# jithendaraa/ODE-RL

Hardware: AMD Instinct MI355X
Metric: integrated latent frames/sec (ODEConvGRU, MovingMNIST) (higher is better)
Workload: dtype f32; 1 GPU; ODEConvGRU latents z0 (B=64,64,16,16) per GPU, T=10 output frames (9 intervals), fixed-step rk4 (3/8 rule), f = 5x conv3x3(64->64)+ReLU, forward only (BASELINE configs[1]); per_gpu_batch=64, frames=10, method=rk4, parallelism=batch-shard x1, nfe=36

## Files before the change

### include/odecgru_hip.h

```cpp
#ifndef ODECGRU_HIP_H
#define ODECGRU_HIP_H

#include <stddef.h>
#include <stdint.h>

#ifdef __cplusplus
extern "C" {
#endif

#define ODEHIP_ABI_VERSION 13
#define ODEHIP_MAX_LAYERS 8
#define ODEHIP_MAX_STAGES 7

enum {
  ODEHIP_OK = 0,
  ODEHIP_EINVAL = -1,
  ODEHIP_EHIP = -2,
  ODEHIP_ENOTCONV = -3,
  ODEHIP_ENAN = -4,
  ODEHIP_ETRUNC = -5
};

enum { ODEHIP_EULER = 0, ODEHIP_MIDPOINT = 1, ODEHIP_RK4 = 2, ODEHIP_DOPRI5 = 3 };

const char* odehip_last_error(void);
int odehip_version(void);
void odehip_set_debug_flags(int flags);
void odehip_set_debug_buffer(void* device_buffer);


size_t odehip_packed_weight_floats(int cout, int cin, int ks);

int odehip_pack_conv_weight(const float* w_oihw, float* w_packed, int cout, int cin, int ks,
                            int transpose_flip, void* stream);

size_t odehip_winograd_weight_floats(int cout, int cin);
int odehip_pack_conv_weight_winograd(const float* w_oihw, float* w_wino, int cout, int cin, int transpose_flip, void* stream);
#define ODEHIP_MAX_PACK_JOBS 32
typedef struct odehip_pack_job {
  const float* w;
  float* out;
  int cout, cin, ks, kind, transpose_flip;
} odehip_pack_job;
int odehip_pack_conv_weights(const odehip_pack_job* jobs, int n_jobs, void* stream);
size_t odehip_winograd5_weight_floats(int cout, int cin);
int odehip_pack_conv_weight_winograd5(const float* w_oihw, float* w_wino, int cout, int cin, int transpose_flip, void* stream);

size_t odehip_bf16_weight_bytes(int cout, int cin);
int odehip_pack_conv_weight_bf16(const float* w_oihw, void* w_bf16, int cout, int cin, int transpose_flip, void* stream);
size_t odehip_fused_bf16_weight_bytes(int n_layers);
int odehip_pack_convstack_fused_bf16(const float* w_oihw, void* w_fused, int exec_index, int transpose_flip, void* stream);
int odehip_pack_conv_weight_bf16_ks(const float* w_oihw, void* w_bf16, int cout, int cin, int ks, int transpose_flip, void* stream);

int odehip_nchw_to_q4(const float* src_nchw, float* dst_q4, int batch, int channels, void* stream);
int odehip_q4_to_nchw(const float* src_q4, float* dst_nchw, int batch, int channels, void* stream);


typedef struct odehip_conv_desc {
  const float* src1;
  const float* src2;
  int cin1, cin, cout, ks, batch;
  const float* w_packed;
  const float* w_wino;
  const void* w_bf16;
  const float* bias;
  float* dst;
  int relu;
} odehip_conv_desc;

int odehip_conv_q4(const odehip_conv_desc* d, void* stream);
struct odehip_convstack;
int odehip_debug_repeat_f(const struct odehip_convstack* f, const float* x_q4, float* out_q4, float* scratch, int batch, int n,
                          void* stream);
int odehip_debug_repeat_conv(const odehip_conv_desc* d, int n, void* stream);


typedef struct odehip_convstack {
  int n_convs;
  int ks;
  int channels[ODEHIP_MAX_LAYERS + 1];
  const float* w_packed[ODEHIP_MAX_LAYERS];
  const float* w_wino[ODEHIP_MAX_LAYERS];
  const void* w_bf16[ODEHIP_MAX_LAYERS];
  const void* w_fused;
  const float* bias[ODEHIP_MAX_LAYERS];
  int final_tanh;
  int act;
} odehip_convstack;

size_t odehip_convstack_workspace_bytes(const odehip_convstack* f, int batch);

int odehip_convstack_forward(const odehip_convstack* f, const float* y_nchw, float* out_nchw, int batch,
                             int negate, void* workspace, size_t workspace_bytes, void* stream);


size_t odehip_odeint_workspace_bytes(const odehip_convstack* f, int batch, int n_times, int method,
                                     int save_for_backward);

int odehip_odeint_fixed(const odehip_convstack* f, int method, const float* z0_nchw, const double* t_host,
                        int n_times, int batch, float* out_nchw, int save_for_backward, int negate, void* workspace,
                        size_t workspace_bytes, int* saved_format_out, void* stream);

int odehip_odeint_fixed_backward(const odehip_convstack* f, const odehip_convstack* f_dgrad, int method, const double* t_host,
                                 int n_times, int batch, const float* grad_out_nchw, float* grad_z0_nchw, float* const* grad_w,
                                 float* const* grad_b, int saved_format, void* workspace, size_t workspace_bytes, void* stream);

int odehip_odeint_adjoint_backward(const odehip_convstack* f, const odehip_convstack* f_dgrad, int method, const double* t_host,
                                   int n_times, int batch, const float* y_traj_nchw, const float* grad_out_nchw,
                                   float* grad_z0_nchw, float* const* grad_w, float* const* grad_b, void* workspace,
                                   size_t workspace_bytes, void* stream);

size_t odehip_adjoint_dopri5_workspace_bytes(const odehip_convstack* f, int batch, int n_times, int max_accept);
int odehip_odeint_adjoint_dopri5_backward(const odehip_convstack* f, const odehip_convstack* f_dgrad, const double* t_host,
                                          int n_times, int batch, float rtol, float atol, const float* y_traj_nchw,
                                          const float* grad_out_nchw, float* grad_z0_nchw, float* const* grad_w,
                                          float* const* grad_b, int max_accept, int mixed_norm, int* stats_host, void* workspace,
                                          size_t workspace_bytes, void* stream);


typedef struct odehip_convgru_cell {
  int input, hidden, ks;
  const float* w_gates;
  const float* b_gates;
  const float* gn_gates_w;
  const float* gn_gates_b;
  const float* w_can;
  const float* b_can;
  const float* gn_can_w;
  const float* gn_can_b;
  const void* w_gates_bf16;
  const void* w_can_bf16;
  const float* w_gates_wino;
  const float* w_can_wino;
} odehip_convgru_cell;

size_t odehip_convgru_cell_workspace_bytes(const odehip_convgru_cell* c, int batch);
int odehip_convgru_cell_forward(const odehip_convgru_cell* c, const float* x_nchw, const float* h_nchw, float* h_next_nchw,
                                int batch, void* workspace, size_t workspace_bytes, void* stream);

typedef struct odehip_encoder {
  odehip_convstack f_enc;
  odehip_convgru_cell cell;
  int head_hidden, out_ch;
  const float* w_head0;
  const float* b_head0;
  const float* w_head1;
  const float* b_head1;
} odehip_encoder;

size_t odehip_encoder_workspace_bytes(const odehip_encoder* e, int n_frames, int batch);
int odehip_odeconvgru_encode(const odehip_encoder* e, const float* inputs_nchw, const double* t_host, int n_frames, int batch,
                             int run_backwards, float* mean_nchw, float* std_nchw, float* latent_nchw, void* workspace,
                             size_t workspace_bytes, void* stream);
int odehip_odeconvgru_encode_masked(const odehip_encoder* e, const float* inputs_nchw, const double* t_host, int n_frames, int batch,
                                    int run_backwards, float* mean_nchw, float* std_nchw, float* latent_nchw, void* workspace,
                                    size_t workspace_bytes, void* stream, const float* mask_tb);
int odehip_odeconvgru_encode_steps(const odehip_encoder* e, const float* inputs_nchw, const double* t_host, int n_frames, int batch,
                                   int run_backwards, float* mean_nchw, float* std_nchw, float* latent_nchw, void* workspace,
                                   size_t workspace_bytes, void* stream, const float* mask_tb, const unsigned char* step_observed_host,
                                   int* cell_steps_run);

typedef struct odehip_convgru_cell_bwd {
  const float* w_gates_dx;
  const float* w_gates_dh;
  const float* w_can_dx;
  const float* w_can_dh;
  const void* bf16[4];
  const float* wino[4];
} odehip_convgru_cell_bwd;
typedef struct odehip_convgru_cell_grads {
  float *w_gates, *b_gates, *gn_gates_w, *gn_gates_b, *w_can, *b_can, *gn_can_w, *gn_can_b;
} odehip_convgru_cell_grads;
size_t odehip_convgru_cell_backward_workspace_bytes(const odehip_convgru_cell* c, int batch);
int odehip_convgru_cell_backward(const odehip_convgru_cell* c, const odehip_convgru_cell_bwd* cb, const float* x_nchw,
                                 const float* h_nchw, const float* grad_h_next_nchw, float* grad_x_nchw, float* grad_h_nchw,
                                 const odehip_convgru_cell_grads* grads, int batch, void* workspace, size_t workspace_bytes,
                                 void* stream);

typedef struct odehip_convgru_cell_halves {
  const float* wino[4];
  const void* bf16[4];
} odehip_convgru_cell_halves;
size_t odehip_convgru_sequence_workspace_bytes(const odehip_convgru_cell* c, int n_steps, int batch, int has_x, int train);
int odehip_convgru_sequence_forward(const odehip_convgru_cell* c, const odehip_convgru_cell_halves* hv, const float* x_seq_nchw, const float* h0_nchw, int n_steps,
                                    int batch, float* h_seq_nchw, void* workspace, size_t workspace_bytes, void* stream);
int odehip_convgru_sequence_train(const odehip_convgru_cell* c, const odehip_convgru_cell_halves* hv, const float* x_seq_nchw, const float* h0_nchw, int n_steps, int batch,
                                  float* h_seq_nchw, void* workspace, size_t workspace_bytes, void* stream);
int odehip_convgru_sequence_backward(const odehip_convgru_cell* c, const odehip_convgru_cell_halves* hv, const odehip_convgru_cell_bwd* cb, int has_x, int has_h0,
                                     int n_steps, int batch, const float* grad_h_seq_nchw, float* grad_x_seq_nchw,
                                     float* grad_h0_nchw, const odehip_convgru_cell_grads* grads, void* workspace,
                                     size_t workspace_bytes, void* stream);


typedef struct odehip_encoder_bwd {
  odehip_convstack f_dgrad;
  const float* w_gates_dx;
  const float* w_gates_dh;
  const float* w_can_dx;
  const float* w_can_dh;
  const float* w_head0_t;
  const float* w_head1_t;
  const void* bf16[4];
  const float* wino[4];
} odehip_encoder_bwd;

typedef struct odehip_encoder_grads {
  float* f_w[ODEHIP_MAX_LAYERS];
  float* f_b[ODEHIP_MAX_LAYERS];
  float *w_gates, *b_gates, *gn_gates_w, *gn_gates_b, *w_can, *b_can, *gn_can_w, *gn_can_b;
  float *w_head0, *b_head0, *w_head1, *b_head1;
} odehip_encoder_grads;

size_t odehip_encoder_train_workspace_bytes(const odehip_encoder* e, int n_frames, int batch);
int odehip_odeconvgru_encode_train(const odehip_encoder* e, const float* inputs_nchw, const double* t_host, int n_frames, int batch,
                                   int run_backwards, float* mean_nchw, float* std_nchw, float* latent_nchw, void* workspace,
                                   size_t workspace_bytes, void* stream);
int odehip_odeconvgru_encode_backward(const odehip_encoder* e, const odehip_encoder_bwd* eb, const double* t_host, int n_frames,
                                      int batch, int run_backwards, const float* grad_mean_nchw, const float* grad_std_nchw,
                                      const float* grad_latent_nchw, float* grad_inputs_nchw, const odehip_encoder_grads* grads,
                                      void* workspace, size_t workspace_bytes, void* stream);
int odehip_odeconvgru_encode_train_masked(const odehip_encoder* e, const float* inputs_nchw, const double* t_host, int n_frames,
                                          int batch, int run_backwards, float* mean_nchw, float* std_nchw, float* latent_nchw,
                                          void* workspace, size_t workspace_bytes, void* stream, const float* mask_tb);
int odehip_odeconvgru_encode_backward_masked(const odehip_encoder* e, const odehip_encoder_bwd* eb, const double* t_host, int n_frames,
                                             int batch, int run_backwards, const float* grad_mean_nchw, const float* grad_std_nchw,
                                             const float* grad_latent_nchw, float* grad_inputs_nchw, const odehip_encoder_grads* grads,
                                             void* workspace, size_t workspace_bytes, void* stream, const float* mask_tb);
int odehip_odeconvgru_encode_train_steps(const odehip_encoder* e, const float* inputs_nchw, const double* t_host, int n_frames,
                                         int batch, int run_backwards, float* mean_nchw, float* std_nchw, float* latent_nchw,
                                         void* workspace, size_t workspace_bytes, void* stream, const float* mask_tb,
                                         const unsigned char* step_observed_host, int* cell_steps_run);
int odehip_odeconvgru_encode_backward_steps(const odehip_encoder* e, const odehip_encoder_bwd* eb, const double* t_host, int n_frames,
                                            int batch, int run_backwards, const float* grad_mean_nchw, const float* grad_std_nchw,
                                            const float* grad_latent_nchw, float* grad_inputs_nchw, const odehip_encoder_grads* grads,
                                            void* workspace, size_t workspace_bytes, void* stream, const float* mask_tb,
                                            const unsigned char* step_observed_host, int* cell_steps_run);


typedef int (*odehip_allreduce_fn)(float* scratch_dev, int n, void* stream, void* user);
int odehip_set_norm_allreduce(odehip_allreduce_fn cb, void* user, int world_size, float* scratch_dev);

size_t odehip_dopri5_workspace_bytes(const odehip_convstack* f, int batch, int n_times);

int odehip_odeint_dopri5(const odehip_convstack* f, const float* z0_nchw, const double* t_host, int n_times, int batch,
                         float rtol, float atol, double first_step, int max_steps, int negate, float* out_nchw,
                         int* stats_host, double* accepted_host, int accepted_cap, void* workspace, size_t workspace_bytes,
                         void* stream);

size_t odehip_dopri5_backward_workspace_bytes(const odehip_convstack* f, int batch, int n_times, int n_steps);
int odehip_odeint_dopri5_backward(const odehip_convstack* f, const odehip_convstack* f_dgrad, const double* t_host, int n_times,
                                  int batch, const double* accepted_host, int n_steps, const float* z0_nchw,
                                  const float* grad_out_nchw, float* grad_z0_nchw, float* const* grad_w, float* const* grad_b,
                                  void* workspace, size_t workspace_bytes, void* stream);

size_t odehip_dopri5_saving_workspace_bytes(const odehip_convstack* f, int batch, int n_times, int max_accept);
int odehip_odeint_dopri5_saving(const odehip_convstack* f, const float* z0_nchw, const double* t_host, int n_times, int batch,
                                float rtol, float atol, double first_step, int max_steps, float* out_nchw, int* stats_host,
                                double* accepted_host, int accepted_cap, int max_accept, int* saved_out, void* workspace,
                                size_t workspace_bytes, void* stream);
int odehip_odeint_dopri5_backward_saved(const odehip_convstack* f, const odehip_convstack* f_dgrad, const double* t_host, int n_times,
                                        int batch, const double* accepted_host, int n_steps, const float* grad_out_nchw,
                                        float* grad_z0_nchw, float* const* grad_w, float* const* grad_b, int max_accept,
                                        void* saved_workspace, size_t saved_workspace_bytes, void* stream);

int odehip_odeint_dopri5_start(const odehip_convstack* f, const float* z0_nchw, const double* t_host, int n_times, int batch,
                               float rtol, float atol, double first_step, int max_steps, float* out_nchw, int max_accept,
                               int attempts, int* token_out, void* workspace, size_t workspace_bytes, void* stream);
int odehip_odeint_dopri5_collect(int token, int* stats_host, double* accepted_host, int accepted_cap, int* saved_out);


int odehip_adam_step(float* const* params, const float* const* grads, float* const* exp_avg, float* const* exp_avg_sq,
                     const long long* numel, int n_tensors, float lr, float beta1, float beta2, float eps, float weight_decay,
                     int step, void* stream);

size_t odehip_grad_norm_workspace_bytes(int n_tensors, const long long* numel);
int odehip_grad_norm(const float* const* grads, const long long* numel, int n_tensors, float max_norm, void* partials_ws, size_t ws_bytes,
                     float* out3, void* stream);
int odehip_grad_scale(float* const* grads, const long long* numel, int n_tensors, const float* coef_dev, void* stream);
int odehip_adam_step_clipped(float* const* params, float* const* grads, float* const* exp_avg, float* const* exp_avg_sq,
                             const long long* numel, int n_tensors, float lr, float beta1, float beta2, float eps, float weight_decay,
                             int step, const float* coef_dev, void* stream);

int odehip_adamax_step(float* const* params, const float* const* grads, float* const* exp_avg, float* const* exp_inf,
                       const long long* numel, int n_tensors, float lr, float beta1, float beta2, float eps, float weight_decay,
                       int step, void* stream);
int odehip_adamax_step_clipped(float* const* params, float* const* grads, float* const* exp_avg, float* const* exp_inf,
                               const long long* numel, int n_tensors, float lr, float beta1, float beta2, float eps, float weight_decay,
                               int step, const float* coef_dev, void* stream);


int odehip_warp_composite(const float* pred_outputs, const float* start_image, const float* grid_x, const float* grid_y, int batch,
                          int n_times, int channels, int height, int width, float* pred_x, float* warped, float* masks,
                          void* stream);
int odehip_warp_composite_backward(const float* pred_outputs, const float* start_image, const float* warped, const float* grid_x,
                                   const float* grid_y, const float* grad_pred_x, const float* grad_warped, const float* grad_masks,
                                   int batch, int n_times, int channels, int height, int width, float* grad_pred_outputs,
                                   float* grad_start_image, void* stream);

int odehip_upsample2x_bilinear(const float* in, float* out, long long planes, int height, int width, void* stream);
int odehip_upsample2x_bilinear_backward(const float* grad_out, float* grad_in, long long planes, int height, int width, void* stream);

size_t odehip_bn_workspace_bytes(int channels);
int odehip_bn_relu_up2x_forward(const float* x, int batch, int channels, int height, int width, const float* weight, const float* bias,
                                float* running_mean, float* running_var, int training, float momentum, float eps, int upsample, float* out,
                                float* mean_out, float* invstd_out, float* scale_out, float* shift_out, void* workspace,
                                size_t workspace_bytes, void* stream);
int odehip_bn_relu_up2x_backward(const float* grad_out, const float* x, int batch, int channels, int height, int width, const float* mean,
                                 const float* invstd, const float* scale, const float* shift, int training, int upsample, float* grad_x,
                                 float* grad_weight, float* grad_bias, float* g_pre, void* workspace, size_t workspace_bytes, void* stream);

int odehip_bn_sync_stats(const float* x, int batch, int channels, int height, int width, double* sums, void* workspace, size_t workspace_bytes,
                         void* stream);
int odehip_bn_sync_relu_up2x_forward(const float* x, int batch, int channels, int height, int width, const double* sums, const float* weight,
                                     const float* bias, float* running_mean, float* running_var, float momentum, float eps, int upsample,
                                     float* out, float* mean_out, float* invstd_out, float* scale_out, float* shift_out, void* stream);
int odehip_bn_sync_backward_sums(const float* grad_out, const float* x, int batch, int channels, int height, int width, const float* mean,
                                 const float* invstd, const float* scale, const float* shift, int upsample, float* g_pre, float* grad_weight,
                                 float* grad_bias, double* sums, void* workspace, size_t workspace_bytes, void* stream);
int odehip_bn_sync_backward_apply(const float* g_pre, const float* x, int batch, int channels, int height, int width, const float* mean,
                                  const float* invstd, const float* scale, const double* sums, const double* count, float* grad_x,
                                  void* workspace, size_t workspace_bytes, void* stream);

size_t odehip_frame_encoder_pack_floats(int in_ch, int out_ch);
int odehip_pack_frame_encoder(const float* w1, const float* b1, const float* w2, const float* b2, int in_ch, int out_ch, float* pack,
                              void* stream);
int odehip_frame_encode(const float* pack, const float* frames, int batch, int n_frames, int in_ch, int out_ch, float negative_slope,
                        float* out_time_first, void* stream);
size_t odehip_frame_decoder_pack_floats(int in_ch, int out_ch);
int odehip_pack_frame_decoder(const float* w1, const float* b1, const float* w2, const float* b2, int in_ch, int out_ch, float* pack,
                              void* stream);
int odehip_frame_decode(const float* pack, const float* latents, int n_images, int in_ch, int out_ch, float negative_slope,
                        int apply_sigmoid, float* out, void* stream);
int odehip_frame_decode_train(const float* pack, const float* latents, int n_images, int in_ch, int out_ch, float negative_slope,
                              int apply_sigmoid, float* out, float* mid_save, void* stream);
size_t odehip_frame_decode_backward_workspace_floats(int n_images, int in_ch, int out_ch);
int odehip_frame_decode_backward(const float* pack, const float* w1, const float* latents, const float* mid_saved, const float* pred,
                                 const float* g_out, int n_images, int in_ch, int out_ch, float negative_slope, int sigmoid_applied,
                                 float* g_latents, float* dw1, float* db1, float* dw2, float* db2, float* workspace,
                                 size_t workspace_floats, void* stream);
size_t odehip_frame_encode_backward_workspace_floats(int batch, int n_frames, int in_ch, int out_ch);
int odehip_frame_encode_backward(const float* pack, const float* w2, const float* frames, const float* out_time_first,
                                 const float* g_out_time_first, int batch, int n_frames, int in_ch, int out_ch, float negative_slope,
                                 float* dw1, float* db1, float* dw2, float* db2, float* workspace, size_t workspace_floats, void* stream);

int odehip_set_persistent_trajectory(int enable);
long long odehip_persistent_trajectory_launches(void);
int odehip_persistent_error(int clear);

int odehip_mmnist_render(const double* init, const int* digit_ids, const unsigned char* glyphs, int n_glyphs,
                         const float* lut256, int batch, int n_digits, int t_in, int t_out, float* out_in, float* out_pred,
                         void* stream);

int odehip_vidode_batch(const unsigned char* store, long long store_frames, int height, int width, int channels,
                        const float* lut256, const int* table, long long table_words, int batch, int n_outputs, float* const* outs,
                        const int* n_frames, void* stream);

int odehip_vidode_batch_rotated(const unsigned char* store, long long store_frames, int height, int width, int channels,
                                const unsigned char* frame_min, int input_norm, const int* table, long long table_words, int batch,
                                int n_outputs, float* const* outs, const int* n_frames, void* stream);

int odehip_frame_metrics(const float* pred, const float* truth, int batch, int n_frames, int channels, int height, int width,
                         float data_range, float* sse, float* ssim, float* mse, float* psnr, float* ssim_t, void* stream);

int odehip_png_metrics(const float* pred, const float* truth, int batch, int n_frames, int channels, int size, int denorm,
                       long long* sse, double* mse, double* ssim, unsigned char* pred_bytes, unsigned char* truth_bytes, void* accum,
                       void* stream);

int odehip_latent_sample(const float* mean, const float* std, int batch, int channels, int height, int width, int n_samples,
                         uint64_t seed, uint64_t offset, int batch_offset, int global_batch, const float* eps_in, float* z0, float* kl,
                         float* eps_out, void* stream);
int odehip_latent_sample_backward(const float* grad_z0, const float* grad_kl, const float* mean, const float* std, int batch,
                                  int channels, int height, int width, int n_samples, uint64_t seed, uint64_t offset, int batch_offset,
                                  int global_batch, const float* eps_in, float* grad_mean, float* grad_std, void* stream);

size_t odehip_loss_mse_workspace_bytes(int n_samples, int batch, long long row_elems);
int odehip_loss_mse(const float* pred, const float* truth, int n_samples, int batch, long long row_elems, const float* kl, double kl_scale,
                    float kl_weight, float* out, void* workspace, size_t workspace_bytes, void* stream);
int odehip_loss_mse_backward(const float* grad_out, const float* pred, const float* truth, int n_samples, int batch, long long row_elems,
                             double kl_scale, float kl_weight, float* grad_pred, float* grad_kl, void* stream);

size_t odehip_loss_vidode_l1_workspace_bytes(int batch, int n_sel, int frame_elems);
int odehip_loss_vidode_l1(const float* pred, const float* inter, long long inter_batch_stride, long long inter_frame_stride,
                          const float* truth, const float* init, long long init_batch_stride, const void* mask, int mask_is_byte, int batch,
                          int n_frames, int n_sel, int frame_elems, float* out, void* workspace, size_t workspace_bytes, void* stream);
int odehip_loss_vidode_l1_backward(const float* grad_out, const float* pred, const float* inter, long long inter_batch_stride,
                                   long long inter_frame_stride, const float* truth, const float* init, long long init_batch_stride,
                                   const void* mask, int mask_is_byte, int batch, int n_frames, int n_sel, int frame_elems, float* grad_pred,
                                   float* grad_inter, void* stream);

int odehip_instnorm_lrelu_forward(const float* x, int planes, int hw, float eps, float slope, float* y, float* mean, float* rstd,
                                  void* stream);
int odehip_instnorm_lrelu_backward(const float* grad_y, const float* x, const float* mean, const float* rstd, int planes, int hw,
                                   float slope, float* grad_x, void* stream);

int odehip_gan_seq_assemble(const float* input_real, const float* frames, int batch, int t_in, int t, long long frame_elems, int interp,
                            float* out, void* stream);
int odehip_gan_seq_assemble_backward(const float* grad_out, int batch, int t_in, int t, long long frame_elems, int interp, float* grad_frames,
                                     void* stream);

size_t odehip_loss_lsgan_workspace_bytes(long long n);
int odehip_loss_lsgan(const float* pred, long long n, float target, float* out, void* workspace, void* stream);
int odehip_loss_lsgan_backward(const float* grad_out, const float* pred, long long n, float target, float* grad, void* stream);

size_t odehip_grid_table_bytes(int n_grid, int n_times);
int odehip_grid_emit_table(const double* grid, int n_grid, const double* t, int n_times, int* first, float* slope, int* exact);
int odehip_grid_emit(const float* grid_states, float* out, const int* first, const float* slope, const int* exact, int n_grid,
                     int n_times, long long state_floats, void* table_dev, size_t table_bytes, void* stream);
int odehip_grid_scatter(const float* grad_out, float* grad_grid, const int* first, const float* slope, const int* exact, int n_grid,
                        int n_times, long long state_floats, void* table_dev, size_t table_bytes, void* stream);

#ifdef __cplusplus
}
#endif
#endif
```

### ode-rl_amd/_lib.py

```python
import ctypes
import os

_HERE = os.path.dirname(os.path.abspath(__file__))
LIB_PATH = os.environ.get("ODEHIP_LIB") or os.path.join(_HERE, "lib", "libodecgru_hip.so")

ABI_VERSION = 13
MAX_LAYERS = 8
MAX_STAGES = 7
EULER, MIDPOINT, RK4, DOPRI5 = 0, 1, 2, 3
METHODS = {"euler": EULER, "midpoint": MIDPOINT, "rk4": RK4, "dopri5": DOPRI5}

c_float_p = ctypes.POINTER(ctypes.c_float)


class ConvDesc(ctypes.Structure):
    _fields_ = [
        ("src1", ctypes.c_void_p), ("src2", ctypes.c_void_p),
        ("cin1", ctypes.c_int), ("cin", ctypes.c_int), ("cout", ctypes.c_int), ("ks", ctypes.c_int),
        ("batch", ctypes.c_int),
        ("w_packed", ctypes.c_void_p), ("w_wino", ctypes.c_void_p), ("w_bf16", ctypes.c_void_p), ("bias", ctypes.c_void_p),
        ("dst", ctypes.c_void_p), ("relu", ctypes.c_int),
    ]


MAX_PACK_JOBS = 32


class PackJob(ctypes.Structure):
    _fields_ = [("w", ctypes.c_void_p), ("out", ctypes.c_void_p), ("cout", ctypes.c_int), ("cin", ctypes.c_int), ("ks", ctypes.c_int),
                ("kind", ctypes.c_int), ("transpose_flip", ctypes.c_int)]


ACT_RELU, ACT_TANH = 0, 1


class ConvStack(ctypes.Structure):
    _fields_ = [
        ("n_convs", ctypes.c_int), ("ks", ctypes.c_int),
        ("channels", ctypes.c_int * (MAX_LAYERS + 1)),
        ("w_packed", ctypes.c_void_p * MAX_LAYERS),
        ("w_wino", ctypes.c_void_p * MAX_LAYERS),
        ("w_bf16", ctypes.c_void_p * MAX_LAYERS),
        ("w_fused", ctypes.c_void_p),
        ("bias", ctypes.c_void_p * MAX_LAYERS),
        ("final_tanh", ctypes.c_int),
        ("act", ctypes.c_int),
    ]


class ConvGRUCellDesc(ctypes.Structure):
    _fields_ = [("input", ctypes.c_int), ("hidden", ctypes.c_int), ("ks", ctypes.c_int),
                ("w_gates", ctypes.c_void_p), ("b_gates", ctypes.c_void_p), ("gn_gates_w", ctypes.c_void_p),
                ("gn_gates_b", ctypes.c_void_p), ("w_can", ctypes.c_void_p), ("b_can", ctypes.c_void_p),
                ("gn_can_w", ctypes.c_void_p), ("gn_can_b", ctypes.c_void_p),
                ("w_gates_bf16", ctypes.c_void_p), ("w_can_bf16", ctypes.c_void_p),
                ("w_gates_wino", ctypes.c_void_p), ("w_can_wino", ctypes.c_void_p)]


class ConvGRUCellHalves(ctypes.Structure):
    _fields_ = [("wino", ctypes.c_void_p * 4), ("bf16", ctypes.c_void_p * 4)]


class EncoderDesc(ctypes.Structure):
    _fields_ = [("f_enc", ConvStack), ("cell", ConvGRUCellDesc), ("head_hidden", ctypes.c_int), ("out_ch", ctypes.c_int),
                ("w_head0", ctypes.c_void_p), ("b_head0", ctypes.c_void_p), ("w_head1", ctypes.c_void_p),
                ("b_head1", ctypes.c_void_p)]


class ConvGRUCellBwd(ctypes.Structure):
    _fields_ = [("w_gates_dx", ctypes.c_void_p), ("w_gates_dh", ctypes.c_void_p), ("w_can_dx", ctypes.c_void_p),
                ("w_can_dh", ctypes.c_void_p), ("bf16", ctypes.c_void_p * 4), ("wino", ctypes.c_void_p * 4)]


class ConvGRUCellGrads(ctypes.Structure):
    _fields_ = [("w_gates", ctypes.c_void_p), ("b_gates", ctypes.c_void_p), ("gn_gates_w", ctypes.c_void_p),
                ("gn_gates_b", ctypes.c_void_p), ("w_can", ctypes.c_void_p), ("b_can", ctypes.c_void_p),
                ("gn_can_w", ctypes.c_void_p), ("gn_can_b", ctypes.c_void_p)]


class EncoderBwd(ctypes.Structure):
    _fields_ = [("f_dgrad", ConvStack), ("w_gates_dx", ctypes.c_void_p), ("w_gates_dh", ctypes.c_void_p),
                ("w_can_dx", ctypes.c_void_p), ("w_can_dh", ctypes.c_void_p), ("w_head0_t", ctypes.c_void_p),
                ("w_head1_t", ctypes.c_void_p), ("bf16", ctypes.c_void_p * 4), ("wino", ctypes.c_void_p * 4)]


class EncoderGrads(ctypes.Structure):
    _fields_ = [("f_w", ctypes.c_void_p * MAX_LAYERS), ("f_b", ctypes.c_void_p * MAX_LAYERS),
                ("w_gates", ctypes.c_void_p), ("b_gates", ctypes.c_void_p), ("gn_gates_w", ctypes.c_void_p),
                ("gn_gates_b", ctypes.c_void_p), ("w_can", ctypes.c_void_p), ("b_can", ctypes.c_void_p),
                ("gn_can_w", ctypes.c_void_p), ("gn_can_b", ctypes.c_void_p), ("w_head0", ctypes.c_void_p),
                ("b_head0", ctypes.c_void_p), ("w_head1", ctypes.c_void_p), ("b_head1", ctypes.c_void_p)]


ALLREDUCE_FN = ctypes.CFUNCTYPE(ctypes.c_int, ctypes.c_void_p, ctypes.c_int, ctypes.c_void_p, ctypes.c_void_p)


class OdeHipError(RuntimeError):
    pass


class AsyncSolveTruncated(OdeHipError):
    """An asynchronous dopri5 solve needed more attempted steps than were enqueued up front (ODEHIP_ETRUNC): the frames it had not
    reached are NaN and everything computed from them since is invalid.  The next asynchronous solve enqueues more; a training step
    can simply be repeated (nothing has been applied to the parameters)."""


_lib = None

SIGNATURES = {
    "odehip_last_error": (ctypes.c_char_p, []),
    "odehip_version": (ctypes.c_int, []),
    "odehip_bf16_weight_bytes": (ctypes.c_size_t, [ctypes.c_int, ctypes.c_int]),
    "odehip_pack_conv_weight_bf16": (ctypes.c_int, [ctypes.c_void_p, ctypes.c_void_p, ctypes.c_int, ctypes.c_int, ctypes.c_int,
                                                    ctypes.c_void_p]),
    "odehip_adam_step": (ctypes.c_int, [ctypes.POINTER(ctypes.c_void_p), ctypes.POINTER(ctypes.c_void_p),
                                        ctypes.POINTER(ctypes.c_void_p), ctypes.POINTER(ctypes.c_void_p),
                                        ctypes.POINTER(ctypes.c_longlong), ctypes.c_int, ctypes.c_float, ctypes.c_float,
                                        ctypes.c_float, ctypes.c_float, ctypes.c_float, ctypes.c_int, ctypes.c_void_p]),
    "odehip_grad_norm_workspace_bytes": (ctypes.c_size_t, [ctypes.c_int, ctypes.POINTER(ctypes.c_longlong)]),
    "odehip_grad_norm": (ctypes.c_int, [ctypes.POINTER(ctypes.c_void_p), ctypes.POINTER(ctypes.c_longlong), ctypes.c_int, ctypes.c_float,
                                        ctypes.c_void_p, ctypes.c_size_t, ctypes.c_void_p, ctypes.c_void_p]),
    "odehip_grad_scale": (ctypes.c_int, [ctypes.POINTER(ctypes.c_void_p), ctypes.POINTER(ctypes.c_longlong), ctypes.c_int, ctypes.c_void_p,
                                         ctypes.c_void_p]),
    "odehip_adam_step_clipped": (ctypes.c_int, [ctypes.POINTER(ctypes.c_void_p), ctypes.POINTER(ctypes.c_void_p),
                                                ctypes.POINTER(ctypes.c_void_p), ctypes.POINTER(ctypes.c_void_p),
                                                ctypes.POINTER(ctypes.c_longlong), ctypes.c_int, ctypes.c_float, ctypes.c_float,
                                                ctypes.c_float, ctypes.c_float, ctypes.c_float, ctypes.c_int, ctypes.c_void_p,
                                                ctypes.c_void_p]),
    "odehip_adamax_step": (ctypes.c_int, [ctypes.POINTER(ctypes.c_void_p)] * 4 + [ctypes.POINTER(ctypes.c_longlong), ctypes.c_int] +
                           [ctypes.c_float] * 5 + [ctypes.c_int, ctypes.c_void_p]),
    "odehip_adamax_step_clipped": (ctypes.c_int, [ctypes.POINTER(ctypes.c_void_p)] * 4 + [ctypes.POINTER(ctypes.c_longlong), ctypes.c_int] +
                                   [ctypes.c_float] * 5 + [ctypes.c_int, ctypes.c_void_p, ctypes.c_void_p]),
    "odehip_set_persistent_trajectory": (ctypes.c_int, [ctypes.c_int]),
    "odehip_persistent_trajectory_launches": (ctypes.c_longlong, []),
    "odehip_persistent_error": (ctypes.c_int, [ctypes.c_int]),
    "odehip_upsample2x_bilinear": (ctypes.c_int, [ctypes.c_void_p, ctypes.c_void_p, ctypes.c_longlong, ctypes.c_int, ctypes.c_int, ctypes.c_void_p]),
    "odehip_upsample2x_bilinear_backward": (ctypes.c_int, [ctypes.c_void_p, ctypes.c_void_p, ctypes.c_longlong, ctypes.c_int, ctypes.c_int,
                                                            ctypes.c_void_p]),
    "odehip_bn_workspace_bytes": (ctypes.c_size_t, [ctypes.c_int]),
    "odehip_bn_relu_up2x_forward": (ctypes.c_int, [ctypes.c_void_p] + [ctypes.c_int] * 4 + [ctypes.c_void_p] * 4 + [ctypes.c_int, ctypes.c_float,
                                                   ctypes.c_float, ctypes.c_int] + [ctypes.c_void_p] * 6 + [ctypes.c_size_t, ctypes.c_void_p]),
    "odehip_bn_relu_up2x_backward": (ctypes.c_int, [ctypes.c_void_p] * 2 + [ctypes.c_int] * 4 + [ctypes.c_void_p] * 4 + [ctypes.c_int] * 2 +
                                     [ctypes.c_void_p] * 5 + [ctypes.c_size_t, ctypes.c_void_p]),
    "odehip_bn_sync_stats": (ctypes.c_int, [ctypes.c_void_p] + [ctypes.c_int] * 4 + [ctypes.c_void_p] * 2 + [ctypes.c_size_t, ctypes.c_void_p]),
    "odehip_bn_sync_relu_up2x_forward": (ctypes.c_int, [ctypes.c_void_p] + [ctypes.c_int] * 4 + [ctypes.c_void_p] * 5 + [ctypes.c_float] * 2 +
                                         [ctypes.c_int] + [ctypes.c_void_p] * 6),
    "odehip_bn_sync_backward_sums": (ctypes.c_int, [ctypes.c_void_p] * 2 + [ctypes.c_int] * 4 + [ctypes.c_void_p] * 4 + [ctypes.c_int] +
                                     [ctypes.c_void_p] * 5 + [ctypes.c_size_t, ctypes.c_void_p]),
    "odehip_bn_sync_backward_apply": (ctypes.c_int, [ctypes.c_void_p] * 2 + [ctypes.c_int] * 4 + [ctypes.c_void_p] * 7 + [ctypes.c_size_t, ctypes.c_void_p]),
    "odehip_warp_composite": (ctypes.c_int, [ctypes.c_void_p] * 4 + [ctypes.c_int] * 5 + [ctypes.c_void_p] * 4),
    "odehip_warp_composite_backward": (ctypes.c_int, [ctypes.c_void_p] * 8 + [ctypes.c_int] * 5 + [ctypes.c_void_p] * 3),
    "odehip_winograd5_weight_floats": (ctypes.c_size_t, [ctypes.c_int, ctypes.c_int]),
    "odehip_pack_conv_weight_winograd5": (ctypes.c_int, [ctypes.c_void_p, ctypes.c_void_p, ctypes.c_int, ctypes.c_int, ctypes.c_int, ctypes.c_void_p]),
    "odehip_frame_encoder_pack_floats": (ctypes.c_size_t, [ctypes.c_int, ctypes.c_int]),
    "odehip_frame_decoder_pack_floats": (ctypes.c_size_t, [ctypes.c_int, ctypes.c_int]),
    "odehip_pack_frame_encoder": (ctypes.c_int, [ctypes.c_void_p] * 4 + [ctypes.c_int] * 2 + [ctypes.c_void_p] * 2),
    "odehip_pack_frame_decoder": (ctypes.c_int, [ctypes.c_void_p] * 4 + [ctypes.c_int] * 2 + [ctypes.c_void_p] * 2),
    "odehip_frame_encode": (ctypes.c_int, [ctypes.c_void_p, ctypes.c_void_p, ctypes.c_int, ctypes.c_int, ctypes.c_int, ctypes.c_int,
                                           ctypes.c_float, ctypes.c_void_p, ctypes.c_void_p]),
    "odehip_frame_decode_backward_workspace_floats": (ctypes.c_size_t, [ctypes.c_int] * 3),
    "odehip_frame_decode_train": (ctypes.c_int, [ctypes.c_void_p, ctypes.c_void_p, ctypes.c_int, ctypes.c_int, ctypes.c_int, ctypes.c_float,
                                                 ctypes.c_int, ctypes.c_void_p, ctypes.c_void_p, ctypes.c_void_p]),
    "odehip_frame_decode_backward": (ctypes.c_int, [ctypes.c_void_p] * 6 + [ctypes.c_int] * 3 + [ctypes.c_float, ctypes.c_int] +
                                     [ctypes.c_void_p] * 6 + [ctypes.c_size_t, ctypes.c_void_p]),
    "odehip_frame_encode_backward_workspace_floats": (ctypes.c_size_t, [ctypes.c_int] * 4),
    "odehip_frame_encode_backward": (ctypes.c_int, [ctypes.c_void_p] * 5 + [ctypes.c_int] * 4 + [ctypes.c_float] +
                                     [ctypes.c_void_p] * 5 + [ctypes.c_size_t, ctypes.c_void_p]),
    "odehip_frame_decode": (ctypes.c_int, [ctypes.c_void_p, ctypes.c_void_p, ctypes.c_int, ctypes.c_int, ctypes.c_int, ctypes.c_float,
                                           ctypes.c_int, ctypes.c_void_p, ctypes.c_void_p]),
    "odehip_mmnist_render": (ctypes.c_int, [ctypes.c_void_p, ctypes.c_void_p, ctypes.c_void_p, ctypes.c_int, ctypes.c_void_p,
                                            ctypes.c_int, ctypes.c_int, ctypes.c_int, ctypes.c_int, ctypes.c_void_p,
                                            ctypes.c_void_p, ctypes.c_void_p]),
    "odehip_vidode_batch": (ctypes.c_int, [ctypes.c_void_p, ctypes.c_longlong, ctypes.c_int, ctypes.c_int, ctypes.c_int, ctypes.c_void_p,
                                           ctypes.c_void_p, ctypes.c_longlong, ctypes.c_int, ctypes.c_int, ctypes.POINTER(ctypes.c_void_p),
                                           ctypes.POINTER(ctypes.c_int), ctypes.c_void_p]),
    "odehip_vidode_batch_rotated": (ctypes.c_int, [ctypes.c_void_p, ctypes.c_longlong, ctypes.c_int, ctypes.c_int, ctypes.c_int,
                                                   ctypes.c_void_p, ctypes.c_int, ctypes.c_void_p, ctypes.c_longlong, ctypes.c_int,
                                                   ctypes.c_int, ctypes.POINTER(ctypes.c_void_p), ctypes.POINTER(ctypes.c_int),
                                                   ctypes.c_void_p]),
    "odehip_frame_metrics": (ctypes.c_int, [ctypes.c_void_p] * 2 + [ctypes.c_int] * 5 + [ctypes.c_float] + [ctypes.c_void_p] * 6),
    "odehip_png_metrics": (ctypes.c_int, [ctypes.c_void_p] * 2 + [ctypes.c_int] * 5 + [ctypes.c_void_p] * 7),
    "odehip_latent_sample": (ctypes.c_int, [ctypes.c_void_p] * 2 + [ctypes.c_int] * 5 + [ctypes.c_uint64] * 2 + [ctypes.c_int] * 2 +
                             [ctypes.c_void_p] * 5),
    "odehip_latent_sample_backward": (ctypes.c_int, [ctypes.c_void_p] * 4 + [ctypes.c_int] * 5 + [ctypes.c_uint64] * 2 + [ctypes.c_int] * 2 +
                                      [ctypes.c_void_p] * 4),
    "odehip_loss_mse_workspace_bytes": (ctypes.c_size_t, [ctypes.c_int, ctypes.c_int, ctypes.c_longlong]),
    "odehip_loss_mse": (ctypes.c_int, [ctypes.c_void_p] * 2 + [ctypes.c_int, ctypes.c_int, ctypes.c_longlong, ctypes.c_void_p, ctypes.c_double,
                                       ctypes.c_float, ctypes.c_void_p, ctypes.c_void_p, ctypes.c_size_t, ctypes.c_void_p]),
    "odehip_loss_mse_backward": (ctypes.c_int, [ctypes.c_void_p] * 3 + [ctypes.c_int, ctypes.c_int, ctypes.c_longlong, ctypes.c_double,
                                                ctypes.c_float] + [ctypes.c_void_p] * 3),
    "odehip_loss_vidode_l1_workspace_bytes": (ctypes.c_size_t, [ctypes.c_int] * 3),
    "odehip_loss_vidode_l1": (ctypes.c_int, [ctypes.c_void_p] * 2 + [ctypes.c_longlong] * 2 + [ctypes.c_void_p] * 2 + [ctypes.c_longlong,
                                             ctypes.c_void_p] + [ctypes.c_int] * 5 + [ctypes.c_void_p] * 2 + [ctypes.c_size_t, ctypes.c_void_p]),
    "odehip_loss_vidode_l1_backward": (ctypes.c_int, [ctypes.c_void_p] * 3 + [ctypes.c_longlong] * 2 + [ctypes.c_void_p] * 2 +
                                       [ctypes.c_longlong, ctypes.c_void_p] + [ctypes.c_int] * 5 + [ctypes.c_void_p] * 3),
    "odehip_instnorm_lrelu_forward": (ctypes.c_int, [ctypes.c_void_p, ctypes.c_int, ctypes.c_int, ctypes.c_float, ctypes.c_float] +
                                      [ctypes.c_void_p] * 4),
    "odehip_instnorm_lrelu_backward": (ctypes.c_int, [ctypes.c_void_p] * 4 + [ctypes.c_int, ctypes.c_int, ctypes.c_float] + [ctypes.c_void_p] * 2),
    "odehip_gan_seq_assemble": (ctypes.c_int, [ctypes.c_void_p] * 2 + [ctypes.c_int] * 3 + [ctypes.c_longlong, ctypes.c_int] + [ctypes.c_void_p] * 2),
    "odehip_gan_seq_assemble_backward": (ctypes.c_int, [ctypes.c_void_p] + [ctypes.c_int] * 3 + [ctypes.c_longlong, ctypes.c_int] +
                                         [ctypes.c_void_p] * 2),
    "odehip_loss_lsgan_workspace_bytes": (ctypes.c_size_t, [ctypes.c_longlong]),
    "odehip_loss_lsgan": (ctypes.c_int, [ctypes.c_void_p, ctypes.c_longlong, ctypes.c_float] + [ctypes.c_void_p] * 3),
    "odehip_loss_lsgan_backward": (ctypes.c_int, [ctypes.c_void_p] * 2 + [ctypes.c_longlong, ctypes.c_float] + [ctypes.c_void_p] * 2),
    "odehip_grid_table_bytes":(ctypes.c_size_t, [ctypes.c_int, ctypes.c_int]),
    "odehip_grid_emit_table": (ctypes.c_int, [ctypes.POINTER(ctypes.c_double), ctypes.c_int, ctypes.POINTER(ctypes.c_double), ctypes.c_int,
                                              ctypes.POINTER(ctypes.c_int), ctypes.POINTER(ctypes.c_float), ctypes.POINTER(ctypes.c_int)]),
    "odehip_grid_emit": (ctypes.c_int, [ctypes.c_void_p, ctypes.c_void_p, ctypes.POINTER(ctypes.c_int), ctypes.POINTER(ctypes.c_float),
                                        ctypes.POINTER(ctypes.c_int), ctypes.c_int, ctypes.c_int, ctypes.c_longlong, ctypes.c_void_p,
                                        ctypes.c_size_t, ctypes.c_void_p]),
    "odehip_grid_scatter": (ctypes.c_int, [ctypes.c_void_p, ctypes.c_void_p, ctypes.POINTER(ctypes.c_int), ctypes.POINTER(ctypes.c_float),
                                           ctypes.POINTER(ctypes.c_int), ctypes.c_int, ctypes.c_int, ctypes.c_longlong, ctypes.c_void_p,
                                           ctypes.c_size_t, ctypes.c_void_p]),
    "odehip_fused_bf16_weight_bytes": (ctypes.c_size_t, [ctypes.c_int]),
    "odehip_pack_convstack_fused_bf16": (ctypes.c_int, [ctypes.c_void_p, ctypes.c_void_p, ctypes.c_int, ctypes.c_int, ctypes.c_void_p]),
    "odehip_pack_conv_weight_bf16_ks": (ctypes.c_int, [ctypes.c_void_p, ctypes.c_void_p, ctypes.c_int, ctypes.c_int, ctypes.c_int,
                                                       ctypes.c_int, ctypes.c_void_p]),
    "odehip_debug_repeat_f": (ctypes.c_int, [ctypes.POINTER(ConvStack), ctypes.c_void_p, ctypes.c_void_p, ctypes.c_void_p, ctypes.c_int,
                                             ctypes.c_int, ctypes.c_void_p]),
    "odehip_set_debug_flags": (None, [ctypes.c_int]),
    "odehip_set_norm_allreduce": (ctypes.c_int, [ctypes.c_void_p, ctypes.c_void_p, ctypes.c_int, ctypes.c_void_p]),
    "odehip_set_debug_buffer": (None, [ctypes.c_void_p]),
    "odehip_packed_weight_floats": (ctypes.c_size_t, [ctypes.c_int, ctypes.c_int, ctypes.c_int]),
    "odehip_pack_conv_weight": (ctypes.c_int, [ctypes.c_void_p, ctypes.c_void_p, ctypes.c_int, ctypes.c_int,
                                               ctypes.c_int, ctypes.c_int, ctypes.c_void_p]),
    "odehip_winograd_weight_floats": (ctypes.c_size_t, [ctypes.c_int, ctypes.c_int]),
    "odehip_pack_conv_weights": (ctypes.c_int, [ctypes.c_void_p, ctypes.c_int, ctypes.c_void_p]),
    "odehip_pack_conv_weight_winograd": (ctypes.c_int, [ctypes.c_void_p, ctypes.c_void_p, ctypes.c_int, ctypes.c_int,
                                                        ctypes.c_int, ctypes.c_void_p]),
    "odehip_nchw_to_q4": (ctypes.c_int, [ctypes.c_void_p, ctypes.c_void_p, ctypes.c_int, ctypes.c_int, ctypes.c_void_p]),
    "odehip_q4_to_nchw": (ctypes.c_int, [ctypes.c_void_p, ctypes.c_void_p, ctypes.c_int, ctypes.c_int, ctypes.c_void_p]),
    "odehip_conv_q4": (ctypes.c_int, [ctypes.POINTER(ConvDesc), ctypes.c_void_p]),
    "odehip_debug_repeat_conv": (ctypes.c_int, [ctypes.POINTER(ConvDesc), ctypes.c_int, ctypes.c_void_p]),
    "odehip_convstack_workspace_bytes": (ctypes.c_size_t, [ctypes.POINTER(ConvStack), ctypes.c_int]),
    "odehip_convstack_forward": (ctypes.c_int, [ctypes.POINTER(ConvStack), ctypes.c_void_p, ctypes.c_void_p,
                                                ctypes.c_int, ctypes.c_int, ctypes.c_void_p, ctypes.c_size_t,
                                                ctypes.c_void_p]),
    "odehip_odeint_workspace_bytes": (ctypes.c_size_t, [ctypes.POINTER(ConvStack), ctypes.c_int, ctypes.c_int,
                                                        ctypes.c_int, ctypes.c_int]),
    "odehip_odeint_fixed": (ctypes.c_int, [ctypes.POINTER(ConvStack), ctypes.c_int, ctypes.c_void_p,
                                           ctypes.POINTER(ctypes.c_double), ctypes.c_int, ctypes.c_int,
                                           ctypes.c_void_p, ctypes.c_int, ctypes.c_int, ctypes.c_void_p, ctypes.c_size_t,
                                           ctypes.POINTER(ctypes.c_int), ctypes.c_void_p]),
    "odehip_odeint_fixed_backward": (ctypes.c_int, [ctypes.POINTER(ConvStack), ctypes.POINTER(ConvStack), ctypes.c_int,
                                                    ctypes.POINTER(ctypes.c_double), ctypes.c_int, ctypes.c_int,
                                                    ctypes.c_void_p, ctypes.c_void_p, ctypes.POINTER(ctypes.c_void_p),
                                                    ctypes.POINTER(ctypes.c_void_p), ctypes.c_int, ctypes.c_void_p, ctypes.c_size_t,
                                                    ctypes.c_void_p]),
    "odehip_odeint_adjoint_backward": (ctypes.c_int, [ctypes.POINTER(ConvStack), ctypes.POINTER(ConvStack), ctypes.c_int,
                                                      ctypes.POINTER(ctypes.c_double), ctypes.c_int, ctypes.c_int,
                                                      ctypes.c_void_p, ctypes.c_void_p, ctypes.c_void_p,
                                                      ctypes.POINTER(ctypes.c_void_p), ctypes.POINTER(ctypes.c_void_p),
                                                      ctypes.c_void_p, ctypes.c_size_t, ctypes.c_void_p]),
    "odehip_adjoint_dopri5_workspace_bytes": (ctypes.c_size_t, [ctypes.POINTER(ConvStack), ctypes.c_int, ctypes.c_int,
                                                                ctypes.c_int]),
    "odehip_odeint_adjoint_dopri5_backward": (ctypes.c_int, [ctypes.POINTER(ConvStack), ctypes.POINTER(ConvStack),
                                                             ctypes.POINTER(ctypes.c_double), ctypes.c_int, ctypes.c_int,
                                                             ctypes.c_float, ctypes.c_float, ctypes.c_void_p,
                                                             ctypes.c_void_p, ctypes.c_void_p,
                                                             ctypes.POINTER(ctypes.c_void_p), ctypes.POINTER(ctypes.c_void_p),
                                                             ctypes.c_int, ctypes.c_int, ctypes.POINTER(ctypes.c_int), ctypes.c_void_p,
                                                             ctypes.c_size_t, ctypes.c_void_p]),
    "odehip_convgru_cell_workspace_bytes": (ctypes.c_size_t, [ctypes.POINTER(ConvGRUCellDesc), ctypes.c_int]),
    "odehip_convgru_cell_forward": (ctypes.c_int, [ctypes.POINTER(ConvGRUCellDesc), ctypes.c_void_p, ctypes.c_void_p,
                                                   ctypes.c_void_p, ctypes.c_int, ctypes.c_void_p, ctypes.c_size_t,
                                                   ctypes.c_void_p]),
    "odehip_convgru_sequence_workspace_bytes": (ctypes.c_size_t, [ctypes.POINTER(ConvGRUCellDesc)] + [ctypes.c_int] * 4),
    "odehip_convgru_sequence_forward": (ctypes.c_int, [ctypes.POINTER(ConvGRUCellDesc), ctypes.POINTER(ConvGRUCellHalves), ctypes.c_void_p, ctypes.c_void_p, ctypes.c_int,
                                                       ctypes.c_int, ctypes.c_void_p, ctypes.c_void_p, ctypes.c_size_t, ctypes.c_void_p]),
    "odehip_convgru_sequence_train": (ctypes.c_int, [ctypes.POINTER(ConvGRUCellDesc), ctypes.POINTER(ConvGRUCellHalves), ctypes.c_void_p, ctypes.c_void_p, ctypes.c_int,
                                                     ctypes.c_int, ctypes.c_void_p, ctypes.c_void_p, ctypes.c_size_t, ctypes.c_void_p]),
    "odehip_convgru_sequence_backward": (ctypes.c_int, [ctypes.POINTER(ConvGRUCellDesc), ctypes.POINTER(ConvGRUCellHalves), ctypes.POINTER(ConvGRUCellBwd)] + [ctypes.c_int] * 4 +
                                         [ctypes.c_void_p] * 3 + [ctypes.POINTER(ConvGRUCellGrads), ctypes.c_void_p, ctypes.c_size_t,
                                                                  ctypes.c_void_p]),
    "odehip_encoder_workspace_bytes": (ctypes.c_size_t, [ctypes.POINTER(EncoderDesc), ctypes.c_int, ctypes.c_int]),
    "odehip_odeconvgru_encode": (ctypes.c_int, [ctypes.POINTER(EncoderDesc), ctypes.c_void_p,
                                                ctypes.POINTER(ctypes.c_double), ctypes.c_int, ctypes.c_int, ctypes.c_int,
                                                ctypes.c_void_p, ctypes.c_void_p, ctypes.c_void_p, ctypes.c_void_p,
                                                ctypes.c_size_t, ctypes.c_void_p]),
    "odehip_odeconvgru_encode_masked": (ctypes.c_int, [ctypes.POINTER(EncoderDesc), ctypes.c_void_p,
                                                       ctypes.POINTER(ctypes.c_double), ctypes.c_int, ctypes.c_int, ctypes.c_int,
                                                       ctypes.c_void_p, ctypes.c_void_p, ctypes.c_void_p, ctypes.c_void_p,
                                                       ctypes.c_size_t, ctypes.c_void_p, ctypes.c_void_p]),
    "odehip_dopri5_workspace_bytes": (ctypes.c_size_t, [ctypes.POINTER(ConvStack), ctypes.c_int, ctypes.c_int]),
    "odehip_convgru_cell_backward_workspace_bytes": (ctypes.c_size_t, [ctypes.POINTER(ConvGRUCellDesc), ctypes.c_int]),
    "odehip_convgru_cell_backward": (ctypes.c_int, [ctypes.POINTER(ConvGRUCellDesc), ctypes.POINTER(ConvGRUCellBwd),
                                                    ctypes.c_void_p, ctypes.c_void_p, ctypes.c_void_p, ctypes.c_void_p,
                                                    ctypes.c_void_p, ctypes.POINTER(ConvGRUCellGrads), ctypes.c_int,
                                                    ctypes.c_void_p, ctypes.c_size_t, ctypes.c_void_p]),
    "odehip_encoder_train_workspace_bytes": (ctypes.c_size_t, [ctypes.POINTER(EncoderDesc), ctypes.c_int, ctypes.c_int]),
    "odehip_odeconvgru_encode_train": (ctypes.c_int, [ctypes.POINTER(EncoderDesc), ctypes.c_void_p,
                                                      ctypes.POINTER(ctypes.c_double), ctypes.c_int, ctypes.c_int, ctypes.c_int,
                                                      ctypes.c_void_p, ctypes.c_void_p, ctypes.c_void_p, ctypes.c_void_p,
                                                      ctypes.c_size_t, ctypes.c_void_p]),
    "odehip_odeconvgru_encode_backward": (ctypes.c_int, [ctypes.POINTER(EncoderDesc), ctypes.POINTER(EncoderBwd),
                                                         ctypes.POINTER(ctypes.c_double), ctypes.c_int, ctypes.c_int, ctypes.c_int,
                                                         ctypes.c_void_p, ctypes.c_void_p, ctypes.c_void_p, ctypes.c_void_p,
                                                         ctypes.POINTER(EncoderGrads), ctypes.c_void_p, ctypes.c_size_t,
                                                         ctypes.c_void_p]),
    "odehip_odeconvgru_encode_train_masked": (ctypes.c_int, [ctypes.POINTER(EncoderDesc), ctypes.c_void_p,
                                                             ctypes.POINTER(ctypes.c_double), ctypes.c_int, ctypes.c_int, ctypes.c_int,
                                                             ctypes.c_void_p, ctypes.c_void_p, ctypes.c_void_p, ctypes.c_void_p,
                                                             ctypes.c_size_t, ctypes.c_void_p, ctypes.c_void_p]),
    "odehip_odeconvgru_encode_backward_masked": (ctypes.c_int, [ctypes.POINTER(EncoderDesc), ctypes.POINTER(EncoderBwd),
                                                                ctypes.POINTER(ctypes.c_double), ctypes.c_int, ctypes.c_int, ctypes.c_int,
                                                                ctypes.c_void_p, ctypes.c_void_p, ctypes.c_void_p, ctypes.c_void_p,
                                                                ctypes.POINTER(EncoderGrads), ctypes.c_void_p, ctypes.c_size_t,
                                                                ctypes.c_void_p, ctypes.c_void_p]),
    "odehip_odeconvgru_encode_steps": (ctypes.c_int, [ctypes.POINTER(EncoderDesc), ctypes.c_void_p,
                                                      ctypes.POINTER(ctypes.c_double), ctypes.c_int, ctypes.c_int, ctypes.c_int,
                                                      ctypes.c_void_p, ctypes.c_void_p, ctypes.c_void_p, ctypes.c_void_p,
                                                      ctypes.c_size_t, ctypes.c_void_p, ctypes.c_void_p, ctypes.c_void_p,
                                                      ctypes.POINTER(ctypes.c_int)]),
    "odehip_odeconvgru_encode_train_steps": (ctypes.c_int, [ctypes.POINTER(EncoderDesc), ctypes.c_void_p,
                                                            ctypes.POINTER(ctypes.c_double), ctypes.c_int, ctypes.c_int, ctypes.c_int,
                                                            ctypes.c_void_p, ctypes.c_void_p, ctypes.c_void_p, ctypes.c_void_p,
                                                            ctypes.c_size_t, ctypes.c_void_p, ctypes.c_void_p, ctypes.c_void_p,
                                                            ctypes.POINTER(ctypes.c_int)]),
    "odehip_odeconvgru_encode_backward_steps": (ctypes.c_int, [ctypes.POINTER(EncoderDesc), ctypes.POINTER(EncoderBwd),
                                                               ctypes.POINTER(ctypes.c_double), ctypes.c_int, ctypes.c_int, ctypes.c_int,
                                                               ctypes.c_void_p, ctypes.c_void_p, ctypes.c_void_p, ctypes.c_void_p,
                                                               ctypes.POINTER(EncoderGrads), ctypes.c_void_p, ctypes.c_size_t,
                                                               ctypes.c_void_p, ctypes.c_void_p, ctypes.c_void_p,
                                                               ctypes.POINTER(ctypes.c_int)]),
    "odehip_odeint_dopri5": (ctypes.c_int, [ctypes.POINTER(ConvStack), ctypes.c_void_p, ctypes.POINTER(ctypes.c_double),
                                            ctypes.c_int, ctypes.c_int, ctypes.c_float, ctypes.c_float, ctypes.c_double, ctypes.c_int,
                                            ctypes.c_int, ctypes.c_void_p, ctypes.POINTER(ctypes.c_int),
                                            ctypes.POINTER(ctypes.c_double), ctypes.c_int, ctypes.c_void_p,
                                            ctypes.c_size_t, ctypes.c_void_p]),
    "odehip_dopri5_backward_workspace_bytes": (ctypes.c_size_t, [ctypes.POINTER(ConvStack), ctypes.c_int, ctypes.c_int,
                                                                 ctypes.c_int]),
    "odehip_dopri5_saving_workspace_bytes": (ctypes.c_size_t, [ctypes.POINTER(ConvStack), ctypes.c_int, ctypes.c_int, ctypes.c_int]),
    "odehip_odeint_dopri5_saving": (ctypes.c_int, [ctypes.POINTER(ConvStack), ctypes.c_void_p, ctypes.POINTER(ctypes.c_double),
                                                   ctypes.c_int, ctypes.c_int, ctypes.c_float, ctypes.c_float, ctypes.c_double, ctypes.c_int,
                                                   ctypes.c_void_p, ctypes.POINTER(ctypes.c_int), ctypes.POINTER(ctypes.c_double),
                                                   ctypes.c_int, ctypes.c_int, ctypes.POINTER(ctypes.c_int), ctypes.c_void_p,
                                                   ctypes.c_size_t, ctypes.c_void_p]),
    "odehip_odeint_dopri5_start": (ctypes.c_int, [ctypes.POINTER(ConvStack), ctypes.c_void_p, ctypes.POINTER(ctypes.c_double),
                                                  ctypes.c_int, ctypes.c_int, ctypes.c_float, ctypes.c_float, ctypes.c_double, ctypes.c_int,
                                                  ctypes.c_void_p, ctypes.c_int, ctypes.c_int, ctypes.POINTER(ctypes.c_int), ctypes.c_void_p,
                                                  ctypes.c_size_t, ctypes.c_void_p]),
    "odehip_odeint_dopri5_collect": (ctypes.c_int, [ctypes.c_int, ctypes.POINTER(ctypes.c_int), ctypes.POINTER(ctypes.c_double), ctypes.c_int,
                                                    ctypes.POINTER(ctypes.c_int)]),
    "odehip_odeint_dopri5_backward_saved": (ctypes.c_int, [ctypes.POINTER(ConvStack), ctypes.POINTER(ConvStack),
                                                           ctypes.POINTER(ctypes.c_double), ctypes.c_int, ctypes.c_int,
                                                           ctypes.POINTER(ctypes.c_double), ctypes.c_int, ctypes.c_void_p, ctypes.c_void_p,
                                                           ctypes.POINTER(ctypes.c_void_p), ctypes.POINTER(ctypes.c_void_p), ctypes.c_int,
                                                           ctypes.c_void_p, ctypes.c_size_t, ctypes.c_void_p]),
    "odehip_odeint_dopri5_backward": (ctypes.c_int, [ctypes.POINTER(ConvStack), ctypes.POINTER(ConvStack),
                                                     ctypes.POINTER(ctypes.c_double), ctypes.c_int, ctypes.c_int,
                                                     ctypes.POINTER(ctypes.c_double), ctypes.c_int, ctypes.c_void_p,
                                                     ctypes.c_void_p, ctypes.c_void_p, ctypes.POINTER(ctypes.c_void_p),
                                                     ctypes.POINTER(ctypes.c_void_p), ctypes.c_void_p, ctypes.c_size_t,
                                                     ctypes.c_void_p]),
}


def load():
    global _lib
    if _lib is not None:
        return _lib
    if not os.path.exists(LIB_PATH):
        raise OdeHipError(
            f"{LIB_PATH} is missing: build it with `python -c 'import __graft_entry__ as g; g.build()'` "
            "or `make -C ode-rl_amd/csrc`.  The HIP path has no CPU fallback.")
    lib = ctypes.CDLL(LIB_PATH)
    for name, (res, args) in SIGNATURES.items():
        fn = getattr(lib, name)
        fn.restype = res
        fn.argtypes = args
    got = lib.odehip_version()
    if got != ABI_VERSION:
        raise OdeHipError(f"{LIB_PATH} reports ABI version {got}, this binding needs {ABI_VERSION}: rebuild the library (make -C ode-rl_amd/csrc)")
    _lib = lib
    return lib


def check(rc):
    if rc == 0:
        code = _lib.odehip_persistent_error(1) if _lib is not None else 0
        if code:
            raise OdeHipError(f"a persistent launch of THIS OR AN EARLIER call gave up waiting for a partner workgroup (code {code}): the word is "
                              "read without synchronising, so the kernel that set it may belong to any call enqueued since the last check.  "
                              "Results since then are invalid (whole-trajectory launches NaN-fill their outputs; single-evaluation launches "
                              "may not); persistent launches are now disabled for this process")
        return
    msg = load().odehip_last_error().decode("utf-8", "replace")
    if rc == -1:
        raise ValueError(msg)
    if rc in (-3, -4):
        raise AssertionError(msg)
    if rc == -5:
        raise AsyncSolveTruncated(msg)
    raise OdeHipError(f"odehip status {rc}: {msg}")
```

### ode-rl_amd/csrc/conv_wino.hip

```cpp
#include <stddef.h>
#include <stdlib.h>
#include <string.h>

#include "conv_common.h"

namespace odehip {

constexpr int kWU = 32 * 1024;
constexpr int kWRaw = 16 * 1024;
constexpr int kWV = 32 * 1024;
constexpr int kWinoLds = 2 * kWRaw + 2 * kWV;
constexpr int kUAhead = 8;

__device__ __forceinline__ f32x4 load_u(__amdgpu_buffer_rsrc_t r, int voffset, int soffset) {
  return __builtin_bit_cast(f32x4, __builtin_amdgcn_raw_buffer_load_b128(r, voffset, soffset, 0));
}

__device__ __forceinline__ f32x4 pk_sub(f32x4 a, f32x4 b) {
  typedef float f32x2 __attribute__((ext_vector_type(2)));
  f32x2 lo, hi;
  const f32x2 alo = {a.x, a.y}, ahi = {a.z, a.w}, blo = {b.x, b.y}, bhi = {b.z, b.w};
  asm("v_pk_add_f32 %0, %1, %2 neg_lo:[0,1] neg_hi:[0,1]" : "=v"(lo) : "v"(alo), "v"(blo));
  asm("v_pk_add_f32 %0, %1, %2 neg_lo:[0,1] neg_hi:[0,1]" : "=v"(hi) : "v"(ahi), "v"(bhi));
  return f32x4{lo.x, lo.y, hi.x, hi.y};
}

struct PersistHook {
  unsigned* done = nullptr;
  unsigned target = 0u;
  int word0 = 0;
  unsigned* abort_ = nullptr;
  unsigned* host_err = nullptr;
  bool fence = false;
  float* nchw_base = nullptr;
  unsigned long long* stamps = nullptr;
  int batch = 0;
  bool first = true;
  bool solo = false;
  bool announce = true;
  bool split_wait = false;
  int sleep6 = 0;
  const unsigned long long* reloc = nullptr;
  unsigned wait_target = 0u;
};

template <typename T>
__device__ __forceinline__ T* rel(const unsigned long long* reloc, T* p) {
  const unsigned long long v = (unsigned long long)p;
  const unsigned cls = (unsigned)(v >> 56);
  if (cls == 0) return p;
  typedef const __attribute__((address_space(4))) unsigned long long ConstU;
  return (T*)((v & 0x00ffffffffffffffull) + *((ConstU*)reloc + cls));
}
__device__ __forceinline__ void pstamp(const PersistHook& hk, int i, int lane) {
  if (hk.stamps && lane == 0) hk.stamps[i] = __builtin_amdgcn_s_memrealtime();
}

template <typename T>
__device__ __forceinline__ T* uniform_ptr(T* p) {
  const unsigned long long v = (unsigned long long)p;
  const unsigned lo = __builtin_amdgcn_readfirstlane((unsigned)v), hi = __builtin_amdgcn_readfirstlane((unsigned)(v >> 32));
  return (T*)(((unsigned long long)hi << 32) | lo);
}

__device__ __forceinline__ void wait_done(const PersistHook& hk, int sel_mask = 0, int sel_val = 0) {
  int n = 0;
  const int lane = threadIdx.x & 63;
  const bool mine = lane < 16 && (lane & sel_mask) == sel_val;
  while (!__all(!mine || __hip_atomic_load(hk.done + (lane & 15), __ATOMIC_RELAXED, __HIP_MEMORY_SCOPE_AGENT) >= hk.wait_target)) {
    __builtin_amdgcn_s_sleep(1);
    if ((++n & 1023) == 0) {
      if (__hip_atomic_load(hk.abort_, __ATOMIC_RELAXED, __HIP_MEMORY_SCOPE_AGENT) == 1u) break;
      if (n > (1 << 23)) {
        __hip_atomic_store(hk.abort_, 1u, __ATOMIC_RELAXED, __HIP_MEMORY_SCOPE_AGENT);
        *hk.host_err = 3;
        break;
      }
    }
  }
  if (hk.fence) __builtin_amdgcn_fence(__ATOMIC_ACQUIRE, "agent");
}

__device__ __forceinline__ void announce(const PersistHook& hk, unsigned* done_word, bool stamp = false) {
  const int lane = threadIdx.x & 63;
  wait_vmcnt<0>();
  if (stamp) pstamp(hk, 7, lane);
  if (hk.fence) __builtin_amdgcn_fence(__ATOMIC_RELEASE, "agent");
  if (lane == 0 && hk.announce) __hip_atomic_store(done_word, hk.target + 1u, __ATOMIC_RELAXED, __HIP_MEMORY_SCOPE_AGENT);
}

template <int GROUP>
__device__ __forceinline__ bool xcc_rendezvous(unsigned* xcc_of, int lid, unsigned* abort_word, unsigned* host_err) {
  const unsigned my_xcc = (__builtin_amdgcn_s_getreg((3 << 11) | 20) & 15u) + 1u;
  if (threadIdx.x == 0) __hip_atomic_store(xcc_of + lid, my_xcc, __ATOMIC_RELAXED, __HIP_MEMORY_SCOPE_AGENT);
  bool fence = false;
  for (int p = 0; p < GROUP; ++p) {
    unsigned v = 0;
    int n = 0;
    while ((v = __hip_atomic_load(xcc_of + (lid & ~(GROUP - 1)) + p, __ATOMIC_RELAXED, __HIP_MEMORY_SCOPE_AGENT)) == 0) {
      __builtin_amdgcn_s_sleep(2);
      if (++n > (1 << 23)) {
        __hip_atomic_store(abort_word, 1u, __ATOMIC_RELAXED, __HIP_MEMORY_SCOPE_AGENT);
        *host_err = 2;
        break;
      }
    }
    fence |= (v != my_xcc);
  }
  return __builtin_amdgcn_readfirstlane(fence);
}

__device__ __forceinline__ bool walk_start(const ConvArgs*& table, int& n_layers, const int* section) {
  typedef const __attribute__((address_space(4))) int ConstI;
  const int* skip = table[0].skip;
  if (skip && *(ConstI*)skip) return false;
  if (section) {
    const int row0 = ((ConstI*)section)[0], n_dev = ((ConstI*)section)[1];
    if (row0 < 0 || n_dev <= 0 || row0 + n_dev > n_layers) return false;
    table += row0;
    n_layers = n_dev;
  }
  return true;
}

struct RowCursor {
  const ConvArgs* table;
  int n_layers;
  const float *src, *u, *src_next, *u_next;
  __device__ __forceinline__ RowCursor(const ConvArgs* t, int n)
      : table(t), n_layers(n), src(t[0].src1), u(t[0].w_wino), src_next(nullptr), u_next(nullptr) {}
  __device__ __forceinline__ const ConvArgs& row(int l) {
    typedef const __attribute__((address_space(4))) ConvArgs ConstArgs;
    const ConvArgs& a = *(const ConvArgs*)((ConstArgs*)table + l);
    src_next = src;
    u_next = u;
    if (l + 1 < n_layers) {
      src_next = table[l + 1].src1;
      u_next = table[l + 1].w_wino;
      if (threadIdx.x < (sizeof(ConvArgs) + 63) / 64) {
        const unsigned v = __builtin_nontemporal_load((const unsigned*)&table[l + 1] + threadIdx.x * 16);
        asm volatile("" ::"v"(v));
      }
    }
    return a;
  }
  __device__ __forceinline__ void next() {
    src = src_next;
    u = u_next;
  }
};

template <int NCHUNK, bool DBG, bool PERSIST, int QOUT = 16, bool ADAPT = false>
__device__ __forceinline__ void wino_layer(const float* __restrict__ p_src, const float* __restrict__ p_u, int p_qin, const ConvArgs& a,
                                           int b, int ct, int rh, char* smem, const PersistHook& hk) {
  static_assert(!PERSIST || (NCHUNK % 2 == 0), "the layer-to-layer LDS hand-over assumes an even chunk count");
  static_assert(kUAhead % 2 == 0 && kUAhead <= 16, "the U ring is refilled a pair of positions at a time");
  constexpr int kRawAux = PERSIST ? 16 : 0;
  char* const Rb = smem;
  char* const Vb = smem + 2 * kWRaw;
  Stamps st(a, (DBG && (a.debug & 16)) ? 256 : (DBG ? 0 : -1));
  st.take(0);
  const int tid = threadIdx.x;
  const int lane = tid & 63;
  const int wave = __builtin_amdgcn_readfirstlane(tid >> 6);
  const int r0 = rh * 8;
  constexpr int nchunk = NCHUNK;
  const bool skip = !PERSIST && a.skip && *a.skip;
  const bool dbg_noprod = DBG && (a.debug & 1), dbg_nomfma = DBG && (a.debug & 2), dbg_notr = DBG && (a.debug & 32),
             dbg_nodma = DBG && (a.debug & 128);

  if (wave >= 4) {
    const int pw = wave - 4, ptid = tid - 256;
    const __amdgpu_buffer_rsrc_t rx = make_rsrc((const char*)p_src + (size_t)b * p_qin * kQuadBytes, (unsigned)p_qin * kQuadBytes);
    int vr[4];
#pragma unroll
    for (int p = 0; p < 4; ++p) {
      const int s = 64 * p + lane;
      const int row = s / 20, w = s - row * 20;
      const int pc = w < 9 ? 2 * w : 2 * (w - 9) + 1;
      const int irow = r0 - 1 + row, col = pc - 1;
      vr[p] = (s < 200 && w < 18 && irow >= 0 && irow < kHW && col >= 0 && col < kHW) ? irow * 256 + col * 16 : kOobOffset;
    }
    auto issue_raw = [&](int c, int buf) {
#pragma unroll
      for (int p = 0; p < 4; ++p)
        __builtin_amdgcn_raw_ptr_buffer_load_lds(rx, ODEHIP_LDS_PTR(Rb + buf * kWRaw + (pw * 4 + p) * 1024), 16, vr[p],
                                                 (c * 4 + pw) * kQuadBytes, 0, kRawAux);
    };
    const int th = lane >> 5, tq = pw, tt = lane & 31;
    (void)ptid;
    const int tty = tt >> 3, ttx = tt & 7;
    const int r_a = th == 0 ? 2 : 1, r_b = th == 0 ? 0 : 2, r_c = th == 0 ? 1 : 3;
    const int raw_base = tq * 4096 + (2 * tty * 20 + ttx) * 16;
    const int off_a = raw_base + r_a * 320, off_b = raw_base + r_b * 320, off_c = raw_base + r_c * 320;
    const float sgn = th == 0 ? 1.0f : -1.0f;
    const int v_off = tq * 512 + tt * 16;
    auto transform = [&](int rbuf, int vbuf) {
      const char* r = Rb + rbuf * kWRaw;
      f32x4 d0[4], d1[4], d2[4];
#pragma unroll
      for (int j = 0; j < 4; ++j) {
        if (DBG && (a.debug & 512)) {
          d0[j] = d1[j] = d2[j] = f32x4{1.f, 2.f, 3.f, (float)j};
        } else {
          const int cj = ((j & 1) * 9 + (j >> 1)) * 16;
          d0[j] = *(const f32x4*)(r + off_a + cj);
          d1[j] = *(const f32x4*)(r + off_b + cj);
          d2[j] = *(const f32x4*)(r + off_c + cj);
        }
      }
      f32x4 T[2][4];
#pragma unroll
      for (int j = 0; j < 4; ++j) {
        T[0][j] = pk_sub(d1[j], d0[j]);
        T[1][j] = d2[j] + d0[j] * sgn;
      }
#pragma unroll
      for (int i = 0; i < 2; ++i) {
        char* v = Vb + vbuf * kWV + v_off + (2 * th + i) * 4 * 2048;
        if (DBG && (a.debug & 256)) {
          const f32x4 sum = (T[i][0] - T[i][2]) + (T[i][1] + T[i][2]) + (T[i][2] - T[i][1]) + (T[i][1] - T[i][3]);
          asm volatile("" ::"v"(sum.x), "v"(sum.y), "v"(sum.z), "v"(sum.w));
        } else {
          *(f32x4*)(v + 0 * 2048) = pk_sub(T[i][0], T[i][2]);
          *(f32x4*)(v + 1 * 2048) = T[i][1] + T[i][2];
          *(f32x4*)(v + 2 * 2048) = pk_sub(T[i][2], T[i][1]);
          *(f32x4*)(v + 3 * 2048) = pk_sub(T[i][1], T[i][3]);
        }
      }
    };

    if (PERSIST) {
      if (pw == 0) pstamp(hk, 0, lane);
      if (!hk.first) {
        if (hk.solo && hk.wait_target == hk.target)
          for (int i = 0; i < hk.sleep6; ++i) __builtin_amdgcn_s_sleep(6);
        if (hk.split_wait) wait_done(hk, 0x8, 0x0); else wait_done(hk);
      }
      if (pw == 0) pstamp(hk, 1, lane);
      issue_raw(0, 0);
      issue_raw(1, 1);
      wait_vmcnt<4>();
      if (pw == 0) pstamp(hk, 2, lane);
      transform(0, 0);
      if (pw == 0) pstamp(hk, 3, lane);
    } else if (!skip && !dbg_noprod) {
      issue_raw(0, 0);
      if (nchunk > 1) issue_raw(1, 1);
      if (nchunk > 1) wait_vmcnt<4>(); else wait_vmcnt<0>();
      transform(0, 0);
    }
    st.take(2);
#pragma unroll
    for (int c = 0; c < nchunk; ++c) {
      __builtin_amdgcn_s_barrier();
      if (!skip && !dbg_noprod && c + 1 < nchunk) {
        if (c + 2 < nchunk) {
          if (PERSIST && c == 0 && !hk.first && hk.split_wait) wait_done(hk, 0x8, 0x8);
          if (!dbg_nodma) issue_raw(c + 2, c & 1);
          wait_vmcnt<4>();
        } else {
          wait_vmcnt<0>();
        }
        if (!dbg_notr) transform((c + 1) & 1, (c + 1) & 1);
      }
      if (c < 4) st.take(3 + c);
    }
    st.flush(a);
    return;
  }

  const int ch = wave >> 1, thh = wave & 1;
  const int i16 = lane & 15, kq = lane >> 4;
  f32x4 acc[16];
#pragma unroll
  for (int x = 0; x < 16; ++x) acc[x] = f32x4{0.f, 0.f, 0.f, 0.f};
  const int u_off = kq * 512 + (ch * 16 + i16) * 16;
  const int v_off = kq * 512 + (thh * 16 + i16) * 16;
  constexpr int kG = 16 * NCHUNK;
  const bool dbg_nou = dbg_noprod || dbg_nodma;
  const __amdgpu_buffer_rsrc_t ru = make_rsrc((const char*)p_u + (size_t)ct * (NCHUNK * kWU), (unsigned)NCHUNK * kWU);
  f32x4 uw[kUAhead];
#pragma unroll
  for (int g = 0; g < kUAhead; ++g) {
    if (skip || dbg_nou) uw[g] = f32x4{1.f, 1.f, 1.f, 1.f};
    else uw[g] = load_u(ru, u_off, g * 2048);
  }
  const int Q = ct * 8 + ch * 4 + kq;
  f32x4 bias4 = {0.f, 0.f, 0.f, 0.f};
  if (a.bias) bias4 = *(const f32x4*)(a.bias + Q * 4);
  const int tile = thh * 16 + i16, oty = tile >> 3, otx = tile & 7;
  int e_combine = 0, e_act = 0, e_np = 0;
  float* e_dst = nullptr;
  float* e_kout = nullptr;
  float* e_out1 = nullptr;
  float* e_out2 = nullptr;
  float* e_nchw = nullptr;
  bool e_y = false;
  float e_h = 1.0f, e_ks = 1.0f, e_c1c = 0.0f, e_c2c = 0.0f, e_c1[3] = {0.f, 0.f, 0.f}, e_c2[3] = {0.f, 0.f, 0.f};
  f32x4 e_yv[4], e_kv[3][4];
  int d_kind = 0;
  f32x4 d_y[4], d_y1[4], d_sa[4], d_sb[4];
  float d_h = 1.0f, d_ks = 1.0f, d_cA = 0.0f, d_cB = 0.0f, d_rtol = 0.0f, d_atol = 0.0f, d_t[6] = {0.f, 0.f, 0.f, 0.f, 0.f, 0.f};
  float* d_o[4] = {nullptr, nullptr, nullptr, nullptr};
  bool d_has_y = false, d_err = false, d_f[4] = {false, false, false, false};
  if constexpr (ADAPT) {
    typedef const __attribute__((address_space(4))) float ConstF;
    const unsigned long long* const rl = hk.reloc;
    e_act = a.act;
    e_dst = rel(rl, a.dst);
    d_kind = a.combine == 0 ? 0 : 5;
    if (a.combine == 2) {
      const BwdArgs& w = a.bwd;
      const float hb = a.h_by_value ? a.cmb.atol : (w.h_ptr ? *(ConstF*)w.h_ptr : 0.0f);
      d_ks = w.sc_c + w.sc_h * hb;
      d_has_y = w.mask_src != nullptr;
      d_kind = 2;
      const float* const mask = rel(rl, w.mask_src);
#pragma unroll
      for (int q = 0; q < 4; ++q) {
        const size_t off = (((size_t)b * QOUT + Q) * kPix + (r0 + 2 * oty + (q >> 1)) * 16 + 2 * otx + (q & 1)) * 4;
        if (d_has_y) d_y[q] = *(const f32x4*)(mask + off);
      }
    } else if (a.combine == 3 && a.bwd.n_targets <= 2 && !a.bwd.h_ptr) {
      const BwdArgs& w = a.bwd;
      d_kind = 3;
#pragma unroll
      for (int t = 0; t < 2; ++t) {
        if (t < w.n_targets) {
          const BwdTarget& T = w.tgt[t];
          d_o[t] = rel(rl, T.out);
          d_t[3 * t] = T.g_c; d_t[3 * t + 1] = T.a_c; d_t[3 * t + 2] = T.b_c;
          d_f[2 * t] = T.srcA != nullptr; d_f[2 * t + 1] = T.srcB != nullptr;
          const float* const sA = rel(rl, T.srcA);
          const float* const sB = rel(rl, T.srcB);
#pragma unroll
          for (int q = 0; q < 4; ++q) {
            const size_t off = (((size_t)b * QOUT + Q) * kPix + (r0 + 2 * oty + (q >> 1)) * 16 + 2 * otx + (q & 1)) * 4;
            if (t == 0) {
              if (d_f[0]) d_y[q] = *(const f32x4*)(sA + off);
              if (d_f[1]) d_y1[q] = *(const f32x4*)(sB + off);
            } else {
              if (d_f[2]) d_sa[q] = *(const f32x4*)(sA + off);
              if (d_f[3]) d_sb[q] = *(const f32x4*)(sB + off);
            }
          }
        }
      }
    } else if (a.combine == 1 && (a.cmb.order == 1 || !a.cmb.y) && !(a.cmb.err_partials && (a.cmb.out2 || a.cmb.out2_nchw || a.dbg))) {
      const CombineArgs& m = a.cmb;
      d_kind = 1;
      const int np = m.n_prev;
      d_h = a.h_by_value ? m.atol : (m.h_ptr ? *(ConstF*)m.h_ptr : 1.0f);
      d_ks = m.k_scale;
      d_err = m.err_partials != nullptr;
      d_has_y = m.y != nullptr;
      d_cA = m.c1[np];
      d_cB = d_err ? m.ce[np] : m.c2[np];
      d_rtol = m.rtol; d_atol = m.atol;
      d_o[0] = rel(rl, m.k_out); d_o[1] = rel(rl, m.out1); d_o[2] = rel(rl, m.out2);
      d_o[3] = a.dbg ? hk.nchw_base + ((size_t)a.dbg - 1) : m.out2_nchw;
      const bool needB = d_err || d_o[2] || d_o[3];
      const float* const yp = rel(rl, m.y);
      const float* const y1p = rel(rl, m.err_y1);
#pragma unroll
      for (int q = 0; q < 4; ++q) {
        d_sa[q] = d_sb[q] = f32x4{0.f, 0.f, 0.f, 0.f};
        if (d_has_y) {
          const size_t off = (((size_t)b * QOUT + Q) * kPix + (r0 + 2 * oty + (q >> 1)) * 16 + 2 * otx + (q & 1)) * 4;
          d_y[q] = *(const f32x4*)(yp + off);
          if (d_err) d_y1[q] = *(const f32x4*)(y1p + off);
        }
      }
      if (d_has_y) {
        const float* kp[ODEHIP_MAX_STAGES - 1];
        float cA[ODEHIP_MAX_STAGES - 1], cB[ODEHIP_MAX_STAGES - 1];
#pragma unroll
        for (int j = 0; j < ODEHIP_MAX_STAGES - 1; ++j) {
          kp[j] = j < np ? rel(rl, m.k_prev[j]) : nullptr;
          cA[j] = m.c1[j];
          cB[j] = d_err ? m.ce[j] : m.c2[j];
        }
#pragma unroll
        for (int j = 0; j < ODEHIP_MAX_STAGES - 1; ++j) {
          if (j < np) {
#pragma unroll
            for (int q = 0; q < 4; ++q) {
              const size_t off = (((size_t)b * QOUT + Q) * kPix + (r0 + 2 * oty + (q >> 1)) * 16 + 2 * otx + (q & 1)) * 4;
              const f32x4 kv = *(const f32x4*)(kp[j] + off);
              d_sa[q] = fma4(kv, cA[j], d_sa[q]);
              if (needB) d_sb[q] = fma4(kv, cB[j], d_sb[q]);
            }
          }
        }
      }
    }
  } else if (PERSIST) {
    e_combine = a.combine;
    e_act = a.act;
    e_dst = a.dst;
    if (e_combine == 1 && !a.h_by_value) e_combine = 3;
    if (e_combine == 2) {
      const BwdArgs& w = a.bwd;
      typedef const __attribute__((address_space(4))) float ConstF;
      const float hb = a.h_by_value ? a.cmb.atol : (w.h_ptr ? *(ConstF*)w.h_ptr : 0.0f);
      e_ks = w.sc_c + w.sc_h * hb;
      e_y = w.mask_src != nullptr;
#pragma unroll
      for (int q = 0; q < 4; ++q) {
        const size_t off = (((size_t)b * QOUT + Q) * kPix + (r0 + 2 * oty + (q >> 1)) * 16 + 2 * otx + (q & 1)) * 4;
        if (e_y) e_yv[q] = *(const f32x4*)(w.mask_src + off);
      }
    } else if (e_combine == 1) {
      const CombineArgs& m = a.cmb;
      e_np = m.n_prev;
      e_h = m.atol;
      e_ks = m.k_scale;
      e_c1c = m.c1[e_np];
      e_c2c = m.c2[e_np];
      e_kout = m.k_out;
      e_out1 = m.out1;
      e_out2 = m.out2;
      e_nchw = a.dbg ? hk.nchw_base + ((size_t)a.dbg - 1) : nullptr;
      e_y = m.y != nullptr;
#pragma unroll
      for (int q = 0; q < 4; ++q) {
        const size_t off = (((size_t)b * QOUT + Q) * kPix + (r0 + 2 * oty + (q >> 1)) * 16 + 2 * otx + (q & 1)) * 4;
        if (e_y) e_yv[q] = *(const f32x4*)(m.y + off);
#pragma unroll
        for (int j = 0; j < 3; ++j)
          if (j < e_np) e_kv[j][q] = *(const f32x4*)(m.k_prev[j] + off);
      }
#pragma unroll
      for (int j = 0; j < 3; ++j) {
        e_c1[j] = m.c1[j];
        e_c2[j] = m.c2[j];
      }
    }
  }
  st.take(2);
#pragma unroll
  for (int c = 0; c < nchunk; ++c) {
    __builtin_amdgcn_s_barrier();
    if (PERSIST && c == 0 && wave == 0) pstamp(hk, 4, lane);
    if (!skip && !dbg_nomfma) {
      const char* v = Vb + (c & 1) * kWV + v_off;
      f32x4 x0 = *(const f32x4*)(v), x1 = *(const f32x4*)(v + 2048);
      f32x4 x0n, x1n;
#pragma unroll
      for (int x = 0; x < 16; x += 2) {
        const int g = c * 16 + x, s0 = g % kUAhead, s1 = (g + 1) % kUAhead;
        const f32x4 w0 = uw[s0], w1 = uw[s1];
        if (x + 2 < 16) {
          x0n = *(const f32x4*)(v + (x + 2) * 2048);
          x1n = *(const f32x4*)(v + (x + 3) * 2048);
        }
        if (g + kUAhead < kG && !dbg_nou) {
          uw[s0] = load_u(ru, u_off, (g + kUAhead) * 2048);
          uw[s1] = load_u(ru, u_off, (g + kUAhead + 1) * 2048);
        }
        acc[x] = __builtin_amdgcn_mfma_f32_16x16x4f32(w0.x, x0.x, acc[x], 0, 0, 0);
        acc[x + 1] = __builtin_amdgcn_mfma_f32_16x16x4f32(w1.x, x1.x, acc[x + 1], 0, 0, 0);
        acc[x] = __builtin_amdgcn_mfma_f32_16x16x4f32(w0.y, x0.y, acc[x], 0, 0, 0);
        acc[x + 1] = __builtin_amdgcn_mfma_f32_16x16x4f32(w1.y, x1.y, acc[x + 1], 0, 0, 0);
        acc[x] = __builtin_amdgcn_mfma_f32_16x16x4f32(w0.z, x0.z, acc[x], 0, 0, 0);
        acc[x + 1] = __builtin_amdgcn_mfma_f32_16x16x4f32(w1.z, x1.z, acc[x + 1], 0, 0, 0);
        acc[x] = __builtin_amdgcn_mfma_f32_16x16x4f32(w0.w, x0.w, acc[x], 0, 0, 0);
        acc[x + 1] = __builtin_amdgcn_mfma_f32_16x16x4f32(w1.w, x1.w, acc[x + 1], 0, 0, 0);
        x0 = x0n; x1 = x1n;
        __builtin_amdgcn_sched_group_barrier(0x008, 1, 0);
        __builtin_amdgcn_sched_group_barrier(0x100, 2, 0);
        __builtin_amdgcn_sched_group_barrier(0x020, 2, 0);
        __builtin_amdgcn_sched_group_barrier(0x008, 7, 0);
        __builtin_amdgcn_sched_barrier(0);
      }
    }
    if (st.on && c < 4) {
      asm volatile("" ::"v"(acc[15][0]));
      st.take(3 + c);
    }
  }
  if (skip) return;
  if (PERSIST && wave == 0) pstamp(hk, 5, lane);

  f32x4 S[2][4];
#pragma unroll
  for (int cI = 0; cI < 4; ++cI) {
    S[0][cI] = acc[0 * 4 + cI] + acc[1 * 4 + cI] + acc[2 * 4 + cI];
    S[1][cI] = pk_sub(pk_sub(acc[1 * 4 + cI], acc[2 * 4 + cI]), acc[3 * 4 + cI]);
  }
  float esum = 0.0f;
  auto emit_pre = [&](int q, int P, f32x4 v) {
    const size_t off = (((size_t)b * QOUT + Q) * kPix + P) * 4;
    if (!e_combine) {
      *(f32x4*)(e_dst + off) = act_fwd(v, e_act);
      return;
    }
    if (e_combine == 2) {
      v *= e_ks;
      if (e_y) v = act_bwd(v, e_yv[q], e_act);
      *(f32x4*)(e_dst + off) = v;
      return;
    }
    if (e_combine == 3) {
      emit_quad<false>(a, b, Q, P, v, esum);
      return;
    }
    const f32x4 kc = act_fwd(v, e_act) * e_ks;
    if (e_kout) *(f32x4*)(e_kout + off) = kc;
    if (e_y) {
      if (e_out1) {
        f32x4 sa = kc * e_c1c;
#pragma unroll
        for (int j = 0; j < 3; ++j)
          if (j < e_np) sa += e_kv[j][q] * e_c1[j];
        *(f32x4*)(e_out1 + off) = e_yv[q] + sa * e_h;
      }
      if (e_out2 || e_nchw) {
        f32x4 sb = kc * e_c2c;
#pragma unroll
        for (int j = 0; j < 3; ++j)
          if (j < e_np) sb += e_kv[j][q] * e_c2[j];
        const f32x4 o2 = e_yv[q] + sb * e_h;
        if (e_out2) *(f32x4*)(e_out2 + off) = o2;
        if (e_nchw) {
          float* o = e_nchw + ((size_t)b * (QOUT * 4) + Q * 4) * kPix + P;
          o[0] = o2.x; o[kPix] = o2.y; o[2 * kPix] = o2.z; o[3 * kPix] = o2.w;
        }
      }
    }
  };
  auto emit_adapt = [&](int q, int P, f32x4 v) {
    const size_t off = (((size_t)b * QOUT + Q) * kPix + P) * 4;
    if (d_kind == 0) {
      *(f32x4*)(e_dst + off) = act_fwd(v, e_act);
    } else if (d_kind == 2) {
      v *= d_ks;
      if (d_has_y) v = act_bwd(v, d_y[q], e_act);
      *(f32x4*)(e_dst + off) = v;
    } else if (d_kind == 1) {
      const f32x4 kc = act_fwd(v, e_act) * d_ks;
      if (d_o[0]) *(f32x4*)(d_o[0] + off) = kc;
      if (d_has_y) {
        if (d_o[1]) *(f32x4*)(d_o[1] + off) = fma4(fma4(kc, d_cA, d_sa[q]), d_h, d_y[q]);
        if (d_err) {
          esum = combine1_err(fma4(kc, d_cB, d_sb[q]), d_h, d_y[q], d_y1[q], d_rtol, d_atol, esum);
        } else if (d_o[2] || d_o[3]) {
          const f32x4 o2 = fma4(fma4(kc, d_cB, d_sb[q]), d_h, d_y[q]);
          if (d_o[2]) *(f32x4*)(d_o[2] + off) = o2;
          if (d_o[3]) {
            float* o = d_o[3] + ((size_t)b * (QOUT * 4) + Q * 4) * kPix + P;
            o[0] = o2.x; o[kPix] = o2.y; o[2 * kPix] = o2.z; o[3 * kPix] = o2.w;
          }
        }
      }
    } else if (d_kind == 3) {
      if (d_o[0]) {
        f32x4 o = v * d_t[0];
        if (d_f[0]) o = fma4(d_y[q], d_t[1], o);
        if (d_f[1]) o = fma4(d_y1[q], d_t[2], o);
        *(f32x4*)(d_o[0] + off) = o;
      }
      if (d_o[1]) {
        f32x4 o = v * d_t[3];
        if (d_f[2]) o = fma4(d_sa[q], d_t[4], o);
        if (d_f[3]) o = fma4(d_sb[q], d_t[5], o);
        *(f32x4*)(d_o[1] + off) = o;
      }
    } else {
      emit_quad(a, b, Q, P, v, esum, a.dbg ? hk.nchw_base + ((size_t)a.dbg - 1) : nullptr);
    }
  };
#pragma unroll
  for (int i = 0; i < 2; ++i) {
    const f32x4 y0 = S[i][0] + S[i][1] + S[i][2] + bias4;
    const f32x4 y1 = pk_sub(pk_sub(S[i][1] + bias4, S[i][2]), S[i][3]);
    const int P = (r0 + 2 * oty + i) * 16 + 2 * otx;
    if constexpr (ADAPT) {
      emit_adapt(2 * i, P, y0);
      emit_adapt(2 * i + 1, P + 1, y1);
    } else if (PERSIST) {
      emit_pre(2 * i, P, y0);
      emit_pre(2 * i + 1, P + 1, y1);
    } else {
      emit_quad(a, b, Q, P, y0, esum);
      emit_quad(a, b, Q, P + 1, y1, esum);
    }
  }
  if (PERSIST) {
    if (a.combine == 1 && a.cmb.err_partials) {
#pragma unroll
      for (int o = 32; o > 0; o >>= 1) esum += __shfl_xor(esum, o, 64);
      const int nwg_pl = (QOUT / 4) * hk.batch, lid_pl = b * (QOUT / 4) + ct * 2 + rh;
      const int bid_pl = (nwg_pl & 7) == 0 ? (lid_pl % (nwg_pl >> 3)) * 8 + lid_pl / (nwg_pl >> 3) : lid_pl;
      if (lane == 0) a.cmb.err_partials[bid_pl * 4 + wave] = esum;
    }
    if (wave == 0) pstamp(hk, 6, lane);
    announce(hk, hk.done + hk.word0 + wave, wave == 0);
  } else {
    finish_err(a, esum, wave);
    st.flush(a);
  }
}

template <int NCHUNK, bool DBG>
__global__ __launch_bounds__(512, 1) void conv3x3_wino_kernel(const float* __restrict__ p_src, const float* __restrict__ p_u,
                                                              int p_qin, int p_qout, const ConvArgs a) {
  extern __shared__ __attribute__((aligned(16))) char smem[];
  (void)p_qout;
  const int nwg = gridDim.x * gridDim.y;
  int lid = blockIdx.x + gridDim.x * blockIdx.y;
  if ((nwg & 7) == 0) lid = (lid & 7) * (nwg >> 3) + (lid >> 3);
  const int rh = lid & 1, ct = (lid >> 1) % (gridDim.x >> 1), b = (lid >> 1) / (gridDim.x >> 1);
  const PersistHook none;
  wino_layer<NCHUNK, DBG, false>(p_src, p_u, p_qin, a, b, ct, rh, smem, none);
}

struct PersistArgs {
  const ConvArgs* table;
  int n_layers, batch;
  unsigned* done;
  unsigned* xcc_of;
  unsigned* host_err;
  float* out_nchw;
  unsigned long long* stamps;
  int sleep6;
  int sleep6_combine;
  const int* n_layers_ptr;
  const unsigned long long* reloc;
  int fault_inject;
};

template <int QOUT>
__device__ __forceinline__ void ew_row(const ConvArgs& a, int b, int ct, int rh, const PersistHook& hk) {
  const int tid = threadIdx.x, lane = tid & 63;
  const int wave = __builtin_amdgcn_readfirstlane(tid >> 6);
  if (wave >= 4) return;
  typedef const __attribute__((address_space(4))) float ConstF;
  const CombineArgs& m = a.cmb;
  const unsigned long long* const rl = hk.reloc;
  const float hs = m.h_ptr ? *(ConstF*)m.h_ptr : 1.0f;
  const int ch = wave >> 1, thh = wave & 1, i16 = lane & 15, kq = lane >> 4;
  const int Q = ct * 8 + ch * 4 + kq, tile = thh * 16 + i16, oty = tile >> 3, otx = tile & 7, r0 = rh * 8;
  const float* const yp = rel(rl, m.y);
  if (a.combine == 5) {
    const float* const pa = rel(rl, m.k_prev[0]);
    const float* const pb = m.n_prev > 1 ? rel(rl, m.k_prev[1]) : nullptr;
    float sum = 0.0f;
#pragma unroll
    for (int q = 0; q < 4; ++q) {
      const size_t o = (((size_t)b * QOUT + Q) * kPix + (r0 + 2 * oty + (q >> 1)) * 16 + 2 * otx + (q & 1)) * 4;
      f32x4 d = *(const f32x4*)(pa + o);
      const f32x4 yv = *(const f32x4*)(yp + o);
      if (pb) d -= *(const f32x4*)(pb + o);
#pragma unroll
      for (int i = 0; i < 4; ++i) {
        const float r = d[i] / __builtin_fmaf(fabsf(yv[i]), m.rtol, m.atol);
        sum = __builtin_fmaf(r, r, sum);
      }
    }
#pragma unroll
    for (int o = 32; o > 0; o >>= 1) sum += __shfl_xor(sum, o, 64);
    if (lane == 0) m.err_partials[(b * 4 + ct * 2 + rh) * 4 + wave] = sum;
    wait_vmcnt<0>();
    if (hk.fence) __builtin_amdgcn_fence(__ATOMIC_RELEASE, "agent");
    if (lane == 0) __hip_atomic_store(hk.done + hk.word0 + wave, hk.target + 1u, __ATOMIC_RELAXED, __HIP_MEMORY_SCOPE_AGENT);
    return;
  }
  float* const o1 = rel(rl, m.out1);
  float* const o2 = rel(rl, m.out2);
  f32x4 s1[4], s2[4];
  size_t off[4];
#pragma unroll
  for (int q = 0; q < 4; ++q) {
    off[q] = (((size_t)b * QOUT + Q) * kPix + (r0 + 2 * oty + (q >> 1)) * 16 + 2 * otx + (q & 1)) * 4;
    s1[q] = f32x4{0.f, 0.f, 0.f, 0.f};
    if (yp) s1[q] = *(const f32x4*)(yp + off[q]);
    s2[q] = s1[q];
  }
  for (int j = 0; j < m.n_prev; ++j) {
    const float* const kp = rel(rl, m.k_prev[j]);
    const float c1 = (m.c_dev ? ((ConstF*)m.c_dev)[j] : m.c1[j]) * hs;
    const float c2 = m.c2[j] * hs;
#pragma unroll
    for (int q = 0; q < 4; ++q) {
      const f32x4 kv = *(const f32x4*)(kp + off[q]);
      s1[q] = fma4(kv, c1, s1[q]);
      if (o2) s2[q] = fma4(kv, c2, s2[q]);
    }
  }
#pragma unroll
  for (int q = 0; q < 4; ++q) {
    if (o1) *(f32x4*)(o1 + off[q]) = s1[q];
    if (o2) *(f32x4*)(o2 + off[q]) = s2[q];
  }
  wait_vmcnt<0>();
  if (hk.fence) __builtin_amdgcn_fence(__ATOMIC_RELEASE, "agent");
  if (lane == 0) __hip_atomic_store(hk.done + hk.word0 + wave, hk.target + 1u, __ATOMIC_RELAXED, __HIP_MEMORY_SCOPE_AGENT);
}

template <bool ADAPT>
__device__ __forceinline__ void persist_walk(const PersistArgs& pa, const ConvArgs* table) {
  extern __shared__ __attribute__((aligned(16))) char smem[];
  const int nwg = gridDim.x;
  const int lid = ((int)blockIdx.x & 7) * (nwg >> 3) + ((int)blockIdx.x >> 3);
  const int rh = lid & 1, ct = (lid >> 1) & 1, group = lid >> 2;
  const bool fence = xcc_rendezvous<4>(pa.xcc_of, lid, pa.xcc_of + nwg, pa.host_err);
  int n_layers = pa.n_layers;
  if (!walk_start(table, n_layers, ADAPT ? pa.n_layers_ptr : nullptr)) return;
  const int n_groups = nwg >> 2;
  for (int b = group; b < pa.batch; b += 2 * n_groups) {
    const int n_interleaved = b + n_groups < pa.batch ? 2 : 1;
    RowCursor cur(table, n_layers);
    int prev_combine = 0;
    for (int l = 0; l < n_layers; ++l) {
      const ConvArgs& a = cur.row(l);
#pragma unroll 1
      for (int s = 0; s < n_interleaved; ++s) {
        const int bs = __builtin_amdgcn_readfirstlane(b + s * n_groups);
        const PersistHook hk = {pa.done + (size_t)bs * kDoneStride, (unsigned)l, (lid & 3) * 4, pa.xcc_of + nwg, pa.host_err, fence,
                                pa.out_nchw, (pa.stamps && lid == 0 && bs == group && l < 64) ? pa.stamps + l * 8 : nullptr, pa.batch,
                                l == 0, n_interleaved == 1, true, true, pa.sleep6 + (prev_combine == 1 ? pa.sleep6_combine : 0),
                                ADAPT ? pa.reloc : nullptr,
                                (unsigned)(ADAPT && a.dep_back > 0 && l > 0 ? l - 1 : l)};
        if constexpr (ADAPT) {
          if (a.combine >= 4) ew_row<16>(a, bs, ct, rh, hk);
          else wino_layer<4, false, true, 16, true>(uniform_ptr(rel(pa.reloc, cur.src)), uniform_ptr(cur.u), 16, a, bs, ct, rh, smem, hk);
        } else {
          wino_layer<4, false, true>(uniform_ptr(cur.src), uniform_ptr(cur.u), 16, a, bs, ct, rh, smem, hk);
        }
      }
      prev_combine = a.combine;
      cur.next();
    }
  }
}

__global__ __launch_bounds__(512, 1) void wino_persist_kernel(const PersistArgs pa) { persist_walk<false>(pa, pa.table); }

__global__ __launch_bounds__(512, 1) void wino_persist_d_kernel(const PersistArgs pa) { persist_walk<true>(pa, pa.table); }

__device__ __forceinline__ void persist_walk_v(const PersistArgs& pa, const ConvArgs* table) {
  extern __shared__ __attribute__((aligned(16))) char smem[];
  const int nwg = gridDim.x;
  const int lid = ((int)blockIdx.x & 7) * (nwg >> 3) + ((int)blockIdx.x >> 3);
  const int rh = lid & 1, ct = (lid >> 1) & 1, group = lid >> 2;
  const bool fence = xcc_rendezvous<4>(pa.xcc_of, lid, pa.xcc_of + nwg, pa.host_err);
  {
    typedef const __attribute__((address_space(4))) int ConstI;
    const int* skip = table[0].skip;
    if (skip && *(ConstI*)skip) return;
  }
  const int n_groups = nwg >> 2;
  for (int b = group; b < pa.batch; b += 2 * n_groups) {
    const int n_interleaved = b + n_groups < pa.batch ? 2 : 1;
    int prev_combine = 0;
    for (int l = 0; l < pa.n_layers; ++l) {
      typedef const __attribute__((address_space(4))) ConvArgs ConstArgs;
      const ConvArgs& a = *(const ConvArgs*)((ConstArgs*)table + l);
      if (l + 1 < pa.n_layers && threadIdx.x < (sizeof(ConvArgs) + 63) / 64) {
        const unsigned v = __builtin_nontemporal_load((const unsigned*)&table[l + 1] + threadIdx.x * 16);
        asm volatile("" ::"v"(v));
      }
      const float* src = uniform_ptr(a.src1);
      const float* u = uniform_ptr(a.w_wino);
      const int qin = a.qin, qout = a.qout;
#pragma unroll 1
      for (int s = 0; s < n_interleaved; ++s) {
        const int bs = __builtin_amdgcn_readfirstlane(b + s * n_groups);
        PersistHook hk = {pa.done + (size_t)bs * kDoneStride, (unsigned)l, (lid & 3) * 4, pa.xcc_of + nwg, pa.host_err, fence,
                          pa.out_nchw, nullptr, pa.batch, l == 0, n_interleaved == 1, true, false,
                          pa.sleep6 + (prev_combine == 1 ? pa.sleep6_combine : 0), nullptr, (unsigned)l};
        if (qout == 16) {
          if (qin == 16) wino_layer<4, false, true, 16>(src, u, 16, a, bs, ct, rh, smem, hk);
          else           wino_layer<8, false, true, 16>(src, u, 32, a, bs, ct, rh, smem, hk);
        } else {
          hk.announce = false;
          wino_layer<4, false, true, 32>(src, u, 16, a, bs, ct, rh, smem, hk);
          hk.announce = true;
          hk.first = true;
          wino_layer<4, false, true, 32>(src, u, 16, a, bs, ct + 2, rh, smem, hk);
        }
      }
      prev_combine = a.combine;
    }
  }
}

__global__ __launch_bounds__(512, 1) void wino_persist_v_kernel(const PersistArgs pa) { persist_walk_v(pa, pa.table); }

template <int NCHUNK, bool DBG>
static int launch_wino_nd(const ConvArgs& a, hipStream_t stream) {
  static bool attr_set = false;
  if (!attr_set) {
    ODEHIP_CHECK_HIP(hipFuncSetAttribute((const void*)conv3x3_wino_kernel<NCHUNK, DBG>, hipFuncAttributeMaxDynamicSharedMemorySize, 160 * 1024));
    attr_set = true;
  }
  hipLaunchKernelGGL((conv3x3_wino_kernel<NCHUNK, DBG>), dim3((a.qout / 8) * 2, a.batch), dim3(512), kWinoLds, stream, a.src1, a.w_wino, a.qin, a.qout, a);
  ODEHIP_CHECK_HIP(hipGetLastError());
  return ODEHIP_OK;
}
template <int NCHUNK>
static int launch_wino_n(const ConvArgs& a, hipStream_t stream) {
  return a.debug ? launch_wino_nd<NCHUNK, true>(a, stream) : launch_wino_nd<NCHUNK, false>(a, stream);
}

int launch_wino_persist(const ConvArgs* table_dev, int n_layers, int batch, unsigned* done, unsigned* xcc_of, unsigned* host_err_dev,
                        float* out_nchw, int grid, hipStream_t stream, bool wide, bool adaptive, const int* n_layers_ptr,
                        const unsigned long long* reloc) {
  static bool attr_set = false;
  ODEHIP_REQUIRE(!(wide && adaptive) && (adaptive || !n_layers_ptr), "wino_persist: no adaptive walk for 128-channel-ended stacks");
  if (!attr_set) {
    ODEHIP_CHECK_HIP(hipFuncSetAttribute((const void*)wino_persist_d_kernel, hipFuncAttributeMaxDynamicSharedMemorySize, 160 * 1024));
    ODEHIP_CHECK_HIP(hipFuncSetAttribute((const void*)wino_persist_v_kernel, hipFuncAttributeMaxDynamicSharedMemorySize, 160 * 1024));
    ODEHIP_CHECK_HIP(hipFuncSetAttribute((const void*)wino_persist_kernel, hipFuncAttributeMaxDynamicSharedMemorySize, 160 * 1024));
    int per_cu = 0;
    ODEHIP_CHECK_HIP(hipOccupancyMaxActiveBlocksPerMultiprocessor(&per_cu, (const void*)wino_persist_kernel, 512, kWinoLds));
    ODEHIP_REQUIRE(per_cu >= 1, "wino_persist: the kernel does not fit a CU");
    ODEHIP_CHECK_HIP(hipOccupancyMaxActiveBlocksPerMultiprocessor(&per_cu, (const void*)wino_persist_d_kernel, 512, kWinoLds));
    ODEHIP_REQUIRE(per_cu >= 1, "wino_persist: the adaptive kernel does not fit a CU");
    attr_set = true;
  }
  PersistArgs pa;
  pa.table = table_dev; pa.n_layers = n_layers; pa.batch = batch; pa.done = done; pa.xcc_of = xcc_of; pa.host_err = host_err_dev;
  pa.out_nchw = out_nchw;
  pa.stamps = g_debug_buf;
  constexpr int kSleep6 = 5;
  constexpr int kSleep6Combine = 4;
  pa.sleep6 = kSleep6;
  pa.sleep6_combine = kSleep6Combine;
  pa.n_layers_ptr = n_layers_ptr;
  pa.reloc = reloc;
  pa.fault_inject = 0;
  if (wide)          hipLaunchKernelGGL(wino_persist_v_kernel, dim3(grid), dim3(512), kWinoLds, stream, pa);
  else if (adaptive) hipLaunchKernelGGL(wino_persist_d_kernel, dim3(grid), dim3(512), kWinoLds, stream, pa);
  else               hipLaunchKernelGGL(wino_persist_kernel, dim3(grid), dim3(512), kWinoLds, stream, pa);
  ODEHIP_CHECK_HIP(hipGetLastError());
  return ODEHIP_OK;
}

constexpr int k16U = 16 * 1024;
constexpr int k16Raw = 8 * 1024;
constexpr int k16V = 16 * 1024;
constexpr int k16X = 8 * 1024;
constexpr int kWino16Lds = 2 * k16U + 2 * k16Raw + 2 * k16V + k16X;

__device__ __forceinline__ void wait_done16(const PersistHook& hk, int lo_word, int hi_word) {
  int n = 0;
  const int lane = threadIdx.x & 63;
  const bool mine = lane >= lo_word && lane < hi_word;
  while (!__all(!mine || __hip_atomic_load(hk.done + lane, __ATOMIC_RELAXED, __HIP_MEMORY_SCOPE_AGENT) >= hk.wait_target)) {
    __builtin_amdgcn_s_sleep(1);
    if ((++n & 1023) == 0) {
      if (__hip_atomic_load(hk.abort_, __ATOMIC_RELAXED, __HIP_MEMORY_SCOPE_AGENT) == 1u) break;
      if (n > (1 << 23)) {
        __hip_atomic_store(hk.abort_, 1u, __ATOMIC_RELAXED, __HIP_MEMORY_SCOPE_AGENT);
        *hk.host_err = 3;
        break;
      }
    }
  }
  if (hk.fence) __builtin_amdgcn_fence(__ATOMIC_ACQUIRE, "agent");
}

__device__ __forceinline__ void wino_layer16(const float* __restrict__ p_src, const float* __restrict__ p_u, const ConvArgs& a, int b,
                                             int cq, int rq, char* smem, const PersistHook& hk) {
  char* const Ub = smem;
  char* const Rb = smem + 2 * k16U;
  char* const Vb = smem + 2 * k16U + 2 * k16Raw;
  char* const Xb = smem + 2 * k16U + 2 * k16Raw + 2 * k16V;
  const int tid = threadIdx.x;
  const int lane = tid & 63;
  const int wave = __builtin_amdgcn_readfirstlane(tid >> 6);
  const int r0 = rq * 4;
  constexpr int nchunk = 4;

  if (wave >= 4) {
    const int pw = wave - 4;
    const int ct = cq >> 1, half = cq & 1;
    const unsigned u_tile_bytes = (unsigned)nchunk * kWU;
    const __amdgpu_buffer_rsrc_t ru = make_rsrc((const char*)p_u + (size_t)ct * u_tile_bytes, u_tile_bytes);
    const __amdgpu_buffer_rsrc_t rx = make_rsrc((const char*)p_src + (size_t)b * 16 * kQuadBytes, 16u * kQuadBytes);
    int vr[2];
#pragma unroll
    for (int p = 0; p < 2; ++p) {
      const int s = 64 * p + lane;
      const int row = s / 20, w = s - row * 20;
      const int pc = w < 9 ? 2 * w : 2 * (w - 9) + 1;
      const int irow = r0 - 1 + row, col = pc - 1;
      vr[p] = (s < 120 && w < 18 && irow >= 0 && irow < kHW && col >= 0 && col < kHW) ? irow * 256 + col * 16 : kOobOffset;
    }
    const int vu = (lane >> 4) * 512 + half * 256 + (lane & 15) * 16;
    auto issue_u = [&](int c, int buf) {
#pragma unroll
      for (int g = 0; g < 4; ++g) {
        const int p = pw * 4 + g;
        dma16(ru, Ub + buf * k16U + p * 1024, vu, c * kWU + p * 2048);
      }
    };
    auto issue_raw = [&](int c, int buf) {
#pragma unroll
      for (int p = 0; p < 2; ++p)
        __builtin_amdgcn_raw_ptr_buffer_load_lds(rx, ODEHIP_LDS_PTR(Rb + buf * k16Raw + pw * 2048 + p * 1024), 16, vr[p],
                                                 (c * 4 + pw) * kQuadBytes, 0, 16);
    };
    const int tt = lane & 15, vi = lane >> 4, tq = pw;
    const int tty = tt >> 3, ttx = tt & 7;
    const int ra = vi == 0 ? 0 : (vi == 1 ? 1 : (vi == 2 ? 2 : 3));
    const int rb = vi == 0 ? 2 : (vi == 1 ? 2 : 1);
    const float sg = vi == 1 ? 1.0f : -1.0f;
    const int raw_base = tq * 2048 + (2 * tty * 20 + ttx) * 16;
    const int off_a = raw_base + ra * 320, off_b = raw_base + rb * 320;
    const int v_off = tq * 256 + tt * 16;
    auto transform = [&](int rbuf, int vbuf) {
      const char* r = Rb + rbuf * k16Raw;
      f32x4 T[4];
#pragma unroll
      for (int j = 0; j < 4; ++j) {
        const int cj = ((j & 1) * 9 + (j >> 1)) * 16;
        const f32x4 da = *(const f32x4*)(r + off_a + cj);
        const f32x4 db = *(const f32x4*)(r + off_b + cj);
        T[j] = da + db * sg;
      }
      char* v = Vb + vbuf * k16V + v_off + vi * 4 * 1024;
      *(f32x4*)(v + 0 * 1024) = pk_sub(T[0], T[2]);
      *(f32x4*)(v + 1 * 1024) = T[1] + T[2];
      *(f32x4*)(v + 2 * 1024) = pk_sub(T[2], T[1]);
      *(f32x4*)(v + 3 * 1024) = pk_sub(T[1], T[3]);
    };
    issue_u(0, 0);
    if (!hk.first) {
      if (hk.wait_target == hk.target)
        for (int i = 0; i < hk.sleep6; ++i) __builtin_amdgcn_s_sleep(6);
      const int lo = rq > 0 ? (rq - 1) * 16 : 0, hi = rq < 3 ? (rq + 2) * 16 : 64;
      wait_done16(hk, lo, hi);
    }
    issue_raw(0, 0);
    issue_raw(1, 1);
    wait_vmcnt<2>();
    transform(0, 0);
#pragma unroll
    for (int c = 0; c < nchunk; ++c) {
      __builtin_amdgcn_s_barrier();
      if (c + 1 < nchunk) {
        issue_u(c + 1, (c + 1) & 1);
        if (c + 2 < nchunk) {
          issue_raw(c + 2, c & 1);
          wait_vmcnt<6>();
        } else {
          wait_vmcnt<4>();
        }
        transform((c + 1) & 1, (c + 1) & 1);
        if (c + 2 < nchunk) wait_vmcnt<2>(); else wait_vmcnt<0>();
      }
    }
    __builtin_amdgcn_s_barrier();
    return;
  }

  const int i16 = lane & 15, kq = lane >> 4;
  f32x4 acc[4];
#pragma unroll
  for (int i = 0; i < 4; ++i) acc[i] = f32x4{0.f, 0.f, 0.f, 0.f};
  const int frag_off = kq * 256 + i16 * 16;
  const int Q = cq * 4 + kq;
  const int oa = wave >> 1, ob = wave & 1;
  const int oty = i16 >> 3, otx = i16 & 7;
  const int P = (r0 + 2 * oty + oa) * 16 + 2 * otx + ob;
  const size_t off = (((size_t)b * 16 + Q) * kPix + P) * 4;
  f32x4 bias4 = {0.f, 0.f, 0.f, 0.f};
  if (a.bias) bias4 = *(const f32x4*)(a.bias + Q * 4);
  const unsigned long long* const rl = hk.reloc;
  typedef const __attribute__((address_space(4))) float ConstF16;
  const bool adapt1 = a.combine == 1 && a.cmb.order == 1 && !(a.cmb.err_partials && (a.cmb.out2 || a.dbg));
  const bool adapt3 = a.combine == 3 && a.bwd.n_targets <= 2 && !a.bwd.h_ptr;
  const int e_combine = adapt1 ? 6 : (adapt3 ? 7 : a.combine);
  const int e_act = a.act;
  float* const e_dst = rel(rl, a.dst);
  f32x4 d_y1 = {0.f, 0.f, 0.f, 0.f}, d_sa = {0.f, 0.f, 0.f, 0.f}, d_sb = {0.f, 0.f, 0.f, 0.f};
  float d_cB = 0.0f, d_rtol = 0.0f, d_atol = 0.0f, d_t[6] = {0.f, 0.f, 0.f, 0.f, 0.f, 0.f};
  float* d_o[2] = {nullptr, nullptr};
  bool d_err = false, d_f[4] = {false, false, false, false};
  float* d_part = nullptr;
  int e_np = 0;
  float* e_kout = nullptr;
  float* e_out1 = nullptr;
  float* e_out2 = nullptr;
  float* e_nchw = nullptr;
  bool e_y = false;
  float e_h = 1.0f, e_ks = 1.0f, e_c1c = 0.0f, e_c2c = 0.0f, e_c1[3] = {0.f, 0.f, 0.f}, e_c2[3] = {0.f, 0.f, 0.f};
  f32x4 e_yv = {0.f, 0.f, 0.f, 0.f}, e_kv[3];
  if (e_combine == 1) {
    const CombineArgs& m = a.cmb;
    e_np = m.n_prev;
    e_h = a.h_by_value ? m.atol : (m.h_ptr ? *(ConstF16*)m.h_ptr : 1.0f);
    e_ks = m.k_scale;
    e_c1c = m.c1[e_np];
    e_c2c = m.c2[e_np];
    e_kout = m.k_out;
    e_out1 = m.out1;
    e_out2 = m.out2;
    e_nchw = a.dbg ? hk.nchw_base + ((size_t)a.dbg - 1) : nullptr;
    e_y = m.y != nullptr;
    if (e_y) e_yv = *(const f32x4*)(m.y + off);
#pragma unroll
    for (int j = 0; j < 3; ++j) {
      if (j < e_np) e_kv[j] = *(const f32x4*)(m.k_prev[j] + off);
      e_c1[j] = m.c1[j];
      e_c2[j] = m.c2[j];
    }
  } else if (e_combine == 2) {
    const BwdArgs& w = a.bwd;
    const float hb = a.h_by_value ? a.cmb.atol : (w.h_ptr ? *(ConstF16*)w.h_ptr : 0.0f);
    e_ks = w.sc_c + w.sc_h * hb;
    e_y = w.mask_src != nullptr;
    if (e_y) e_yv = *(const f32x4*)(rel(rl, w.mask_src) + off);
  } else if (e_combine == 6) {
    const CombineArgs& m = a.cmb;
    e_np = m.n_prev;
    e_h = a.h_by_value ? m.atol : (m.h_ptr ? *(ConstF16*)m.h_ptr : 1.0f);
    e_ks = m.k_scale;
    d_err = m.err_partials != nullptr;
    d_part = m.err_partials;
    e_y = m.y != nullptr;
    e_c1c = m.c1[e_np];
    d_cB = d_err ? m.ce[e_np] : m.c2[e_np];
    d_rtol = m.rtol; d_atol = m.atol;
    e_kout = rel(rl, m.k_out);
    e_out1 = rel(rl, m.out1);
    e_out2 = rel(rl, m.out2);
    e_nchw = m.out2_nchw;
    const bool needB = d_err || e_out2 || e_nchw;
    if (e_y) {
      e_yv = *(const f32x4*)(rel(rl, m.y) + off);
      if (d_err) d_y1 = *(const f32x4*)(rel(rl, m.err_y1) + off);
      const float* kp[ODEHIP_MAX_STAGES - 1];
      float cA[ODEHIP_MAX_STAGES - 1], cB[ODEHIP_MAX_STAGES - 1];
#pragma unroll
      for (int j = 0; j < ODEHIP_MAX_STAGES - 1; ++j) {
        kp[j] = j < e_np ? rel(rl, m.k_prev[j]) : nullptr;
        cA[j] = m.c1[j];
        cB[j] = d_err ? m.ce[j] : m.c2[j];
      }
#pragma unroll
      for (int j = 0; j < ODEHIP_MAX_STAGES - 1; ++j)
        if (j < e_np) {
          const f32x4 kv = *(const f32x4*)(kp[j] + off);
          d_sa = fma4(kv, cA[j], d_sa);
          if (needB) d_sb = fma4(kv, cB[j], d_sb);
        }
    }
  } else if (e_combine == 7) {
    const BwdArgs& w = a.bwd;
#pragma unroll
    for (int t = 0; t < 2; ++t)
      if (t < w.n_targets) {
        const BwdTarget& T = w.tgt[t];
        d_o[t] = rel(rl, T.out);
        d_t[3 * t] = T.g_c; d_t[3 * t + 1] = T.a_c; d_t[3 * t + 2] = T.b_c;
        d_f[2 * t] = T.srcA != nullptr; d_f[2 * t + 1] = T.srcB != nullptr;
        if (t == 0) {
          if (d_f[0]) e_yv = *(const f32x4*)(rel(rl, T.srcA) + off);
          if (d_f[1]) d_y1 = *(const f32x4*)(rel(rl, T.srcB) + off);
        } else {
          if (d_f[2]) d_sa = *(const f32x4*)(rel(rl, T.srcA) + off);
          if (d_f[3]) d_sb = *(const f32x4*)(rel(rl, T.srcB) + off);
        }
      }
  }
#pragma unroll
  for (int c = 0; c < nchunk; ++c) {
    __builtin_amdgcn_s_barrier();
    const char* u = Ub + (c & 1) * k16U + frag_off;
    const char* v = Vb + (c & 1) * k16V + frag_off;
    f32x4 wf[4], xf[4];
#pragma unroll
    for (int i = 0; i < 4; ++i) {
      wf[i] = *(const f32x4*)(u + (4 * i + wave) * 1024);
      xf[i] = *(const f32x4*)(v + (4 * i + wave) * 1024);
    }
#pragma unroll
    for (int i = 0; i < 4; ++i) acc[i] = __builtin_amdgcn_mfma_f32_16x16x4f32(wf[i].x, xf[i].x, acc[i], 0, 0, 0);
#pragma unroll
    for (int i = 0; i < 4; ++i) acc[i] = __builtin_amdgcn_mfma_f32_16x16x4f32(wf[i].y, xf[i].y, acc[i], 0, 0, 0);
#pragma unroll
    for (int i = 0; i < 4; ++i) acc[i] = __builtin_amdgcn_mfma_f32_16x16x4f32(wf[i].z, xf[i].z, acc[i], 0, 0, 0);
#pragma unroll
    for (int i = 0; i < 4; ++i) acc[i] = __builtin_amdgcn_mfma_f32_16x16x4f32(wf[i].w, xf[i].w, acc[i], 0, 0, 0);
  }
  {
    const f32x4 S0 = acc[0] + acc[1] + acc[2];
    const f32x4 S1 = pk_sub(pk_sub(acc[1], acc[2]), acc[3]);
    *(f32x4*)(Xb + (0 * 4 + wave) * 1024 + lane * 16) = S0;
    *(f32x4*)(Xb + (1 * 4 + wave) * 1024 + lane * 16) = S1;
  }
  asm volatile("s_waitcnt lgkmcnt(0)" ::: "memory");
  __builtin_amdgcn_s_barrier();
  f32x4 val;
  {
    const char* x = Xb + oa * 4 * 1024 + lane * 16;
    if (ob == 0) {
      val = *(const f32x4*)(x) + *(const f32x4*)(x + 1024) + *(const f32x4*)(x + 2048) + bias4;
    } else {
      val = pk_sub(pk_sub(*(const f32x4*)(x + 1024) + bias4, *(const f32x4*)(x + 2048)), *(const f32x4*)(x + 3072));
    }
  }
  if (!e_combine) {
    *(f32x4*)(e_dst + off) = act_fwd(val, e_act);
  } else if (e_combine == 2) {
    val *= e_ks;
    if (e_y) val = act_bwd(val, e_yv, e_act);
    *(f32x4*)(e_dst + off) = val;
  } else if (e_combine == 3) {
    float esum = 0.0f;
    emit_quad<false>(a, b, Q, P, val, esum);
  } else if (e_combine == 6) {
    const f32x4 kc = act_fwd(val, e_act) * e_ks;
    if (e_kout) *(f32x4*)(e_kout + off) = kc;
    if (e_y) {
      if (e_out1) *(f32x4*)(e_out1 + off) = fma4(fma4(kc, e_c1c, d_sa), e_h, e_yv);
      if (d_err) {
        float esum = combine1_err(fma4(kc, d_cB, d_sb), e_h, e_yv, d_y1, d_rtol, d_atol, 0.0f);
#pragma unroll
        for (int o = 32; o > 0; o >>= 1) esum += __shfl_xor(esum, o, 64);
        if (lane == 0) d_part[(b * 16 + rq * 4 + cq) * 4 + wave] = esum;
      } else if (e_out2 || e_nchw) {
        const f32x4 o2 = fma4(fma4(kc, d_cB, d_sb), e_h, e_yv);
        if (e_out2) *(f32x4*)(e_out2 + off) = o2;
        if (e_nchw) {
          float* o = e_nchw + ((size_t)b * 64 + Q * 4) * kPix + P;
          o[0] = o2.x; o[kPix] = o2.y; o[2 * kPix] = o2.z; o[3 * kPix] = o2.w;
        }
      }
    }
  } else if (e_combine == 7) {
    if (d_o[0]) {
      f32x4 o = val * d_t[0];
      if (d_f[0]) o = fma4(e_yv, d_t[1], o);
      if (d_f[1]) o = fma4(d_y1, d_t[2], o);
      *(f32x4*)(d_o[0] + off) = o;
    }
    if (d_o[1]) {
      f32x4 o = val * d_t[3];
      if (d_f[2]) o = fma4(d_sa, d_t[4], o);
      if (d_f[3]) o = fma4(d_sb, d_t[5], o);
      *(f32x4*)(d_o[1] + off) = o;
    }
  } else {
    const f32x4 kc = act_fwd(val, e_act) * e_ks;
    if (e_kout) *(f32x4*)(e_kout + off) = kc;
    if (e_y) {
      if (e_out1) {
        f32x4 sa = kc * e_c1c;
#pragma unroll
        for (int j = 0; j < 3; ++j)
          if (j < e_np) sa += e_kv[j] * e_c1[j];
        *(f32x4*)(e_out1 + off) = e_yv + sa * e_h;
      }
      if (e_out2 || e_nchw) {
        f32x4 sb = kc * e_c2c;
#pragma unroll
        for (int j = 0; j < 3; ++j)
          if (j < e_np) sb += e_kv[j] * e_c2[j];
        const f32x4 o2 = e_yv + sb * e_h;
        if (e_out2) *(f32x4*)(e_out2 + off) = o2;
        if (e_nchw) {
          float* o = e_nchw + ((size_t)b * 64 + Q * 4) * kPix + P;
          o[0] = o2.x; o[kPix] = o2.y; o[2 * kPix] = o2.z; o[3 * kPix] = o2.w;
        }
      }
    }
  }
  announce(hk, hk.done + (rq * 4 + cq) * 4 + wave);
}

__device__ __forceinline__ void ew_row16(const ConvArgs& a, int b, int cq, int rq, const PersistHook& hk) {
  const int tid = threadIdx.x, lane = tid & 63;
  const int wave = __builtin_amdgcn_readfirstlane(tid >> 6);
  if (wave >= 4) return;
  typedef const __attribute__((address_space(4))) float ConstF;
  const CombineArgs& m = a.cmb;
  const unsigned long long* const rl = hk.reloc;
  const int i16 = lane & 15, kq = lane >> 4;
  const int Q = cq * 4 + kq, oa = wave >> 1, ob = wave & 1, oty = i16 >> 3, otx = i16 & 7;
  const int P = (rq * 4 + 2 * oty + oa) * 16 + 2 * otx + ob;
  const size_t off = (((size_t)b * 16 + Q) * kPix + P) * 4;
  const float* const yp = rel(rl, m.y);
  if (a.combine == 5) {
    f32x4 d = *(const f32x4*)(rel(rl, m.k_prev[0]) + off);
    const f32x4 yv = *(const f32x4*)(yp + off);
    if (m.n_prev > 1) d -= *(const f32x4*)(rel(rl, m.k_prev[1]) + off);
    float sum = 0.0f;
#pragma unroll
    for (int i = 0; i < 4; ++i) {
      const float r = d[i] / __builtin_fmaf(fabsf(yv[i]), m.rtol, m.atol);
      sum = __builtin_fmaf(r, r, sum);
    }
#pragma unroll
    for (int o = 32; o > 0; o >>= 1) sum += __shfl_xor(sum, o, 64);
    if (lane == 0) m.err_partials[(b * 16 + rq * 4 + cq) * 4 + wave] = sum;
  } else {
    const float hs = m.h_ptr ? *(ConstF*)m.h_ptr : 1.0f;
    float* const o1 = rel(rl, m.out1);
    float* const o2 = rel(rl, m.out2);
    f32x4 s1 = {0.f, 0.f, 0.f, 0.f};
    if (yp) s1 = *(const f32x4*)(yp + off);
    f32x4 s2 = s1;
    for (int j = 0; j < m.n_prev; ++j) {
      const f32x4 kv = *(const f32x4*)(rel(rl, m.k_prev[j]) + off);
      s1 = fma4(kv, (m.c_dev ? ((ConstF*)m.c_dev)[j] : m.c1[j]) * hs, s1);
      if (o2) s2 = fma4(kv, m.c2[j] * hs, s2);
    }
    if (o1) *(f32x4*)(o1 + off) = s1;
    if (o2) *(f32x4*)(o2 + off) = s2;
  }
  announce(hk, hk.done + (rq * 4 + cq) * 4 + wave);
}

__device__ __forceinline__ void nan_fill_row16(const ConvArgs& a, int b, int cq, int rq, const unsigned long long* rl, float* nchw_base) {
  const int tid = threadIdx.x, lane = tid & 63;
  const int wave = __builtin_amdgcn_readfirstlane(tid >> 6);
  if (wave >= 4) return;
  const int i16 = lane & 15, kq = lane >> 4, oa = wave >> 1, ob = wave & 1, oty = i16 >> 3, otx = i16 & 7;
  const int Q = cq * 4 + kq, P = (rq * 4 + 2 * oty + oa) * 16 + 2 * otx + ob;
  const size_t off = (((size_t)b * 16 + Q) * kPix + P) * 4;
  const float nanv = __builtin_nanf("");
  const f32x4 nan4 = {nanv, nanv, nanv, nanv};
  float* outs[6] = {nullptr, nullptr, nullptr, nullptr, nullptr, nullptr};
  float* frame = nullptr;
  if (a.combine == 0 || a.combine == 2) {
    outs[0] = rel(rl, a.dst);
  } else if (a.combine == 1 || a.combine == 4) {
    outs[0] = rel(rl, a.cmb.k_out); outs[1] = rel(rl, a.cmb.out1); outs[2] = rel(rl, a.cmb.out2);
    frame = a.dbg ? nchw_base + ((size_t)a.dbg - 1) : a.cmb.out2_nchw;
  } else if (a.combine == 3) {
    for (int t = 0; t < 4; ++t)
      if (t < a.bwd.n_targets) outs[t] = rel(rl, a.bwd.tgt[t].out);
  }
#pragma unroll
  for (int i = 0; i < 6; ++i)
    if (outs[i]) *(f32x4*)(outs[i] + off) = nan4;
  if (frame) {
    float* o = frame + ((size_t)b * 64 + Q * 4) * kPix + P;
    o[0] = o[kPix] = o[2 * kPix] = o[3 * kPix] = nanv;
  }
  if ((a.combine == 1 || a.combine == 5) && a.cmb.err_partials && lane == 0) a.cmb.err_partials[(b * 16 + rq * 4 + cq) * 4 + wave] = nanv;
}

__global__ __launch_bounds__(512, 1) void wino_persist16_kernel(const PersistArgs pa) {
  extern __shared__ __attribute__((aligned(16))) char smem[];
  const int lid = ((int)blockIdx.x & 7) * 32 + ((int)blockIdx.x >> 3);
  const int xcd = lid >> 5, slot = (lid >> 4) & 1, wg = lid & 15;
  const int b = slot * 8 + xcd;
  const int rq = wg >> 2, cq = wg & 3;
  if (b >= pa.batch) return;
  const bool fence = xcc_rendezvous<16>(pa.xcc_of, lid, pa.xcc_of + gridDim.x, pa.host_err);
  const ConvArgs* table = pa.table;
  int n_layers = pa.n_layers;
  if (!walk_start(table, n_layers, pa.n_layers_ptr)) return;
  RowCursor cur(table, n_layers);
  for (int l = 0; l < n_layers; ++l) {
    const ConvArgs& a = cur.row(l);
    PersistHook hk;
    hk.done = pa.done + (size_t)b * kDoneStride;
    hk.target = (unsigned)l;
    hk.wait_target = (unsigned)(a.dep_back > 0 && l > 0 ? l - 1 : l);
    hk.abort_ = pa.xcc_of + gridDim.x; hk.host_err = pa.host_err;
    hk.fence = fence;
    hk.nchw_base = pa.out_nchw;
    hk.batch = pa.batch;
    hk.first = l == 0;
    hk.solo = true;
    hk.sleep6 = pa.sleep6;
    hk.reloc = pa.reloc;
    if (pa.fault_inject && lid == 0 && l == 1) return;
    if (a.combine >= 4) ew_row16(a, b, cq, rq, hk);
    else wino_layer16(uniform_ptr(rel(pa.reloc, cur.src)), uniform_ptr(cur.u), a, b, cq, rq, smem, hk);
    cur.next();
  }
  if (__hip_atomic_load(pa.xcc_of + gridDim.x, __ATOMIC_RELAXED, __HIP_MEMORY_SCOPE_AGENT) != 0u) {
    for (int l = 0; l < n_layers; ++l) {
      typedef const __attribute__((address_space(4))) ConvArgs ConstArgs;
      nan_fill_row16(*(const ConvArgs*)((ConstArgs*)table + l), b, cq, rq, pa.reloc, pa.out_nchw);
    }
  }
}

int launch_wino_persist16(const ConvArgs* table_dev, int n_layers, int batch, unsigned* done, unsigned* xcc_of, unsigned* host_err_dev,
                          float* out_nchw, hipStream_t stream, const int* n_layers_ptr, const unsigned long long* reloc) {
  static bool attr_set = false;
  ODEHIP_REQUIRE(batch >= 1 && batch <= 16, "wino_persist16: batch %d out of range", batch);
  if (!attr_set) {
    ODEHIP_CHECK_HIP(hipFuncSetAttribute((const void*)wino_persist16_kernel, hipFuncAttributeMaxDynamicSharedMemorySize, 160 * 1024));
    int per_cu = 0;
    ODEHIP_CHECK_HIP(hipOccupancyMaxActiveBlocksPerMultiprocessor(&per_cu, (const void*)wino_persist16_kernel, 512, kWino16Lds));
    ODEHIP_REQUIRE(per_cu >= 1, "wino_persist16: the kernel does not fit a CU");
    attr_set = true;
  }
  PersistArgs pa;
  memset(&pa, 0, sizeof(pa));
  pa.table = table_dev; pa.n_layers = n_layers; pa.batch = batch; pa.done = done; pa.xcc_of = xcc_of; pa.host_err = host_err_dev;
  pa.out_nchw = out_nchw;
  pa.n_layers_ptr = n_layers_ptr;
  pa.reloc = reloc;
  constexpr int kSleep6Upto8 = 4, kSleep6Above8 = 5;
  pa.sleep6 = batch > 8 ? kSleep6Above8 : kSleep6Upto8;
  {
    static int injected = 0;
    const char* e = getenv("ODEHIP_FAULT_INJECT");
    pa.fault_inject = e && e[0] == '1' && injected++ == 0;
  }
  hipLaunchKernelGGL(wino_persist16_kernel, dim3(256), dim3(512), kWino16Lds, stream, pa);
  ODEHIP_CHECK_HIP(hipGetLastError());
  return ODEHIP_OK;
}

int launch_wino(const ConvArgs& a, hipStream_t stream) {
  switch (a.qin / 4) {
    case 1: return launch_wino_n<1>(a, stream);
    case 2: return launch_wino_n<2>(a, stream);
    case 3: return launch_wino_n<3>(a, stream);
    case 4: return launch_wino_n<4>(a, stream);
    case 8: return launch_wino_n<8>(a, stream);
    default: return 1;
  }
}

}
```

### ode-rl_amd/csrc/odehip_internal.h

```cpp
#pragma once
#include <hip/hip_runtime.h>
#include <stddef.h>
#include <stdint.h>
#include <string.h>
#include <time.h>

#include "../../include/odecgru_hip.h"
#include "dopri5_control.h"

namespace odehip {

constexpr int kHW = 16;
constexpr int kPix = kHW * kHW;
constexpr int kQuadBytes = kPix * 16;

void set_error(const char* fmt, ...);
int hip_fail(hipError_t e, const char* what);

#define ODEHIP_CHECK_HIP(expr)                                   \
  do {                                                           \
    hipError_t e__ = (expr);                                     \
    if (e__ != hipSuccess) return ::odehip::hip_fail(e__, #expr); \
  } while (0)

#define ODEHIP_REQUIRE(cond, ...)            \
  do {                                       \
    if (!(cond)) {                           \
      ::odehip::set_error(__VA_ARGS__);      \
      return ODEHIP_EINVAL;                  \
    }                                        \
  } while (0)

constexpr int kActNone = 0;
constexpr int kActRelu = 1;
constexpr int kActTanh = 2;
constexpr int kActTanhSeed = 3;

struct CombineArgs {
  const float* y;
  const float* k_prev[ODEHIP_MAX_STAGES];
  float* k_out;
  float* out1;
  float* out2;
  float* out2_nchw;
  const float* h_ptr;
  int n_prev;
  float c1[ODEHIP_MAX_STAGES + 1];
  float c2[ODEHIP_MAX_STAGES + 1];
  float k_scale;
  const float* err_y1;
  float* err_partials;
  float ce[ODEHIP_MAX_STAGES + 1];
  float rtol, atol;
  int order;
  const float* c_dev;
};

struct BwdTarget {
  float* out;
  const float* srcA;
  const float* srcB;
  float a_c, a_h, b_c, b_h, g_c, g_h;
};
struct BwdArgs {
  const float* mask_src;
  float sc_c, sc_h;
  int n_targets;
  BwdTarget tgt[4];
  const float* h_ptr;
};

struct ConvArgs {
  const float* src1;
  const float* src2;
  const float* w_packed;
  const float* w_wino;
  const void* w_bf16;
  const float* bias;
  float* dst;
  int q1;
  int qin;
  int qout;
  int batch;
  int act;
  int combine;
  int debug;
  int h_by_value;
  int dep_back;
  const int* skip;
  unsigned long long* dbg;
  CombineArgs cmb;
  BwdArgs bwd;
};

int launch_conv(const ConvArgs& a, int ks, hipStream_t stream);
struct ConvRecorder {
  ConvArgs* items;
  int count, capacity;
};
extern thread_local ConvRecorder* g_conv_recorder;
constexpr int kDoneStride = 64;
int launch_wino_persist(const ConvArgs* table_dev, int n_layers, int batch, unsigned* done, unsigned* xcc_of, unsigned* host_err_dev,
                        float* out_nchw, int grid, hipStream_t stream, bool wide = false,
                        bool adaptive = false, const int* n_layers_ptr = nullptr,
                        const unsigned long long* reloc = nullptr);
int launch_ew_row(const ConvArgs& a, hipStream_t stream);
int launch_wino_persist16(const ConvArgs* table_dev, int n_layers, int batch, unsigned* done, unsigned* xcc_of, unsigned* host_err_dev,
                          float* out_nchw, hipStream_t stream, const int* n_layers_ptr = nullptr, const unsigned long long* reloc = nullptr);
int persist_partials_per_sample(int batch);
int launch_wino(const ConvArgs& a, hipStream_t stream);
int launch_wino5(const ConvArgs& a, hipStream_t stream);
int launch_bf16(const ConvArgs& a, hipStream_t stream);
int launch_bf16_5x5(const ConvArgs& a, hipStream_t stream);

struct FusedArgs {
  const float* x;
  const void* w_fused;
  const float* bias[ODEHIP_MAX_LAYERS];
  float* store[ODEHIP_MAX_LAYERS];
  const float* mask[ODEHIP_MAX_LAYERS];
  int n_layers;
  ConvArgs last;
};
int launch_fstack_bf16(const FusedArgs& fa, int batch, hipStream_t stream);
int launch_ftraj_bf16(const odehip_convstack* f, int method, const float* z0_nchw, float* out_nchw, const float* hdev, int n_times,
                      int batch, int negate, hipStream_t stream);
extern int g_debug_flags;
extern unsigned long long* g_debug_buf;


static inline size_t al256(size_t v) { return (v + 255) / 256 * 256; }

int check_stack(const odehip_convstack* f);
inline int grad_slots(const odehip_convstack* f) { return f->n_convs + (f->final_tanh ? 1 : 0); }
inline int wgrad_slot(const odehip_convstack* f, int l) { return (f->final_tanh && l == f->n_convs - 1) ? f->n_convs : l; }
inline bool all_64(const odehip_convstack* f) {
  if (f->ks != 3) return false;
  for (int l = 0; l <= f->n_convs; ++l)
    if (f->channels[l] != 64) return false;
  return true;
}
int traj_prologue(const float* src, float* dst_q4, float* copy_nchw, int batch, int channels, const float* h_host, int n_h, float* hdev,
                  unsigned* zero_words, int n_zero, hipStream_t stream);
int max_hidden(const odehip_convstack* f);
inline bool cell_is_plain(const odehip_convgru_cell* c) { return !c->gn_gates_w && !c->gn_gates_b && !c->gn_can_w && !c->gn_can_b; }
void launch_plain_gates(const float* gates_raw, const float* h, float* u, float* rh, int hidden, int batch, hipStream_t stream);
void launch_plain_update(const float* cand_raw, const float* h, const float* u, float* h_out, float* h_out_nchw, long long nchw_batch_stride,
                         int hidden, int batch, const float* mask_b, hipStream_t stream);
void launch_plain_update_bwd(const float* cand_raw, const float* gh, const float* u, const float* h, float* g_cand_raw, float* g_gates_raw,
                             float* gh_out, int hidden, int batch, const float* mask_b, hipStream_t stream);
void launch_plain_gates_bwd(const float* gates_raw, const float* g_rh, const float* h, float* gh_io, float* g_gates_raw, int hidden,
                            int batch, const float* mask_b, hipStream_t stream);
inline bool step_is_observed(const unsigned char* step_observed_host, int frame) { return !step_observed_host || step_observed_host[frame] != 0; }
void launch_state_to_latent(const float* h, float* h_out_nchw, long long nchw_batch_stride, int hidden, int batch, hipStream_t stream);
int upload_floats(float* dst, const float* src, int n, hipStream_t stream);
int enqueue_f(const odehip_convstack* f, const float* x_q4, int batch, float* ping, float* pong, const CombineArgs* cmb,
              float* plain_dst, const int* skip, hipStream_t stream);
int enqueue_f_saving(const odehip_convstack* f, const float* x_q4, int batch, float* const* hidden, float* ping, float* pong,
                     const CombineArgs* cmb, float* plain_dst, const int* skip, hipStream_t stream);

int enqueue_dgrad_chain(const odehip_convstack* f, const odehip_convstack* f_dgrad, int batch, float* const* gp,
                        const float* const* hidden, const ConvArgs& last, hipStream_t stream);

struct WgradPair {
  const float* g;
  const float* a;
  float scale;
  float pad_[3];
};
constexpr int kWgradSlabFloats = 16 * 64 * 64 + 64;
inline int wgrad_esplit(int batch, int n_eval) {
  int e = batch > 0 ? 256 / batch : 4;
  if (e > n_eval) e = n_eval;
  return e < 4 ? 4 : e;
}
inline int wgrad_esplit_max(int batch) { return batch >= 64 ? 4 : (256 / batch < 4 ? 4 : 256 / batch); }
inline size_t wgrad_slab_bytes(int batch) { return ((size_t)batch * wgrad_esplit_max(batch) + 1) * kWgradSlabFloats * 4; }

struct WgradTile {
  const WgradPair* table;
  int n_eval, batch, esplit;
  float* slabs;
  float* dw;
  float* db;
  int ks, cin_total, co0, ci0;
  int g_quads, g_quad0, a_quads, a_quad0;
  bool write_bias;
};
int launch_wgrad_layer(const WgradPair* table_dev, int n_eval, int batch, int esplit, float* slabs, float* dw, float* db, int ks, int cout,
                       int cin, int cin_total, int ci_off, bool bf16, bool bias, hipStream_t stream);
inline int launch_wgrad(const WgradPair* table_dev, int n_eval, int batch, int esplit, float* slabs, float* dw, float* db, int cout,
                        int cin, hipStream_t stream, bool bf16 = false) {
  return launch_wgrad_layer(table_dev, n_eval, batch, esplit, slabs, dw, db, 3, cout, cin, cin, 0, bf16, true, stream);
}
int launch_wgrad_q4h(const WgradPair* table_dev, int n_eval, int batch, int esplit, float* slabs, float* dw, int accumulate,
                     hipStream_t stream);
int launch_wgrad_wino(const WgradPair* table_dev, int n_eval, int batch, int esplit, float* slabs, float* dw, float* db, int cout,
                      int cin, hipStream_t stream);
int launch_wgrad_wino5(const WgradTile& t, hipStream_t stream);
void launch_slab_sum4(const float* slabs, int n_slabs, int stride, int n_vals, float* sum, hipStream_t stream);
int wgrad_raise_lds(const void* kernel);

int launch_ftraj_bf16_saving(const odehip_convstack* f, const float* z0_nchw, float* out_nchw, const float* hdev, int n_times, int batch,
                             void* save_x, size_t stride_x, void* save_h, size_t stride_h_eval, size_t stride_h_layer,
                             hipStream_t stream);
int launch_btraj_bf16_rk4(const odehip_convstack* f_dgrad, const float* grad_out_nchw, float* grad_z0_nchw, const float* hdev, int n_times,
                          int batch, int n_lo, int n_hi, float* state_g, float* state_seed, const void* save_h, size_t stride_h_eval,
                          size_t stride_h_layer, void* save_g, size_t stride_g_eval, size_t stride_g_layer, float* bias_part,
                          hipStream_t stream);
int launch_bias_reduce(const float* bias_part, int n_parts, int n_layers, float* const* grad_b, hipStream_t stream);

inline void dopri5_stage_combine(CombineArgs& c, int s, const float* y, const float* h_ptr, float* const* k, float* out_next,
                                 float* err_partials, float rtol, float atol) {
  memset(&c, 0, sizeof(c));
  c.y = y;
  c.h_ptr = h_ptr;
  c.n_prev = s - 1;
  for (int j = 0; j < s - 1; ++j) c.k_prev[j] = k[j];
  c.k_out = k[s - 1];
  if (s <= 6) {
    for (int j = 0; j < s; ++j) c.c1[j] = (float)dp5::kBeta[s - 1][j];
    c.out1 = out_next;
  } else {
    for (int j = 0; j < 7; ++j) c.ce[j] = (float)dp5::kCErr[j];
    c.err_y1 = out_next;
    c.err_partials = err_partials;
    c.rtol = rtol;
    c.atol = atol;
  }
}

struct MailboxWatch {
  const volatile int* word;
  int seen;
  double t_progress;
  explicit MailboxWatch(const volatile int* w) : word(w), seen(*w), t_progress(now_s()) {}
  static double now_s() {
    timespec ts;
    clock_gettime(CLOCK_MONOTONIC, &ts);
    return ts.tv_sec + 1e-9 * ts.tv_nsec;
  }
  bool stalled() {
    if (*word != seen) {
      seen = *word;
      t_progress = now_s();
    }
    return now_s() - t_progress > 120.0;
  }
};

inline void write_stats(int* stats_host, int nfe, int n_accept, int n_reject) {
  if (!stats_host) return;
  stats_host[0] = nfe;
  stats_host[1] = n_accept;
  stats_host[2] = n_reject;
}

inline int controller_error(bool adjoint, int status, int max_accept = 0) {
  if (!adjoint) {
    if (status == ODEHIP_ENAN) set_error("odeint_dopri5: non-finite error ratio (non-finite values in state `y`)");
    else if (status == ODEHIP_ENOTCONV) set_error("odeint_dopri5: underflow in dt or max_num_steps exceeded");
    else return ODEHIP_OK;
  } else if (status == ODEHIP_ENAN) {
    set_error("odeint_adjoint_dopri5_backward: non-finite error ratio");
  } else if (status == ODEHIP_ENOTCONV) {
    set_error("odeint_adjoint_dopri5_backward: underflow in dt");
  } else if (status != 0) {
    set_error("odeint_adjoint_dopri5_backward: more than max_accept = %d accepted steps", max_accept);
  }
  return status;
}

}
```

### ode-rl_amd/csrc/persist.h

```cpp
#pragma once
#include <mutex>
#include <vector>

#include "odehip_internal.h"

namespace odehip {

constexpr int kPersistGrid = 256;
inline size_t persist_sync_bytes(int batch) { return ((size_t)batch * kDoneStride + kPersistGrid + 64) * 4; }

class PersistScope {
 public:
  PersistScope();
  ~PersistScope();
  int begin(const odehip_convstack* f, const odehip_convstack* f2, int max_layers, bool small = false);
  bool active() const { return active_; }
  void set_volatile_table(bool v) { volatile_ = v; }
  void set_device_steering(const int* rows_dev, const unsigned long long* reloc_dev) {
    rows_dev_ = rows_dev;
    reloc_dev_ = reloc_dev;
    adaptive_ = true;
  }
  bool recording() const { return active_; }
  int finish(const float* hbuf, const float* hdev, float* out_nchw, int batch, unsigned* sync, int ks, hipStream_t stream,
             bool sync_is_zero = false);
  int guard(float* const* regions, const size_t* floats, int n, hipStream_t stream);
  bool launched() const { return launched_; }
  int relaunch(int batch, unsigned* sync, hipStream_t stream, bool sync_is_zero);

 private:
  std::unique_lock<std::mutex> lock_;
  std::vector<ConvArgs> items_;
  ConvRecorder rec_ = {nullptr, 0, 0};
  bool active_ = false;
  bool eval_walk_small_only_ = false;
  bool eval_walk_ = false;
  bool adaptive_ = false;
  bool volatile_ = false;
  const int* rows_dev_ = nullptr;
  const unsigned long long* reloc_dev_ = nullptr;
  bool launched_ = false;
  const unsigned* abort_word_ = nullptr;
  const ConvArgs* table_ = nullptr;
  int table_rows_ = 0;
  bool table_wide_ = false, table_adaptive_ = false, table_small16_ = false;
};

bool persist_switch_on();
void persist_count_launch();

int staged_upload(void* dst_dev, const void* src, size_t bytes, hipStream_t stream);

unsigned persist_error(bool clear);

}
```

### ode-rl_amd/csrc/persist.hip

```cpp
#include <stdlib.h>
#include <string.h>

#include "persist.h"

namespace odehip {

struct PersistState {
  std::mutex mu;
  struct Entry {
    std::vector<char> host;
    ConvArgs* dev = nullptr;
    size_t cap = 0;
    unsigned long long stamp = 0;
  } tab[8];
  unsigned long long clock = 0;
  unsigned* host_err = nullptr;
  unsigned* host_err_dev = nullptr;
  int enabled = -1;
  long long launches = 0;
  static constexpr int kVolSlots = 4;
  struct VolSlot {
    ConvArgs* dev = nullptr;
    size_t cap = 0;
    hipEvent_t ev = nullptr;
    bool pending = false;
  } vol[kVolSlots];
  int vol_next = 0;
  int vol_last = -1;
  unsigned* eval_sync = nullptr;
  int eval_batch_cap = 0;
};
static PersistState g_persist;

static bool persist_available() {
  PersistState& P = g_persist;
  if (P.enabled >= 0) return P.enabled == 1;
  P.enabled = 0;
  const char* env = getenv("ODEHIP_PERSISTENT");
  if (env && env[0] == '0') return false;
  int dev = 0, cus = 0;
  if (hipGetDevice(&dev) != hipSuccess) return false;
  if (hipDeviceGetAttribute(&cus, hipDeviceAttributeMultiprocessorCount, dev) != hipSuccess || cus < kPersistGrid) return false;
  if (hipHostMalloc((void**)&P.host_err, 64, hipHostMallocMapped) != hipSuccess) return false;
  *P.host_err = 0;
  if (hipHostGetDevicePointer((void**)&P.host_err_dev, P.host_err, 0) != hipSuccess) return false;
  P.enabled = 1;
  return true;
}

static int persist_layer_kind(const ConvArgs& a) {
  if (a.combine == 4 || a.combine == 5) return a.qout == 16 && !a.src2 ? 3 : 0;
  if (a.act == kActTanhSeed) return 0;
  if (!a.w_wino || a.w_bf16 || a.src2 || a.q1 != a.qin || a.combine < 0 || a.combine > 3) return 0;
  if (a.qin == 16 && a.qout == 16) return (a.combine == 1 && a.cmb.order == 1) ? 3 : 1;
  if ((a.qin == 32 && a.qout == 16) || (a.qin == 16 && a.qout == 32)) return 2;
  return 0;
}

static const ConvArgs* persist_table(const ConvArgs* items, int n, hipStream_t stream) {
  PersistState& P = g_persist;
  const size_t bytes = (size_t)n * sizeof(ConvArgs);
  PersistState::Entry* lru = &P.tab[0];
  for (auto& e : P.tab) {
    if (e.dev && e.host.size() == bytes && memcmp(e.host.data(), items, bytes) == 0) {
      e.stamp = ++P.clock;
      return e.dev;
    }
    if (e.stamp < lru->stamp) lru = &e;
  }
  if (hipStreamSynchronize(stream) != hipSuccess) return nullptr;
  if (lru->cap < bytes) {
    if (lru->dev) (void)hipFree(lru->dev);
    lru->dev = nullptr;
    lru->cap = 0;
    if (hipMalloc((void**)&lru->dev, bytes) != hipSuccess) return nullptr;
    lru->cap = bytes;
  }
  lru->host.assign((const char*)items, (const char*)items + bytes);
  if (hipMemcpy(lru->dev, items, bytes, hipMemcpyHostToDevice) != hipSuccess) {
    lru->host.clear();
    return nullptr;
  }
  lru->stamp = ++P.clock;
  return lru->dev;
}

struct StageSlot {
  char* host = nullptr;
  size_t cap = 0;
  hipEvent_t ev = nullptr;
  bool pending = false;
};
static std::mutex g_stage_mu;
static StageSlot g_stage[8];
static int g_stage_next = 0;
int staged_upload(void* dst_dev, const void* src, size_t bytes, hipStream_t stream) {
  if (bytes == 0) return ODEHIP_OK;
  std::lock_guard<std::mutex> lk(g_stage_mu);
  StageSlot& v = g_stage[g_stage_next];
  g_stage_next = (g_stage_next + 1) % 8;
  if (v.pending) {
    ODEHIP_CHECK_HIP(hipEventSynchronize(v.ev));
    v.pending = false;
  }
  if (!v.ev) ODEHIP_CHECK_HIP(hipEventCreateWithFlags(&v.ev, hipEventDisableTiming));
  if (v.cap < bytes) {
    if (v.host) (void)hipHostFree(v.host);
    v.host = nullptr;
    v.cap = 0;
    const size_t cap = (bytes + 65535) / 65536 * 65536;
    ODEHIP_CHECK_HIP(hipHostMalloc((void**)&v.host, cap, hipHostMallocDefault));
    v.cap = cap;
  }
  memcpy(v.host, src, bytes);
  ODEHIP_CHECK_HIP(hipMemcpyAsync(dst_dev, v.host, bytes, hipMemcpyHostToDevice, stream));
  ODEHIP_CHECK_HIP(hipEventRecord(v.ev, stream));
  v.pending = true;
  return ODEHIP_OK;
}

static const ConvArgs* persist_table_async(const ConvArgs* items, int n, hipStream_t stream) {
  PersistState& P = g_persist;
  const size_t bytes = (size_t)n * sizeof(ConvArgs);
  PersistState::VolSlot& v = P.vol[P.vol_next];
  if (v.pending) {
    if (hipEventSynchronize(v.ev) != hipSuccess) return nullptr;
    v.pending = false;
  }
  if (!v.ev && hipEventCreateWithFlags(&v.ev, hipEventDisableTiming) != hipSuccess) return nullptr;
  if (v.cap < bytes) {
    if (v.dev) (void)hipFree(v.dev);
    v.dev = nullptr;
    v.cap = 0;
    const size_t cap = (bytes + 65535) / 65536 * 65536;
    if (hipMalloc((void**)&v.dev, cap) != hipSuccess) return nullptr;
    v.cap = cap;
  }
  if (staged_upload(v.dev, items, bytes, stream) != ODEHIP_OK) return nullptr;
  P.vol_last = P.vol_next;
  P.vol_next = (P.vol_next + 1) % PersistState::kVolSlots;
  return v.dev;
}
static void persist_table_async_done(hipStream_t stream) {
  PersistState& P = g_persist;
  if (P.vol_last < 0) return;
  PersistState::VolSlot& v = P.vol[P.vol_last];
  P.vol_last = -1;
  if (hipEventRecord(v.ev, stream) == hipSuccess) v.pending = true;
  else (void)hipStreamSynchronize(stream);
}

constexpr int kGuardRegions = 24;
struct GuardArgs {
  const unsigned* abort_word;
  int n;
  float* p[kGuardRegions];
  unsigned long long floats[kGuardRegions];
};

__global__ void persist_guard_kernel(const GuardArgs a) {
  if (__hip_atomic_load(a.abort_word, __ATOMIC_RELAXED, __HIP_MEMORY_SCOPE_AGENT) == 0) return;
  for (int r = 0; r < a.n; ++r)
    for (unsigned long long i = (unsigned long long)blockIdx.x * blockDim.x + threadIdx.x; i < a.floats[r]; i += (unsigned long long)gridDim.x * blockDim.x)
      a.p[r][i] = __builtin_nanf("");
}

static bool walk16_on() {
  static const bool on16 = [] { const char* e = getenv("ODEHIP_PERSIST16"); return !(e && e[0] == '0'); }();
  return on16;
}

int persist_partials_per_sample(int batch) {
  std::lock_guard<std::mutex> g(g_persist.mu);
  return batch <= 16 && walk16_on() && persist_available() ? 64 : 16;
}

bool persist_switch_on() {
  std::lock_guard<std::mutex> g(g_persist.mu);
  if (g_persist.enabled == 0) return false;
  static const bool env_off = [] { const char* e = getenv("ODEHIP_PERSISTENT"); return e && e[0] == '0'; }();
  return !env_off;
}

void persist_count_launch() {
  std::lock_guard<std::mutex> g(g_persist.mu);
  ++g_persist.launches;
}

static unsigned persist_error_locked(bool clear) {
  PersistState& P = g_persist;
  if (!P.host_err) return 0;
  const unsigned code = *P.host_err;
  if (code && clear) {
    *P.host_err = 0;
    P.enabled = 0;
  }
  return code;
}

unsigned persist_error(bool clear) {
  std::lock_guard<std::mutex> g(g_persist.mu);
  return persist_error_locked(clear);
}

PersistScope::PersistScope() : lock_(g_persist.mu, std::defer_lock) {}

int PersistScope::guard(float* const* regions, const size_t* floats, int n, hipStream_t stream) {
  if (!launched_ || !abort_word_) return ODEHIP_OK;
  for (int base = 0; base < n; base += kGuardRegions) {
    GuardArgs a;
    memset(&a, 0, sizeof(a));
    a.abort_word = abort_word_;
    a.n = n - base < kGuardRegions ? n - base : kGuardRegions;
    for (int i = 0; i < a.n; ++i) {
      a.p[i] = regions[base + i];
      a.floats[i] = regions[base + i] ? floats[base + i] : 0;
    }
    hipLaunchKernelGGL(persist_guard_kernel, dim3(64), dim3(256), 0, stream, a);
    ODEHIP_CHECK_HIP(hipGetLastError());
  }
  return ODEHIP_OK;
}
PersistScope::~PersistScope() {
  if (g_conv_recorder == &rec_) g_conv_recorder = nullptr;
}

int PersistScope::begin(const odehip_convstack* f, const odehip_convstack* f2, int max_layers, bool small) {
    if (small && (g_conv_recorder || max_layers > 5)) return ODEHIP_OK;
    if (f2 && f->final_tanh) return ODEHIP_OK;
    static const int eval_walk_env = [] { const char* e = getenv("ODEHIP_EVAL_WALK"); return e ? (e[0] == '1' ? 1 : 0) : -1; }();
    eval_walk_small_only_ = eval_walk_env < 0;
    if (small) {
      if (eval_walk_env == 0) return ODEHIP_OK;
      eval_walk_ = true;
      volatile_ = true;
      for (int l = 0; l <= f->n_convs; ++l)
        if (f->channels[l] != 64) return ODEHIP_OK;
    }
    if (f->ks != 3 || f->w_fused || (f2 && f2->w_fused) || g_debug_flags) return ODEHIP_OK;
    for (int l = 0; l <= f->n_convs; ++l)
      if (f->channels[l] != 64 && f->channels[l] != 128) return ODEHIP_OK;
    for (int l = 0; l < f->n_convs; ++l)
      if (f->channels[l] == 128 && f->channels[l + 1] == 128) return ODEHIP_OK;
    for (int l = 0; l < f->n_convs; ++l)
      if (!f->w_wino[l] || f->w_bf16[l] || (f2 && (!f2->w_wino[l] || f2->w_bf16[l]))) return ODEHIP_OK;
    lock_.lock();
    if (!persist_available()) {
      lock_.unlock();
      return ODEHIP_OK;
    }
    if (*g_persist.host_err) {
      const unsigned code = *g_persist.host_err;
      *g_persist.host_err = 0;
      g_persist.enabled = 0;
      set_error("an earlier persistent launch gave up waiting for a partner workgroup (code %u); its result is invalid.  "
                "Persistent launches are now disabled for this process", code);
      return ODEHIP_EINVAL;
    }
    items_.resize((size_t)max_layers);
    rec_.items = items_.data();
    rec_.count = 0;
    rec_.capacity = max_layers;
    g_conv_recorder = &rec_;
    active_ = true;
    return ODEHIP_OK;
  }

int PersistScope::finish(const float* hbuf, const float* hdev, float* out_nchw, int batch, unsigned* sync, int ks, hipStream_t stream,
                         bool sync_is_zero) {
    if (g_conv_recorder == &rec_) g_conv_recorder = nullptr;
    if (!active_) return ODEHIP_OK;
    active_ = false;
    const bool eval_skip = eval_walk_ && eval_walk_small_only_ && (batch > 16 || !walk16_on());
    if (eval_walk_ && !sync && !eval_skip) {
      PersistState& P = g_persist;
      if (batch > P.eval_batch_cap) {
        bool ok = hipStreamSynchronize(stream) == hipSuccess;
        if (ok && P.eval_sync) (void)hipFree(P.eval_sync);
        P.eval_sync = nullptr;
        P.eval_batch_cap = 0;
        const int cap = batch < 64 ? 64 : batch;
        ok = ok && hipMalloc((void**)&P.eval_sync, persist_sync_bytes(cap)) == hipSuccess;
        if (ok) P.eval_batch_cap = cap;
      }
      sync = P.eval_sync;
      sync_is_zero = false;
    }
    bool all_ok = rec_.count > 0 && !(eval_walk_ && !sync), wide = false, adaptive = adaptive_;
    if (eval_skip) all_ok = false;
    for (int i = 0; i < rec_.count && all_ok; ++i) {
      const int kind = persist_layer_kind(rec_.items[i]);
      all_ok = kind != 0;
      wide = wide || kind == 2;
      adaptive = adaptive || kind == 3;
    }
    if (wide && adaptive) all_ok = false;
    const ConvArgs* table = nullptr;
    if (all_ok) {
      for (int i = 0; i < rec_.count; ++i) {
        ConvArgs& a = rec_.items[i];
        a.dbg = nullptr;
        a.h_by_value = 0;
        if (hbuf) {
          const float* hp = a.combine == 1 ? a.cmb.h_ptr : (a.combine >= 2 ? a.bwd.h_ptr : nullptr);
          a.cmb.atol = hp ? hbuf[hp - hdev] : (a.combine == 1 ? 1.0f : 0.0f);
          a.h_by_value = 1;
        }
        if (a.combine == 1 && a.cmb.out2_nchw) {
          a.dbg = (unsigned long long*)(uintptr_t)((size_t)(a.cmb.out2_nchw - out_nchw) + 1);
          a.cmb.out2_nchw = nullptr;
        }
      }
      table = volatile_ ? persist_table_async(rec_.items, rec_.count, stream) : persist_table(rec_.items, rec_.count, stream);
    }
    int rc;
    bool small16 = false;
    if (table && !wide && batch <= 16 && walk16_on()) {
      small16 = true;
      for (int i = 0; i < rec_.count && small16; ++i) {
        const ConvArgs& a = rec_.items[i];
        if (a.combine >= 4) continue;
        small16 = a.qin == 16 && a.qout == 16 &&
                  (a.combine == 0 || a.combine == 2 || a.combine == 3 ||
                   (a.combine == 1 && (((a.h_by_value || eval_walk_) && a.cmb.n_prev <= 3 && !a.cmb.err_partials && !a.cmb.order) ||
                                       (a.cmb.order == 1 && !(a.cmb.err_partials && (a.cmb.out2 || a.cmb.out2_nchw))))));
      }
      if (adaptive && !small16) {
        set_error("persistent walk: an adaptive table of batch %d has a row the sixteen-workgroup walk does not take", batch);
        return ODEHIP_EINVAL;
      }
    }
    if (table) {
      if (!sync_is_zero) ODEHIP_CHECK_HIP(hipMemsetAsync(sync, 0, persist_sync_bytes(batch), stream));
      if (small16) rc = launch_wino_persist16(table, rec_.count, batch, sync, sync + (size_t)batch * kDoneStride, g_persist.host_err_dev, out_nchw, stream,
                                              rows_dev_, reloc_dev_);
      else
      rc = launch_wino_persist(table, rec_.count, batch, sync, sync + (size_t)batch * kDoneStride, g_persist.host_err_dev, out_nchw,
                               kPersistGrid, stream, wide, adaptive, rows_dev_, reloc_dev_);
      if (volatile_) persist_table_async_done(stream);
      if (rc == ODEHIP_OK) {
        ++g_persist.launches;
        launched_ = true;
        abort_word_ = sync + (size_t)batch * kDoneStride + kPersistGrid;
        table_ = table;
        table_rows_ = rec_.count;
        table_wide_ = wide;
        table_adaptive_ = adaptive;
        table_small16_ = small16;
        return rc;
      }
      g_persist.enabled = 0;
      (void)hipGetLastError();
    }
    if (rows_dev_ || reloc_dev_) {
      set_error("the persistent walk refused a device-steered table (%d rows): it cannot be replayed as ordinary launches", rec_.count);
      return ODEHIP_EHIP;
    }
    for (int i = 0; i < rec_.count; ++i) {
      ConvArgs a = rec_.items[i];
      if (a.dbg) a.cmb.out2_nchw = out_nchw + ((size_t)(uintptr_t)a.dbg - 1);
      a.dbg = nullptr;
      if (a.h_by_value && a.combine != 1) a.cmb.atol = 0.0f;
      a.h_by_value = 0;
      if ((rc = launch_conv(a, ks, stream)) != ODEHIP_OK) return rc;
    }
    return ODEHIP_OK;
  }

int PersistScope::relaunch(int batch, unsigned* sync, hipStream_t stream, bool sync_is_zero) {
  ODEHIP_REQUIRE(launched_ && table_ && !volatile_, "persistent relaunch without a table");
  if (!sync_is_zero) ODEHIP_CHECK_HIP(hipMemsetAsync(sync, 0, persist_sync_bytes(batch), stream));
  const int rc = table_small16_
                     ? launch_wino_persist16(table_, table_rows_, batch, sync, sync + (size_t)batch * kDoneStride, g_persist.host_err_dev, nullptr,
                                             stream, rows_dev_, reloc_dev_)
                     : launch_wino_persist(table_, table_rows_, batch, sync, sync + (size_t)batch * kDoneStride, g_persist.host_err_dev, nullptr,
                                           kPersistGrid, stream, table_wide_, table_adaptive_, rows_dev_, reloc_dev_);
  if (rc == ODEHIP_OK) ++g_persist.launches;
  return rc;
}

}

using namespace odehip;

extern "C" int odehip_set_persistent_trajectory(int enable) {
  std::lock_guard<std::mutex> g(g_persist.mu);
  const int was = g_persist.enabled != 0;
  g_persist.enabled = enable ? (g_persist.host_err ? 1 : -1) : 0;
  return was;
}

extern "C" int odehip_persistent_error(int clear) {
  return (int)persist_error(clear != 0);
}

extern "C" long long odehip_persistent_trajectory_launches(void) {
  std::lock_guard<std::mutex> g(g_persist.mu);
  return g_persist.launches;
}
```

Baseline: 489,900 latent frames/s.

## Add strip walk: four workgroups per sample split rows of persistent conv stack

Adds a new persistent Winograd kernel in which each sample is handled by a group of four workgroups, each owning a 4-row strip. Strips synchronise with only their neighbouring strips (a halo wait) rather than the whole sample. It is enabled by default when the table is a fixed-grid 64-channel table and batch fits in grid/4. The epilogue is also factored into a reusable struct. The goal is to spread each sample's layer chain across more CUs and cut per-layer serialization, at the cost of finer-grained cross-workgroup synchronisation and extra halo loads.

```diff
diff --git a/include/odecgru_hip.h b/include/odecgru_hip.h
--- a/include/odecgru_hip.h
+++ b/include/odecgru_hip.h
@@ -345,6 +345,8 @@
 
 int odehip_set_persistent_trajectory(int enable);
 long long odehip_persistent_trajectory_launches(void);
+int odehip_set_strip_walk(int enable);
+long long odehip_strip_walk_launches(void);
 int odehip_persistent_error(int clear);
 
 int odehip_mmnist_render(const double* init, const int* digit_ids, const unsigned char* glyphs, int n_glyphs,
diff --git a/ode-rl_amd/_lib.py b/ode-rl_amd/_lib.py
--- a/ode-rl_amd/_lib.py
+++ b/ode-rl_amd/_lib.py
@@ -133,6 +133,8 @@
                                    [ctypes.c_float] * 5 + [ctypes.c_int, ctypes.c_void_p, ctypes.c_void_p]),
     "odehip_set_persistent_trajectory": (ctypes.c_int, [ctypes.c_int]),
     "odehip_persistent_trajectory_launches": (ctypes.c_longlong, []),
+    "odehip_set_strip_walk": (ctypes.c_int, [ctypes.c_int]),
+    "odehip_strip_walk_launches": (ctypes.c_longlong, []),
     "odehip_persistent_error": (ctypes.c_int, [ctypes.c_int]),
     "odehip_upsample2x_bilinear": (ctypes.c_int, [ctypes.c_void_p, ctypes.c_void_p, ctypes.c_longlong, ctypes.c_int, ctypes.c_int, ctypes.c_void_p]),
     "odehip_upsample2x_bilinear_backward": (ctypes.c_int, [ctypes.c_void_p, ctypes.c_void_p, ctypes.c_longlong, ctypes.c_int, ctypes.c_int,
diff --git a/ode-rl_amd/csrc/conv_wino.hip b/ode-rl_amd/csrc/conv_wino.hip
--- a/ode-rl_amd/csrc/conv_wino.hip
+++ b/ode-rl_amd/csrc/conv_wino.hip
@@ -150,6 +150,104 @@
   }
 };
 
+template <int QOUT>
+struct PreEpilogue {
+  int combine = 0, act = 0, np = 0;
+  float* dst = nullptr;
+  float* kout = nullptr;
+  float* out1 = nullptr;
+  float* out2 = nullptr;
+  float* nchw = nullptr;
+  bool y = false;
+  float h = 1.0f, ks = 1.0f, c1c = 0.0f, c2c = 0.0f, c1[3] = {0.f, 0.f, 0.f}, c2[3] = {0.f, 0.f, 0.f};
+  f32x4 yv[4], kv[3][4];
+
+  __device__ __forceinline__ void fetch(const ConvArgs& a, const PersistHook& hk, int b, int Q, int row0, int otx) {
+    combine = a.combine;
+    act = a.act;
+    dst = a.dst;
+    if (combine == 1 && !a.h_by_value) combine = 3;
+    if (combine == 2) {
+      const BwdArgs& w = a.bwd;
+      typedef const __attribute__((address_space(4))) float ConstF;
+      const float hb = a.h_by_value ? a.cmb.atol : (w.h_ptr ? *(ConstF*)w.h_ptr : 0.0f);
+      ks = w.sc_c + w.sc_h * hb;
+      y = w.mask_src != nullptr;
+#pragma unroll
+      for (int q = 0; q < 4; ++q) {
+        const size_t off = (((size_t)b * QOUT + Q) * kPix + (row0 + (q >> 1)) * 16 + 2 * otx + (q & 1)) * 4;
+        if (y) yv[q] = *(const f32x4*)(w.mask_src + off);
+      }
+    } else if (combine == 1) {
+      const CombineArgs& m = a.cmb;
+      np = m.n_prev;
+      h = m.atol;
+      ks = m.k_scale;
+      c1c = m.c1[np];
+      c2c = m.c2[np];
+      kout = m.k_out;
+      out1 = m.out1;
+      out2 = m.out2;
+      nchw = a.dbg ? hk.nchw_base + ((size_t)a.dbg - 1) : nullptr;
+      y = m.y != nullptr;
+#pragma unroll
+      for (int q = 0; q < 4; ++q) {
+        const size_t off = (((size_t)b * QOUT + Q) * kPix + (row0 + (q >> 1)) * 16 + 2 * otx + (q & 1)) * 4;
+        if (y) yv[q] = *(const f32x4*)(m.y + off);
+#pragma unroll
+        for (int j = 0; j < 3; ++j)
+          if (j < np) kv[j][q] = *(const f32x4*)(m.k_prev[j] + off);
+      }
+#pragma unroll
+      for (int j = 0; j < 3; ++j) {
+        c1[j] = m.c1[j];
+        c2[j] = m.c2[j];
+      }
+    }
+  }
+
+  __device__ __forceinline__ void emit(const ConvArgs& a, int b, int Q, int q, int P, f32x4 v, float& esum) const {
+    const size_t off = (((size_t)b * QOUT + Q) * kPix + P) * 4;
+    if (!combine) {
+      *(f32x4*)(dst + off) = act_fwd(v, act);
+      return;
+    }
+    if (combine == 2) {
+      v *= ks;
+      if (y) v = act_bwd(v, yv[q], act);
+      *(f32x4*)(dst + off) = v;
+      return;
+    }
+    if (combine == 3) {
+      emit_quad<false>(a, b, Q, P, v, esum);
+      return;
+    }
+    const f32x4 kc = act_fwd(v, act) * ks;
+    if (kout) *(f32x4*)(kout + off) = kc;
+    if (y) {
+      if (out1) {
+        f32x4 sa = kc * c1c;
+#pragma unroll
+        for (int j = 0; j < 3; ++j)
+          if (j < np) sa += kv[j][q] * c1[j];
+        *(f32x4*)(out1 + off) = yv[q] + sa * h;
+      }
+      if (out2 || nchw) {
+        f32x4 sb = kc * c2c;
+#pragma unroll
+        for (int j = 0; j < 3; ++j)
+          if (j < np) sb += kv[j][q] * c2[j];
+        const f32x4 o2 = yv[q] + sb * h;
+        if (out2) *(f32x4*)(out2 + off) = o2;
+        if (nchw) {
+          float* o = nchw + ((size_t)b * (QOUT * 4) + Q * 4) * kPix + P;
+          o[0] = o2.x; o[kPix] = o2.y; o[2 * kPix] = o2.z; o[3 * kPix] = o2.w;
+        }
+      }
+    }
+  }
+};
+
 template <int NCHUNK, bool DBG, bool PERSIST, int QOUT = 16, bool ADAPT = false>
 __device__ __forceinline__ void wino_layer(const float* __restrict__ p_src, const float* __restrict__ p_u, int p_qin, const ConvArgs& a,
                                            int b, int ct, int rh, char* smem, const PersistHook& hk) {
@@ -290,15 +388,7 @@
   f32x4 bias4 = {0.f, 0.f, 0.f, 0.f};
   if (a.bias) bias4 = *(const f32x4*)(a.bias + Q * 4);
   const int tile = thh * 16 + i16, oty = tile >> 3, otx = tile & 7;
-  int e_combine = 0, e_act = 0, e_np = 0;
-  float* e_dst = nullptr;
-  float* e_kout = nullptr;
-  float* e_out1 = nullptr;
-  float* e_out2 = nullptr;
-  float* e_nchw = nullptr;
-  bool e_y = false;
-  float e_h = 1.0f, e_ks = 1.0f, e_c1c = 0.0f, e_c2c = 0.0f, e_c1[3] = {0.f, 0.f, 0.f}, e_c2[3] = {0.f, 0.f, 0.f};
-  f32x4 e_yv[4], e_kv[3][4];
+  PreEpilogue<QOUT> ep;
   int d_kind = 0;
   f32x4 d_y[4], d_y1[4], d_sa[4], d_sb[4];
   float d_h = 1.0f, d_ks = 1.0f, d_cA = 0.0f, d_cB = 0.0f, d_rtol = 0.0f, d_atol = 0.0f, d_t[6] = {0.f, 0.f, 0.f, 0.f, 0.f, 0.f};
@@ -307,8 +397,8 @@
   if constexpr (ADAPT) {
     typedef const __attribute__((address_space(4))) float ConstF;
     const unsigned long long* const rl = hk.reloc;
-    e_act = a.act;
-    e_dst = rel(rl, a.dst);
+    ep.act = a.act;
+    ep.dst = rel(rl, a.dst);
     d_kind = a.combine == 0 ? 0 : 5;
     if (a.combine == 2) {
       const BwdArgs& w = a.bwd;
@@ -396,47 +486,7 @@
       }
     }
   } else if (PERSIST) {
-    e_combine = a.combine;
-    e_act = a.act;
-    e_dst = a.dst;
-    if (e_combine == 1 && !a.h_by_value) e_combine = 3;
-    if (e_combine == 2) {
-      const BwdArgs& w = a.bwd;
-      typedef const __attribute__((address_space(4))) float ConstF;
-      const float hb = a.h_by_value ? a.cmb.atol : (w.h_ptr ? *(ConstF*)w.h_ptr : 0.0f);
-      e_ks = w.sc_c + w.sc_h * hb;
-      e_y = w.mask_src != nullptr;
-#pragma unroll
-      for (int q = 0; q < 4; ++q) {
-        const size_t off = (((size_t)b * QOUT + Q) * kPix + (r0 + 2 * oty + (q >> 1)) * 16 + 2 * otx + (q & 1)) * 4;
-        if (e_y) e_yv[q] = *(const f32x4*)(w.mask_src + off);
-      }
-    } else if (e_combine == 1) {
-      const CombineArgs& m = a.cmb;
-      e_np = m.n_prev;
-      e_h = m.atol;
-      e_ks = m.k_scale;
-      e_c1c = m.c1[e_np];
-      e_c2c = m.c2[e_np];
-      e_kout = m.k_out;
-      e_out1 = m.out1;
-      e_out2 = m.out2;
-      e_nchw = a.dbg ? hk.nchw_base + ((size_t)a.dbg - 1) : nullptr;
-      e_y = m.y != nullptr;
-#pragma unroll
-      for (int q = 0; q < 4; ++q) {
-        const size_t off = (((size_t)b * QOUT + Q) * kPix + (r0 + 2 * oty + (q >> 1)) * 16 + 2 * otx + (q & 1)) * 4;
-        if (e_y) e_yv[q] = *(const f32x4*)(m.y + off);
-#pragma unroll
-        for (int j = 0; j < 3; ++j)
-          if (j < e_np) e_kv[j][q] = *(const f32x4*)(m.k_prev[j] + off);
-      }
-#pragma unroll
-      for (int j = 0; j < 3; ++j) {
-        e_c1[j] = m.c1[j];
-        e_c2[j] = m.c2[j];
-      }
-    }
+    ep.fetch(a, hk, b, Q, r0 + 2 * oty, otx);
   }
   st.take(2);
 #pragma unroll
@@ -490,56 +540,16 @@
     S[1][cI] = pk_sub(pk_sub(acc[1 * 4 + cI], acc[2 * 4 + cI]), acc[3 * 4 + cI]);
   }
   float esum = 0.0f;
-  auto emit_pre = [&](int q, int P, f32x4 v) {
-    const size_t off = (((size_t)b * QOUT + Q) * kPix + P) * 4;
-    if (!e_combine) {
-      *(f32x4*)(e_dst + off) = act_fwd(v, e_act);
-      return;
-    }
-    if (e_combine == 2) {
-      v *= e_ks;
-      if (e_y) v = act_bwd(v, e_yv[q], e_act);
-      *(f32x4*)(e_dst + off) = v;
-      return;
-    }
-    if (e_combine == 3) {
-      emit_quad<false>(a, b, Q, P, v, esum);
-      return;
-    }
-    const f32x4 kc = act_fwd(v, e_act) * e_ks;
-    if (e_kout) *(f32x4*)(e_kout + off) = kc;
-    if (e_y) {
-      if (e_out1) {
-        f32x4 sa = kc * e_c1c;
-#pragma unroll
-        for (int j = 0; j < 3; ++j)
-          if (j < e_np) sa += e_kv[j][q] * e_c1[j];
-        *(f32x4*)(e_out1 + off) = e_yv[q] + sa * e_h;
-      }
-      if (e_out2 || e_nchw) {
-        f32x4 sb = kc * e_c2c;
-#pragma unroll
-        for (int j = 0; j < 3; ++j)
-          if (j < e_np) sb += e_kv[j][q] * e_c2[j];
-        const f32x4 o2 = e_yv[q] + sb * e_h;
-        if (e_out2) *(f32x4*)(e_out2 + off) = o2;
-        if (e_nchw) {
-          float* o = e_nchw + ((size_t)b * (QOUT * 4) + Q * 4) * kPix + P;
-          o[0] = o2.x; o[kPix] = o2.y; o[2 * kPix] = o2.z; o[3 * kPix] = o2.w;
-        }
-      }
-    }
-  };
   auto emit_adapt = [&](int q, int P, f32x4 v) {
     const size_t off = (((size_t)b * QOUT + Q) * kPix + P) * 4;
     if (d_kind == 0) {
-      *(f32x4*)(e_dst + off) = act_fwd(v, e_act);
+      *(f32x4*)(ep.dst + off) = act_fwd(v, ep.act);
     } else if (d_kind == 2) {
       v *= d_ks;
-      if (d_has_y) v = act_bwd(v, d_y[q], e_act);
-      *(f32x4*)(e_dst + off) = v;
+      if (d_has_y) v = act_bwd(v, d_y[q], ep.act);
+      *(f32x4*)(ep.dst + off) = v;
     } else if (d_kind == 1) {
-      const f32x4 kc = act_fwd(v, e_act) * d_ks;
+      const f32x4 kc = act_fwd(v, ep.act) * d_ks;
       if (d_o[0]) *(f32x4*)(d_o[0] + off) = kc;
       if (d_has_y) {
         if (d_o[1]) *(f32x4*)(d_o[1] + off) = fma4(fma4(kc, d_cA, d_sa[q]), d_h, d_y[q]);
@@ -580,8 +590,8 @@
       emit_adapt(2 * i, P, y0);
       emit_adapt(2 * i + 1, P + 1, y1);
     } else if (PERSIST) {
-      emit_pre(2 * i, P, y0);
-      emit_pre(2 * i + 1, P + 1, y1);
+      ep.emit(a, b, Q, 2 * i, P, y0, esum);
+      ep.emit(a, b, Q, 2 * i + 1, P + 1, y1, esum);
     } else {
       emit_quad(a, b, Q, P, y0, esum);
       emit_quad(a, b, Q, P + 1, y1, esum);
@@ -789,6 +799,8 @@
 
 __global__ __launch_bounds__(512, 1) void wino_persist_v_kernel(const PersistArgs pa) { persist_walk_v(pa, pa.table); }
 
+__global__ void wino_persist_strip_kernel(const PersistArgs pa);
+
 template <int NCHUNK, bool DBG>
 static int launch_wino_nd(const ConvArgs& a, hipStream_t stream) {
   static bool attr_set = false;
@@ -807,18 +819,22 @@
 
 int launch_wino_persist(const ConvArgs* table_dev, int n_layers, int batch, unsigned* done, unsigned* xcc_of, unsigned* host_err_dev,
                         float* out_nchw, int grid, hipStream_t stream, bool wide, bool adaptive, const int* n_layers_ptr,
-                        const unsigned long long* reloc) {
+                        const unsigned long long* reloc, bool strip) {
   static bool attr_set = false;
   ODEHIP_REQUIRE(!(wide && adaptive) && (adaptive || !n_layers_ptr), "wino_persist: no adaptive walk for 128-channel-ended stacks");
+  ODEHIP_REQUIRE(!strip || (!wide && !adaptive && batch <= grid / 4), "wino_persist: the strip walk takes fixed-grid 64-channel tables, one sample per group");
   if (!attr_set) {
     ODEHIP_CHECK_HIP(hipFuncSetAttribute((const void*)wino_persist_d_kernel, hipFuncAttributeMaxDynamicSharedMemorySize, 160 * 1024));
     ODEHIP_CHECK_HIP(hipFuncSetAttribute((const void*)wino_persist_v_kernel, hipFuncAttributeMaxDynamicSharedMemorySize, 160 * 1024));
     ODEHIP_CHECK_HIP(hipFuncSetAttribute((const void*)wino_persist_kernel, hipFuncAttributeMaxDynamicSharedMemorySize, 160 * 1024));
+    ODEHIP_CHECK_HIP(hipFuncSetAttribute((const void*)wino_persist_strip_kernel, hipFuncAttributeMaxDynamicSharedMemorySize, 160 * 1024));
     int per_cu = 0;
     ODEHIP_CHECK_HIP(hipOccupancyMaxActiveBlocksPerMultiprocessor(&per_cu, (const void*)wino_persist_kernel, 512, kWinoLds));
     ODEHIP_REQUIRE(per_cu >= 1, "wino_persist: the kernel does not fit a CU");
     ODEHIP_CHECK_HIP(hipOccupancyMaxActiveBlocksPerMultiprocessor(&per_cu, (const void*)wino_persist_d_kernel, 512, kWinoLds));
     ODEHIP_REQUIRE(per_cu >= 1, "wino_persist: the adaptive kernel does not fit a CU");
+    ODEHIP_CHECK_HIP(hipOccupancyMaxActiveBlocksPerMultiprocessor(&per_cu, (const void*)wino_persist_strip_kernel, 512, kWinoLds));
+    ODEHIP_REQUIRE(per_cu >= 1, "wino_persist: the strip kernel does not fit a CU");
     attr_set = true;
   }
   PersistArgs pa;
@@ -827,12 +843,14 @@
   pa.stamps = g_debug_buf;
   constexpr int kSleep6 = 5;
   constexpr int kSleep6Combine = 4;
-  pa.sleep6 = kSleep6;
-  pa.sleep6_combine = kSleep6Combine;
+  constexpr int kStripSleep6 = 10, kStripSleep6Combine = 4;
+  pa.sleep6 = strip ? kStripSleep6 : kSleep6;
+  pa.sleep6_combine = strip ? kStripSleep6Combine : kSleep6Combine;
   pa.n_layers_ptr = n_layers_ptr;
   pa.reloc = reloc;
   pa.fault_inject = 0;
-  if (wide)          hipLaunchKernelGGL(wino_persist_v_kernel, dim3(grid), dim3(512), kWinoLds, stream, pa);
+  if (strip)         hipLaunchKernelGGL(wino_persist_strip_kernel, dim3(grid), dim3(512), kWinoLds, stream, pa);
+  else if (wide)     hipLaunchKernelGGL(wino_persist_v_kernel, dim3(grid), dim3(512), kWinoLds, stream, pa);
   else if (adaptive) hipLaunchKernelGGL(wino_persist_d_kernel, dim3(grid), dim3(512), kWinoLds, stream, pa);
   else               hipLaunchKernelGGL(wino_persist_kernel, dim3(grid), dim3(512), kWinoLds, stream, pa);
   ODEHIP_CHECK_HIP(hipGetLastError());
@@ -1315,6 +1333,187 @@
   return ODEHIP_OK;
 }
 
+constexpr int kStripLds = 2 * k16Raw + 2 * k16V;
+static_assert(kStripLds <= kWinoLds, "the strip walk is launched with the other walks' LDS request");
+
+__device__ __forceinline__ void wino_strip_layer(const float* __restrict__ p_src, const float* __restrict__ p_u, const ConvArgs& a, int b,
+                                                 int rq, char* smem, const PersistHook& hk) {
+  char* const Rb = smem;
+  char* const Vb = smem + 2 * k16Raw;
+  const int tid = threadIdx.x;
+  const int lane = tid & 63;
+  const int wave = __builtin_amdgcn_readfirstlane(tid >> 6);
+  const int r0 = rq * 4;
+  constexpr int nchunk = 4;
+
+  if (wave >= 4) {
+    const int pw = wave - 4;
+    const __amdgpu_buffer_rsrc_t rx = make_rsrc((const char*)p_src + (size_t)b * 16 * kQuadBytes, 16u * kQuadBytes);
+    int vr[2];
+#pragma unroll
+    for (int p = 0; p < 2; ++p) {
+      const int s = 64 * p + lane;
+      const int row = s / 20, w = s - row * 20;
+      const int pc = w < 9 ? 2 * w : 2 * (w - 9) + 1;
+      const int irow = r0 - 1 + row, col = pc - 1;
+      vr[p] = (s < 120 && w < 18 && irow >= 0 && irow < kHW && col >= 0 && col < kHW) ? irow * 256 + col * 16 : kOobOffset;
+    }
+    auto issue_raw = [&](int c, int buf) {
+#pragma unroll
+      for (int p = 0; p < 2; ++p)
+        __builtin_amdgcn_raw_ptr_buffer_load_lds(rx, ODEHIP_LDS_PTR(Rb + buf * k16Raw + pw * 2048 + p * 1024), 16, vr[p],
+                                                 (c * 4 + pw) * kQuadBytes, 0, 16);
+    };
+    const int tt = lane & 15, vi = lane >> 4, tq = pw;
+    const int tty = tt >> 3, ttx = tt & 7;
+    const int ra = vi;
+    const int rb = vi < 2 ? 2 : 1;
+    const float sg = vi == 1 ? 1.0f : -1.0f;
+    const int raw_base = tq * 2048 + (2 * tty * 20 + ttx) * 16;
+    const int off_a = raw_base + ra * 320, off_b = raw_base + rb * 320;
+    const int v_off = tq * 256 + tt * 16;
+    auto transform = [&](int rbuf, int vbuf) {
+      const char* r = Rb + rbuf * k16Raw;
+      f32x4 T[4];
+#pragma unroll
+      for (int j = 0; j < 4; ++j) {
+        const int cj = ((j & 1) * 9 + (j >> 1)) * 16;
+        const f32x4 da = *(const f32x4*)(r + off_a + cj);
+        const f32x4 db = *(const f32x4*)(r + off_b + cj);
+        T[j] = da + db * sg;
+      }
+      char* v = Vb + vbuf * k16V + v_off + vi * 4 * 1024;
+      *(f32x4*)(v + 0 * 1024) = pk_sub(T[0], T[2]);
+      *(f32x4*)(v + 1 * 1024) = T[1] + T[2];
+      *(f32x4*)(v + 2 * 1024) = pk_sub(T[2], T[1]);
+      *(f32x4*)(v + 3 * 1024) = pk_sub(T[1], T[3]);
+    };
+    if (pw == 0) pstamp(hk, 0, lane);
+    if (!hk.first) {
+      for (int i = 0; i < hk.sleep6; ++i) __builtin_amdgcn_s_sleep(6);
+      wait_done16(hk, rq > 0 ? (rq - 1) * 4 : 0, rq < 3 ? (rq + 2) * 4 : 16);
+    }
+    if (pw == 0) pstamp(hk, 1, lane);
+    issue_raw(0, 0);
+    issue_raw(1, 1);
+    wait_vmcnt<2>();
+    if (pw == 0) pstamp(hk, 2, lane);
+    transform(0, 0);
+    if (pw == 0) pstamp(hk, 3, lane);
+#pragma unroll
+    for (int c = 0; c < nchunk; ++c) {
+      __builtin_amdgcn_s_barrier();
+      if (c + 1 < nchunk) {
+        if (c + 2 < nchunk) {
+          issue_raw(c + 2, c & 1);
+          wait_vmcnt<2>();
+        } else {
+          wait_vmcnt<0>();
+        }
+        transform((c + 1) & 1, (c + 1) & 1);
+      }
+    }
+    return;
+  }
+
+  const int i16 = lane & 15, kq = lane >> 4;
+  f32x4 acc[16];
+#pragma unroll
+  for (int x = 0; x < 16; ++x) acc[x] = f32x4{0.f, 0.f, 0.f, 0.f};
+  const int u_off = (wave >> 1) * (nchunk * kWU) + kq * 512 + ((wave & 1) * 16 + i16) * 16;
+  const int v_off = kq * 256 + i16 * 16;
+  constexpr int kG = 16 * nchunk;
+  const __amdgpu_buffer_rsrc_t ru = make_rsrc(p_u, 2u * nchunk * kWU);
+  f32x4 uw[kUAhead];
+#pragma unroll
+  for (int g = 0; g < kUAhead; ++g) uw[g] = load_u(ru, u_off, g * 2048);
+  const int Q = wave * 4 + kq;
+  f32x4 bias4 = {0.f, 0.f, 0.f, 0.f};
+  if (a.bias) bias4 = *(const f32x4*)(a.bias + Q * 4);
+  const int oty = i16 >> 3, otx = i16 & 7;
+  PreEpilogue<16> ep;
+  ep.fetch(a, hk, b, Q, r0 + 2 * oty, otx);
+#pragma unroll
+  for (int c = 0; c < nchunk; ++c) {
+    __builtin_amdgcn_s_barrier();
+    if (c == 0 && wave == 0) pstamp(hk, 4, lane);
+    const char* v = Vb + (c & 1) * k16V + v_off;
+    f32x4 x0 = *(const f32x4*)(v), x1 = *(const f32x4*)(v + 1024);
+    f32x4 x0n, x1n;
+#pragma unroll
+    for (int x = 0; x < 16; x += 2) {
+      const int g = c * 16 + x, s0 = g % kUAhead, s1 = (g + 1) % kUAhead;
+      const f32x4 w0 = uw[s0], w1 = uw[s1];
+      if (x + 2 < 16) {
+        x0n = *(const f32x4*)(v + (x + 2) * 1024);
+        x1n = *(const f32x4*)(v + (x + 3) * 1024);
+      }
+      if (g + kUAhead < kG) {
+        uw[s0] = load_u(ru, u_off, (g + kUAhead) * 2048);
+        uw[s1] = load_u(ru, u_off, (g + kUAhead + 1) * 2048);
+      }
+      acc[x] = __builtin_amdgcn_mfma_f32_16x16x4f32(w0.x, x0.x, acc[x], 0, 0, 0);
+      acc[x + 1] = __builtin_amdgcn_mfma_f32_16x16x4f32(w1.x, x1.x, acc[x + 1], 0, 0, 0);
+      acc[x] = __builtin_amdgcn_mfma_f32_16x16x4f32(w0.y, x0.y, acc[x], 0, 0, 0);
+      acc[x + 1] = __builtin_amdgcn_mfma_f32_16x16x4f32(w1.y, x1.y, acc[x + 1], 0, 0, 0);
+      acc[x] = __builtin_amdgcn_mfma_f32_16x16x4f32(w0.z, x0.z, acc[x], 0, 0, 0);
+      acc[x + 1] = __builtin_amdgcn_mfma_f32_16x16x4f32(w1.z, x1.z, acc[x + 1], 0, 0, 0);
+      acc[x] = __builtin_amdgcn_mfma_f32_16x16x4f32(w0.w, x0.w, acc[x], 0, 0, 0);
+      acc[x + 1] = __builtin_amdgcn_mfma_f32_16x16x4f32(w1.w, x1.w, acc[x + 1], 0, 0, 0);
+      x0 = x0n; x1 = x1n;
+      __builtin_amdgcn_sched_group_barrier(0x008, 1, 0);
+      __builtin_amdgcn_sched_group_barrier(0x100, 2, 0);
+      __builtin_amdgcn_sched_group_barrier(0x020, 2, 0);
+      __builtin_amdgcn_sched_group_barrier(0x008, 7, 0);
+      __builtin_amdgcn_sched_barrier(0);
+    }
+  }
+  if (wave == 0) pstamp(hk, 5, lane);
+
+  f32x4 S[2][4];
+#pragma unroll
+  for (int cI = 0; cI < 4; ++cI) {
+    S[0][cI] = acc[0 * 4 + cI] + acc[1 * 4 + cI] + acc[2 * 4 + cI];
+    S[1][cI] = pk_sub(pk_sub(acc[1 * 4 + cI], acc[2 * 4 + cI]), acc[3 * 4 + cI]);
+  }
+  float esum = 0.0f;
+#pragma unroll
+  for (int i = 0; i < 2; ++i) {
+    const f32x4 y0 = S[i][0] + S[i][1] + S[i][2] + bias4;
+    const f32x4 y1 = pk_sub(pk_sub(S[i][1] + bias4, S[i][2]), S[i][3]);
+    const int P = (r0 + 2 * oty + i) * 16 + 2 * otx;
+    ep.emit(a, b, Q, 2 * i, P, y0, esum);
+    ep.emit(a, b, Q, 2 * i + 1, P + 1, y1, esum);
+  }
+  if (wave == 0) pstamp(hk, 6, lane);
+  announce(hk, hk.done + hk.word0 + wave, wave == 0);
+}
+
+__global__ __launch_bounds__(512, 1) void wino_persist_strip_kernel(const PersistArgs pa) {
+  extern __shared__ __attribute__((aligned(16))) char smem[];
+  const int nwg = gridDim.x;
+  const int lid = ((int)blockIdx.x & 7) * (nwg >> 3) + ((int)blockIdx.x >> 3);
+  const int rq = lid & 3, group = lid >> 2;
+  const bool fence = xcc_rendezvous<4>(pa.xcc_of, lid, pa.xcc_of + nwg, pa.host_err);
+  const ConvArgs* table = pa.table;
+  int n_layers = pa.n_layers;
+  if (!walk_start(table, n_layers, nullptr)) return;
+  const int n_groups = nwg >> 2;
+  for (int b = group; b < pa.batch; b += n_groups) {
+    RowCursor cur(table, n_layers);
+    int prev_combine = 0;
+    for (int l = 0; l < n_layers; ++l) {
+      const ConvArgs& a = cur.row(l);
+      const PersistHook hk = {pa.done + (size_t)b * kDoneStride, (unsigned)l, rq * 4, pa.xcc_of + nwg, pa.host_err, fence,
+                              pa.out_nchw, (pa.stamps && lid == 0 && b == group && l < 64) ? pa.stamps + l * 8 : nullptr, pa.batch,
+                              l == 0, true, true, false, pa.sleep6 + (prev_combine == 1 ? pa.sleep6_combine : 0), nullptr, (unsigned)l};
+      wino_strip_layer(uniform_ptr(cur.src), uniform_ptr(cur.u), a, b, rq, smem, hk);
+      prev_combine = a.combine;
+      cur.next();
+    }
+  }
+}
+
 int launch_wino(const ConvArgs& a, hipStream_t stream) {
   switch (a.qin / 4) {
     case 1: return launch_wino_n<1>(a, stream);
diff --git a/ode-rl_amd/csrc/odehip_internal.h b/ode-rl_amd/csrc/odehip_internal.h
--- a/ode-rl_amd/csrc/odehip_internal.h
+++ b/ode-rl_amd/csrc/odehip_internal.h
@@ -103,7 +103,8 @@
 int launch_wino_persist(const ConvArgs* table_dev, int n_layers, int batch, unsigned* done, unsigned* xcc_of, unsigned* host_err_dev,
                         float* out_nchw, int grid, hipStream_t stream, bool wide = false,
                         bool adaptive = false, const int* n_layers_ptr = nullptr,
-                        const unsigned long long* reloc = nullptr);
+                        const unsigned long long* reloc = nullptr,
+                        bool strip = false);
 int launch_ew_row(const ConvArgs& a, hipStream_t stream);
 int launch_wino_persist16(const ConvArgs* table_dev, int n_layers, int batch, unsigned* done, unsigned* xcc_of, unsigned* host_err_dev,
                           float* out_nchw, hipStream_t stream, const int* n_layers_ptr = nullptr, const unsigned long long* reloc = nullptr);
diff --git a/ode-rl_amd/csrc/persist.h b/ode-rl_amd/csrc/persist.h
--- a/ode-rl_amd/csrc/persist.h
+++ b/ode-rl_amd/csrc/persist.h
@@ -43,7 +43,7 @@
   const unsigned* abort_word_ = nullptr;
   const ConvArgs* table_ = nullptr;
   int table_rows_ = 0;
-  bool table_wide_ = false, table_adaptive_ = false, table_small16_ = false;
+  bool table_wide_ = false, table_adaptive_ = false, table_small16_ = false, table_strip_ = false;
 };
 
 bool persist_switch_on();
diff --git a/ode-rl_amd/csrc/persist.hip b/ode-rl_amd/csrc/persist.hip
--- a/ode-rl_amd/csrc/persist.hip
+++ b/ode-rl_amd/csrc/persist.hip
@@ -18,6 +18,8 @@
   unsigned* host_err_dev = nullptr;
   int enabled = -1;
   long long launches = 0;
+  int strip = -1;
+  long long strip_launches = 0;
   static constexpr int kVolSlots = 4;
   struct VolSlot {
     ConvArgs* dev = nullptr;
@@ -170,6 +172,15 @@
   return on16;
 }
 
+static bool strip_walk_on() {
+  PersistState& P = g_persist;
+  if (P.strip < 0) {
+    const char* e = getenv("ODEHIP_STRIP_WALK");
+    P.strip = !(e && e[0] == '0');
+  }
+  return P.strip == 1;
+}
+
 int persist_partials_per_sample(int batch) {
   std::lock_guard<std::mutex> g(g_persist.mu);
   return batch <= 16 && walk16_on() && persist_available() ? 64 : 16;
@@ -330,16 +341,25 @@
         return ODEHIP_EINVAL;
       }
     }
+    bool strip = false;
+    if (table && !wide && !adaptive && !small16 && !eval_walk_ && hbuf && batch <= kPersistGrid / 4 && strip_walk_on()) {
+      strip = true;
+      for (int i = 0; i < rec_.count && strip; ++i) {
+        const ConvArgs& a = rec_.items[i];
+        strip = !(a.combine == 1 && (a.cmb.err_partials || a.cmb.n_prev > 3));
+      }
+    }
     if (table) {
       if (!sync_is_zero) ODEHIP_CHECK_HIP(hipMemsetAsync(sync, 0, persist_sync_bytes(batch), stream));
       if (small16) rc = launch_wino_persist16(table, rec_.count, batch, sync, sync + (size_t)batch * kDoneStride, g_persist.host_err_dev, out_nchw, stream,
                                               rows_dev_, reloc_dev_);
       else
       rc = launch_wino_persist(table, rec_.count, batch, sync, sync + (size_t)batch * kDoneStride, g_persist.host_err_dev, out_nchw,
-                               kPersistGrid, stream, wide, adaptive, rows_dev_, reloc_dev_);
+                               kPersistGrid, stream, wide, adaptive, rows_dev_, reloc_dev_, strip);
       if (volatile_) persist_table_async_done(stream);
       if (rc == ODEHIP_OK) {
         ++g_persist.launches;
+        if (strip) ++g_persist.strip_launches;
         launched_ = true;
         abort_word_ = sync + (size_t)batch * kDoneStride + kPersistGrid;
         table_ = table;
@@ -347,6 +367,7 @@
         table_wide_ = wide;
         table_adaptive_ = adaptive;
         table_small16_ = small16;
+        table_strip_ = strip;
         return rc;
       }
       g_persist.enabled = 0;
@@ -374,8 +395,11 @@
                      ? launch_wino_persist16(table_, table_rows_, batch, sync, sync + (size_t)batch * kDoneStride, g_persist.host_err_dev, nullptr,
                                              stream, rows_dev_, reloc_dev_)
                      : launch_wino_persist(table_, table_rows_, batch, sync, sync + (size_t)batch * kDoneStride, g_persist.host_err_dev, nullptr,
-                                           kPersistGrid, stream, table_wide_, table_adaptive_, rows_dev_, reloc_dev_);
-  if (rc == ODEHIP_OK) ++g_persist.launches;
+                                           kPersistGrid, stream, table_wide_, table_adaptive_, rows_dev_, reloc_dev_, table_strip_);
+  if (rc == ODEHIP_OK) {
+    ++g_persist.launches;
+    if (table_strip_) ++g_persist.strip_launches;
+  }
   return rc;
 }
 
@@ -390,6 +414,18 @@
   return was;
 }
 
+extern "C" int odehip_set_strip_walk(int enable) {
+  std::lock_guard<std::mutex> g(g_persist.mu);
+  const int was = strip_walk_on();
+  g_persist.strip = enable ? 1 : 0;
+  return was;
+}
+
+extern "C" long long odehip_strip_walk_launches(void) {
+  std::lock_guard<std::mutex> g(g_persist.mu);
+  return g_persist.strip_launches;
+}
+
 extern "C" int odehip_persistent_error(int clear) {
   return (int)persist_error(clear != 0);
 }
```

Result: faster. 530,200 latent frames/s (median of 6 runs) (+8.2%).
